# zhipeng-wei/Image-to-Video-I2V-attack

Hardware: AMD Instinct MI355X
Metric: adversarial frames/sec (10-step I2V, ResNet-50 layer3, 32x224^2 clips) (higher is better)
Workload: dtype f32

## Files before the change

### image-to-video-i2v-attack_amd/csrc/i2v_be.h

```cpp
#pragma once
#include <hip/hip_runtime.h>
#include <math.h>
#include <stdint.h>
#include <stdio.h>
#include <stdlib.h>
#include <string.h>

#include <type_traits>
#include <utility>

#include "i2v_kernels.h"

typedef float f32x16 __attribute__((ext_vector_type(16)));
typedef float f32x4 __attribute__((ext_vector_type(4)));

extern thread_local char g_be_err[256];
extern thread_local bool g_be_has_err;
int hip_fail(hipError_t e, const char* what);
#define HIPCHK(x) do { hipError_t e_ = (x); if (e_ != hipSuccess) return hip_fail(e_, #x); } while (0)
#define LAUNCH_CHECK(name) do { hipError_t e_ = hipGetLastError(); if (e_ != hipSuccess) return hip_fail(e_, name); } while (0)
extern long long g_stat_conv, g_stat_pws, g_stat_bf3, g_stat_igh, g_stat_sth, g_stat_fastblock, g_stat_vfma, g_stat_igv, g_stat_gconv;

__device__ __forceinline__ unsigned fastdiv(unsigned n, unsigned m, unsigned s) {
    return (unsigned)(((unsigned long long)n * m) >> s);
}
static inline void fastdiv_magic(unsigned d, uint32_t* m, uint32_t* s) {
    unsigned l = 0; while ((1ull << l) < d) ++l;
    *s = 31 + l;
    *m = (uint32_t)(((1ull << (31 + l)) / d) + 1);
}
typedef int i2v_v4i __attribute__((ext_vector_type(4)));
__device__ __forceinline__ I2VKEntry load_kentry(const I2VKEntry* tab, int k) {
#if defined(__HIP_DEVICE_COMPILE__)
    const i2v_v4i v = ((const __attribute__((address_space(4))) i2v_v4i*)tab)[k];
    return I2VKEntry{v.x, v.y, v.z, v.w};
#else
    return tab[k];
#endif
}

static inline void conv_magics(I2VConvParams& p) {
    fastdiv_magic((unsigned)(p.Hg * p.Wg), &p.dv_hw_m, &p.dv_hw_s);
    fastdiv_magic((unsigned)p.Wg, &p.dv_w_m, &p.dv_w_s);
    fastdiv_magic((unsigned)(p.Tg > 0 ? p.Tg : 1), &p.dv_t_m, &p.dv_t_s);
    fastdiv_magic((unsigned)(p.Wo > 0 ? p.Wo : 1), &p.dv_wo_m, &p.dv_wo_s);
}

static inline bool conv_wants_prefetch(const I2VConvParams& p) {
    return p.vec_epilogue && !p.gate_scale && !p.pre_scale && p.add0_stride == 1 && (p.add0 || p.add1 || p.mask || p.gate) && p.Kpad <= 256 && (p.pointwise || p.tap_uniform) && p.Cd > 32;
}

static inline int conv_tail_px_tiles(const I2VConvParams& p) {
    if (p.quad || p.pre_scale || p.temporal || !(p.pointwise || p.tap_uniform) || p.Cd % 16 != 0 || p.blk > 1) return 0;
    const int64_t P = (int64_t)p.N * p.Hg * p.Wg;
    const int64_t n_px = (P + 63) / 64; const int n_cd = (p.Cd + 63) / 64;
    const int64_t tiles = n_px * n_cd;
    if (tiles < 2 * 256) return 0;
    const int r = (int)(tiles % 256);
    if (r == 0 || r > 104) return 0;
    return r / n_cd;
}

static inline bool conv_halo_ok(const I2VConvParams& p) {
    return p.halo == 9 && p.tap_uniform && !p.temporal && !p.pre_scale && !p.quad && p.blk <= 1 && p.sh == 1 && p.sw == 1 && p.Hs == p.Hg &&
           p.Ws == p.Wg && (p.Ws == 14 || p.Ws == 28 || p.Ws == 56) && p.Kpad == p.K && (p.Kpad / I2V_KC) % 9 == 0;
}

static inline bool conv_dc_ok(const I2VConvParams& p) {
    return (p.pointwise || p.tap_uniform) && !p.temporal && !p.pre_scale && !p.quad && p.Cd > 32 && (p.Kpad / I2V_KC) % 2 == 0 && p.Kpad >= 4 * I2V_KC;
}

static inline bool conv_bf3_ok(const I2VConvParams& p) {
#ifdef I2V_EXPERIMENTAL
    return p.bf3 && p.wp3 && (p.pointwise || p.tap_uniform) && (!p.temporal || p.tap_uniform) && !p.pre_scale && !p.quad && p.blk <= 1 && p.blkt <= 1 && p.Cd > 32;
#else
    (void)p; return false;
#endif
}

int launch_conv_cfg0(const I2VConvParams& p, hipStream_t s);
int launch_conv_cfg1(const I2VConvParams& p, hipStream_t s);
int launch_conv_cfg2(const I2VConvParams& p, hipStream_t s);
int launch_conv_cfg3(const I2VConvParams& p, hipStream_t s);
int launch_conv_cfg4(const I2VConvParams& p, hipStream_t s);
int launch_conv_cfg5(const I2VConvParams& p, hipStream_t s);
bool conv_ighalo_ok(const I2VConvParams& p);
int launch_conv_ighalo(const I2VConvParams& p, hipStream_t s);
bool conv_igvfma_ok(const I2VConvParams& p);
int launch_conv_igvfma(const I2VConvParams& p, hipStream_t s);
bool conv_stemhalo_ok(const I2VConvParams& p);
int launch_conv_stemhalo(const I2VConvParams& p, hipStream_t s);
bool conv_vfma_ok(const I2VConvParams& p);
int launch_conv_vfma(const I2VConvParams& p, hipStream_t s);
#ifdef I2V_EXPERIMENTAL
#ifndef I2V_BF3_VARIANT
#define I2V_BF3_VARIANT 1
#endif
#endif
#ifdef I2V_EXPERIMENTAL
bool conv_stem64_ok(const I2VConvParams& p);
int launch_conv_stem64(const I2VConvParams& p, hipStream_t s);
int conv_pws_grid(const I2VConvParams& p);
int launch_conv_pws(const I2VConvParams& p, hipStream_t s);
int launch_conv_bf3(const I2VConvParams& p, hipStream_t s);
#endif
```

### image-to-video-i2v-attack_amd/csrc/i2v_conv_cfg0.hip

```cpp
#include "i2v_conv_launch.h"

int launch_conv_cfg0(const I2VConvParams& p, hipStream_t s) { return launch_conv_cfg<128, 128, 2, 2>(p, s); }
```

### image-to-video-i2v-attack_amd/csrc/i2v_conv_cfg1.hip

```cpp
#include "i2v_conv_launch.h"

int launch_conv_cfg1(const I2VConvParams& p, hipStream_t s) { return launch_conv_cfg<64, 128, 2, 2>(p, s); }
```

### image-to-video-i2v-attack_amd/csrc/i2v_conv_cfg2.hip

```cpp
#include "i2v_conv_launch.h"

int launch_conv_cfg2(const I2VConvParams& p, hipStream_t s) { return launch_conv_cfg<128, 64, 2, 2>(p, s); }
```

### image-to-video-i2v-attack_amd/csrc/i2v_conv_cfg3.hip

```cpp
#include "i2v_conv_launch.h"

int launch_conv_cfg3(const I2VConvParams& p, hipStream_t s) { return launch_conv_cfg<64, 64, 2, 2>(p, s); }
```

### image-to-video-i2v-attack_amd/csrc/i2v_conv_cfg4.hip

```cpp
#include "i2v_conv_launch.h"

int launch_conv_cfg4(const I2VConvParams& p, hipStream_t s) { return launch_conv_cfg<32, 256, 1, 4>(p, s); }
```

### image-to-video-i2v-attack_amd/csrc/i2v_conv_cfg5.hip

```cpp
#include "i2v_conv_launch.h"

int launch_conv_cfg5(const I2VConvParams& p, hipStream_t s) { return launch_conv_cfg<16, 256, 1, 4, true>(p, s); }
```

### image-to-video-i2v-attack_amd/csrc/i2v_conv_launch.h

```cpp
#pragma once
#include "i2v_conv_tile.h"

template <int BD, int BP, int WD, int WP, bool MF16 = false>
static int launch_conv_cfg(const I2VConvParams& p, hipStream_t s) {
    const int64_t P = (int64_t)p.N * p.Hg * p.Wg;
    const int n_cd = (p.Cd + BD - 1) / BD;
    const int64_t n_px = (P + BP - 1) / BP;
    const int64_t grid = n_px * n_cd;
    if (grid <= 0) return 0;
    if (grid > 0x7fffffff) { snprintf(g_be_err, sizeof g_be_err, "conv grid too large"); g_be_has_err = true; return 1; }
    if (p.quad) {
        if (p.pre_scale || (p.quad != 1 && p.quad != 2)) { snprintf(g_be_err, sizeof g_be_err, "bad quad-row launch"); g_be_has_err = true; return 1; }
        if (p.temporal) hipLaunchKernelGGL((conv_igemm<BD, BP, WD, WP, 4, false, false, true, MF16>), dim3((unsigned)grid), dim3(256), 0, s, p, n_cd);
        else hipLaunchKernelGGL((conv_igemm<BD, BP, WD, WP, 4, false, false, false, MF16>), dim3((unsigned)grid), dim3(256), 0, s, p, n_cd);
        LAUNCH_CHECK("conv_igemm");
        return 0;
    }
    if constexpr (BD == 64 && BP == 64 && !MF16) {
        if (p.cfg > 0 && ((p.cfg - 1) & 16) && conv_halo_ok(p)) {
            if (p.Ws == 14) hipLaunchKernelGGL((conv_igemm_halo<14>), dim3((unsigned)grid), dim3(256), 0, s, p, n_cd);
            else if (p.Ws == 28) hipLaunchKernelGGL((conv_igemm_halo<28>), dim3((unsigned)grid), dim3(256), 0, s, p, n_cd);
            else hipLaunchKernelGGL((conv_igemm_halo<56>), dim3((unsigned)grid), dim3(256), 0, s, p, n_cd);
            LAUNCH_CHECK("conv_igemm_halo");
            return 0;
        }
        if (p.cfg > 0 && ((p.cfg - 1) & 64) && conv_dc_ok(p)) {
            if (p.pointwise) hipLaunchKernelGGL((conv_igemm_dc<1, 2>), dim3((unsigned)grid), dim3(256), 0, s, p, n_cd);
            else hipLaunchKernelGGL((conv_igemm_dc<2, 2>), dim3((unsigned)grid), dim3(256), 0, s, p, n_cd);
            LAUNCH_CHECK("conv_igemm_dc");
            return 0;
        }
        if (p.cfg > 0 && ((p.cfg - 1) & 32)) {
            const int tail = conv_tail_px_tiles(p);
            if (tail > 0 && !conv_wants_prefetch(p)) {
                const int nA = (int)((n_px - tail) * n_cd), n_cd_b = (p.Cd + 15) / 16;
                const int64_t nB = (int64_t)tail * n_cd_b;
                const dim3 g((unsigned)(nA + nB));
                if (p.pointwise) hipLaunchKernelGGL((conv_igemm_tail<1>), g, dim3(256), 0, s, p, n_cd, nA, n_cd_b, (n_px - tail) * 64);
                else hipLaunchKernelGGL((conv_igemm_tail<2>), g, dim3(256), 0, s, p, n_cd, nA, n_cd_b, (n_px - tail) * 64);
                LAUNCH_CHECK("conv_igemm_tail");
                return 0;
            }
        }
    }
    if constexpr (MF16) {
        if (p.pre_scale) { snprintf(g_be_err, sizeof g_be_err, "pre-activation convolutions have no 16-row variant"); g_be_has_err = true; return 1; }
        if (p.pointwise) hipLaunchKernelGGL((conv_igemm<BD, BP, WD, WP, 1, false, false, false, true>), dim3((unsigned)grid), dim3(256), 0, s, p, n_cd);
        else if (p.tap_uniform && p.temporal) hipLaunchKernelGGL((conv_igemm<BD, BP, WD, WP, 2, false, false, true, true>), dim3((unsigned)grid), dim3(256), 0, s, p, n_cd);
        else if (p.tap_uniform) hipLaunchKernelGGL((conv_igemm<BD, BP, WD, WP, 2, false, false, false, true>), dim3((unsigned)grid), dim3(256), 0, s, p, n_cd);
        else if (p.temporal) hipLaunchKernelGGL((conv_igemm<BD, BP, WD, WP, 0, false, false, true, true>), dim3((unsigned)grid), dim3(256), 0, s, p, n_cd);
        else hipLaunchKernelGGL((conv_igemm<BD, BP, WD, WP, 0, false, false, false, true>), dim3((unsigned)grid), dim3(256), 0, s, p, n_cd);
    } else if (p.pre_scale) {
        if (p.temporal) { snprintf(g_be_err, sizeof g_be_err, "pre-activation convolutions have no temporal variant"); g_be_has_err = true; return 1; }
        if constexpr ((BD == 64 && BP == 64) || (BD == 128 && BP == 128)) {
            if (p.pointwise) hipLaunchKernelGGL((conv_igemm<BD, BP, WD, WP, 1, false, true>), dim3((unsigned)grid), dim3(256), 0, s, p, n_cd);
            else if (p.tap_uniform) hipLaunchKernelGGL((conv_igemm<BD, BP, WD, WP, 2, false, true>), dim3((unsigned)grid), dim3(256), 0, s, p, n_cd);
            else hipLaunchKernelGGL((conv_igemm<BD, BP, WD, WP, 0, false, true>), dim3((unsigned)grid), dim3(256), 0, s, p, n_cd);
        }
    } else if (BD == 64 && BP == 64 && conv_wants_prefetch(p) && !(p.cfg > 0 && ((p.cfg - 1) & 8))) {
        if constexpr (BD == 64 && BP == 64) {
            if (p.pointwise) hipLaunchKernelGGL((conv_igemm<BD, BP, WD, WP, 1, true>), dim3((unsigned)grid), dim3(256), 0, s, p, n_cd);
            else if (p.temporal) hipLaunchKernelGGL((conv_igemm<BD, BP, WD, WP, 2, true, false, true>), dim3((unsigned)grid), dim3(256), 0, s, p, n_cd);
            else hipLaunchKernelGGL((conv_igemm<BD, BP, WD, WP, 2, true>), dim3((unsigned)grid), dim3(256), 0, s, p, n_cd);
        }
    } else if (p.pointwise) hipLaunchKernelGGL((conv_igemm<BD, BP, WD, WP, 1, false>), dim3((unsigned)grid), dim3(256), 0, s, p, n_cd);
    else if (p.tap_uniform && p.temporal) hipLaunchKernelGGL((conv_igemm<BD, BP, WD, WP, 2, false, false, true>), dim3((unsigned)grid), dim3(256), 0, s, p, n_cd);
    else if (p.tap_uniform) hipLaunchKernelGGL((conv_igemm<BD, BP, WD, WP, 2, false>), dim3((unsigned)grid), dim3(256), 0, s, p, n_cd);
    else if (p.temporal) hipLaunchKernelGGL((conv_igemm<BD, BP, WD, WP, 0, false, false, true>), dim3((unsigned)grid), dim3(256), 0, s, p, n_cd);
    else hipLaunchKernelGGL((conv_igemm<BD, BP, WD, WP, 0, false>), dim3((unsigned)grid), dim3(256), 0, s, p, n_cd);
    LAUNCH_CHECK("conv_igemm");
    return 0;
}
```

### image-to-video-i2v-attack_amd/csrc/i2v_conv_tile.h

```cpp
#pragma once
#include "i2v_be.h"

#ifndef I2V_PROBE_T
struct I2VNoProbe {
    __device__ __forceinline__ void entry() {}
    __device__ __forceinline__ void loop_begin() {}
    __device__ __forceinline__ void loop_end(int ) {}
    __device__ __forceinline__ void exit(int ) {}
};
#define I2V_PROBE_T I2VNoProbe
#endif

#ifndef I2V_PRIO_LEVELS
#define I2V_PRIO_LEVELS 3
#endif
#ifndef I2V_DEEP
#define I2V_DEEP 1
#endif
#ifndef I2V_DEEP_STAGES
#define I2V_DEEP_STAGES 3
#endif
#ifndef I2V_BF3_STAGES
#define I2V_BF3_STAGES 2
#endif
// ... 572 lines not shown
                const float rl = lo - __builtin_bit_cast(float, a << 16), rh = hi - __builtin_bit_cast(float, a & 0xffff0000u);
                asm("v_cvt_pk_bf16_f32 %0, %1, %2" : "=v"(b) : "v"(rl), "v"(rh));
                const float sl = rl - __builtin_bit_cast(float, b << 16), sh = rh - __builtin_bit_cast(float, b & 0xffff0000u);
                asm("v_cvt_pk_bf16_f32 %0, %1, %2" : "=v"(c) : "v"(sl), "v"(sh));
                p1 = a; p2 = b; p3 = c;
            };
            bf8 wnxt[BF3 == 2 ? CPB : 1][BF3 == 2 ? TD : 1][3];
            if constexpr (BF3 == 2 && MORE) {
#pragma unroll
                for (int sb = 0; sb < CPB; ++sb)
#pragma unroll
                    for (int i = 0; i < TD; ++i)
#pragma unroll
                        for (int pl = 0; pl < 3; ++pl) wnxt[sb][i][pl] = load_w3((c + 1) * CPB + sb, i, pl);
            }
            (void)wnxt;
            [&]<int... SB>(std::integer_sequence<int, SB...>) {
                (([&] {
                    constexpr int sub = SB;
                    bf8 wa[TD][3], xb[TP][3];
                    if constexpr (BF3 == 2) {
#pragma unroll
                        for (int i = 0; i < TD; ++i)
#pragma unroll
                            for (int pl = 0; pl < 3; ++pl) wa[i][pl] = wcur[sub][i][pl];
                    } else {
                        const float* const abase = As3 + buf * AF + sub * (AF / CPB) + lane * 4;
#pragma unroll
                        for (int i = 0; i < TD; ++i)
#pragma unroll
                            for (int pl = 0; pl < 3; ++pl)
                                wa[i][pl] = __builtin_bit_cast(bf8, *reinterpret_cast<const f4*>(abase + ((wd * TD + i) * 3 + pl) * 256));
                    }
#pragma unroll
                    for (int j = 0; j < TP; ++j) {
                        float x[8];
#pragma unroll
                        for (int e = 0; e < 8; ++e) x[e] = Bs[buf][sub * KC + 8 * lk + e][wpx * (BP / WP) + j * FR + l31];
                        unsigned q1[4], q2[4], q3[4];
#pragma unroll
                        for (int e = 0; e < 4; ++e) split2(x[2 * e], x[2 * e + 1], q1[e], q2[e], q3[e]);
                        typedef unsigned u4 __attribute__((ext_vector_type(4)));
                        xb[j][0] = __builtin_bit_cast(bf8, (u4){q1[0], q1[1], q1[2], q1[3]});
                        xb[j][1] = __builtin_bit_cast(bf8, (u4){q2[0], q2[1], q2[2], q2[3]});
                        xb[j][2] = __builtin_bit_cast(bf8, (u4){q3[0], q3[1], q3[2], q3[3]});
                    }
                    constexpr int TW[6] = {2, 1, 0, 1, 0, 0}, TX[6] = {0, 1, 2, 0, 1, 0};
                    [&]<int... M>(std::integer_sequence<int, M...>) {
                        (([&] {
                            constexpr int m = M, term = m / (TD * TP), ij = m % (TD * TP), i = ij / TP, j = ij % TP;
                            acc[i][j] = __builtin_amdgcn_mfma_f32_32x32x16_bf16(wa[i][TW[term]], xb[j][TX[term]], acc[i][j], 0, 0, 0);
                            if constexpr (MORE) {
                                constexpr int jp = sub * 6 * TD * TP + m;
                                if constexpr (jp < CPB * NL) {
                                    constexpr int sb2 = jp / NL;
                                    I2V_ISSUE_PIECE_SUB(jp % NL, ((c + AHEAD) * CPB + sb2) * KC, (buf + AHEAD) % NST, vb[sb2], sb2);
                                }
                            }
                        }()), ...);
                    }(std::make_integer_sequence<int, 6 * TD * TP>{});
                }()), ...);
            }(std::make_integer_sequence<int, CPB>{});
            if constexpr (BF3 == 2 && MORE) {
#pragma unroll
                for (int sb = 0; sb < CPB; ++sb)
#pragma unroll
                    for (int i = 0; i < TD; ++i)
#pragma unroll
                        for (int pl = 0; pl < 3; ++pl) wcur[sb][i][pl] = wnxt[sb][i][pl];
            }
            return;
        }
        float fa[2][TD], fb[2][TP];
        auto read_frags = [&](const int s, const int set) {
#pragma unroll
            for (int i = 0; i < TD; ++i) fa[set][i] = As[buf][KR * s + lk][wd * (BD / WD) + i * FR + l31];
            if constexpr (QUAD) {
                const float* const bq = &Bs[buf][0][0];
#pragma unroll
                for (int j = 0; j < TP; ++j) {
                    const int px = wpx * (BP / WP) + j * FR + l31;
                    const int qd = MF16 ? s : (s >> 1), el = MF16 ? lk : 2 * (s & 1) + lk;
                    const float v = bq[(qd * BP + px) * 4 + el];
                    const bool m = ((qd & 1) && p.quad == 2) ? qok[j][1][MF16 ? 0 : (s & 1)] : qok[j][0][MF16 ? 0 : (s & 1)];
                    fb[set][j] = m ? v : 0.f;
                }
            } else {
#pragma unroll
                for (int j = 0; j < TP; ++j) fb[set][j] = Bs[buf][KR * s + lk][wpx * (BP / WP) + j * FR + l31];
            }
        };
        read_frags(0, 0);
        [&]<int... S>(std::integer_sequence<int, S...>) {
            (([&] {
                constexpr int s = S, set = S & 1;
                if constexpr (s + 1 < CPB * KS) read_frags(s + 1, set ^ 1);
                __builtin_amdgcn_sched_barrier(0);
                if constexpr (PRE) {
                    typedef const __attribute__((address_space(4))) float* cfp;
                    const int kr = c * KB + 2 * s;
                    const float sc = lk ? ((cfp)p.pre_scale)[kr + 1] : ((cfp)p.pre_scale)[kr];
                    const float sh = lk ? ((cfp)p.pre_shift)[kr + 1] : ((cfp)p.pre_shift)[kr];
#pragma unroll
                    for (int j = 0; j < TP; ++j) fb[set][j] = fmaxf(fmaf(fb[set][j], sc, sh), 0.f);
                }
#pragma unroll
                for (int i = 0; i < TD; ++i)
#pragma unroll
                    for (int j = 0; j < TP; ++j) {
                        if constexpr (MF16) acc[i][j] = __builtin_amdgcn_mfma_f32_16x16x4f32(fa[set][i], fb[set][j], acc[i][j], 0, 0, 0);
                        else acc[i][j] = __builtin_amdgcn_mfma_f32_32x32x2f32(fa[set][i], fb[set][j], acc[i][j], 0, 0, 0);
                    }
                if constexpr (MORE) {
                    [&]<int... Q>(std::integer_sequence<int, Q...>) {
                        (([&] {
                            constexpr int jp = s * PPS + Q;
                            if constexpr (jp < CPB * NL) {
                                constexpr int sub = jp / NL;
                                I2V_ISSUE_PIECE_SUB(jp % NL, ((c + AHEAD) * CPB + sub) * KC, DEEP ? (buf + AHEAD) % NST : (buf ^ 1), vb[sub], sub);
                            }
                        }()), ...);
                    }(std::make_integer_sequence<int, PPS>{});
                }
            }()), ...);
        }(std::make_integer_sequence<int, CPB * KS>{});
    };
    if constexpr (BF3 == 3) {
        asm volatile("s_waitcnt vmcnt(0)" ::: "memory");
        __builtin_amdgcn_s_barrier();
        const int l31_ = lane & 31, lk_ = lane >> 5;
#pragma unroll
        for (int j = 0; j < TP_; ++j) {
            float x[8];
#pragma unroll
            for (int e = 0; e < 8; ++e) x[e] = Bs[0][8 * lk_ + e][(wave % WP) * (BP / WP) + j * 32 + l31_];
            bf3_split_frag(x, xcur[j]);
        }
    }
    if constexpr (!HALO) {
        int c = 0, buf = 0;
        for (; c + AHEAD < nsuper; ++c) { chunk_body(c, buf, std::true_type{}); buf = buf + 1 == NST ? 0 : buf + 1; }
        for (; c < nsuper; ++c) { chunk_body(c, buf, std::false_type{}); buf = buf + 1 == NST ? 0 : buf + 1; }
    }
#undef I2V_ISSUE_PIECE
#undef I2V_ISSUE_PIECE_SUB
#undef I2V_CHUNK_VB
    if (prio_hi > 0) __builtin_amdgcn_s_setprio(0);
    probe.loop_end(probe_slot);

    const int HoWo = p.Ho * p.Wo;
    if (p.vec_epilogue) {
        conv_vec_epilogue<BD, BP, WD, WP, PREF, MF16, FUSE != 0>(p, acc, cd0, px0, smem, pre0, pregw, mid);
        return;
    }
    if (p.blk > 1 || (VID && p.blkt > 1)) {
        const int bb = p.blk * p.blk, Creal = p.Cd / ((VID ? p.blkt : 1) * bb);
#pragma unroll
        for (int j = 0; j < TP; ++j) {
            const int64_t pp = px0 + wpx * (BP / WP) + j * FR + l31;
            if (pp >= P) continue;
            const int64_t ng = fastdiv((unsigned)pp, p.dv_hw_m, p.dv_hw_s);
            const int rem = (int)(pp - ng * HWg);
            const int gi = (int)fastdiv((unsigned)rem, p.dv_w_m, p.dv_w_s), gj = rem - gi * p.Wg;
            const int64_t clip = VID ? fastdiv((unsigned)ng, p.dv_t_m, p.dv_t_s) : ng;
            const int otb = VID ? (int)(ng - clip * p.Tg) * p.ost + p.ot0 : 0;
#pragma unroll
            for (int i = 0; i < TD; ++i)
#pragma unroll
                for (int r = 0; r < NR; ++r) {
                    const int cd = cd0 + wd * (BD / WD) + i * FR + I2V_FROW(r);
                    if (cd >= p.Cd) continue;
                    const int cls3 = cd / Creal, c = cd - cls3 * Creal;
                    const int ct = VID ? cls3 / bb : 0, cls = cls3 - ct * bb;
                    const int oh = gi * p.osh + cls / p.blk + p.oh0, ow = gj * p.osw + cls % p.blk + p.ow0;
                    if (oh >= p.Ho || ow >= p.Wo || (VID && otb + ct * p.oct >= p.To)) continue;
                    const int64_t n = VID ? clip * p.To + otb + ct * p.oct : ng;
                    const int64_t o = (int64_t)c * HoWo + oh * p.Wo + ow;
                    float v = acc[i][j][r];
                    if (p.shift) v += p.shift[c];
                    if (p.add1) v += p.add1[n * p.add1_nstride + o];
                    if (p.relu) v = fmaxf(v, 0.f);
                    if (p.mask && !(p.mask[n * p.mask_nstride + o] > 0.f)) v = 0.f;
                    p.dst[n * p.dst_nstride + o] = v;
                }
        }
        return;
    }
#pragma unroll
    for (int j = 0; j < TP; ++j) {
        const int64_t pp = px0 + wpx * (BP / WP) + j * FR + l31;
        const bool pin = pp < P;
        const int64_t ng = pin ? fastdiv((unsigned)pp, p.dv_hw_m, p.dv_hw_s) : 0;
        const int rem = (int)(pin ? pp - ng * HWg : 0);
        const int gi = (int)fastdiv((unsigned)rem, p.dv_w_m, p.dv_w_s), gj = rem - gi * p.Wg;
        const int oh = gi * p.osh + p.oh0, ow = gj * p.osw + p.ow0;
        bool ok = pin && oh < p.Ho && ow < p.Wo;
        int64_t n = ng;
        if (VID) {
            const int64_t clip = fastdiv((unsigned)ng, p.dv_t_m, p.dv_t_s);
            const int ot = (int)(ng - clip * p.Tg) * p.ost + p.ot0;
            if (ot >= p.To) ok = false;
            n = clip * p.To + ot;
        }
        const int opix = oh * p.Wo + ow;
        float* dstn = p.dst + n * p.dst_nstride + opix;
        const float* a0 = nullptr; int a0_plane = HoWo;
        if (p.add0 && ok) {
            if (p.add0_stride == 1) a0 = p.add0 + n * p.add0_nstride + opix;
            else {
                const int s = p.add0_stride, qh = oh / s, qw = ow / s;
                if (qh * s == oh && qw * s == ow && qh < p.add0_H && qw < p.add0_W) {
                    a0 = p.add0 + n * p.add0_nstride + qh * p.add0_W + qw;
                    a0_plane = p.add0_H * p.add0_W;
                }
            }
        }
        const float* a1 = p.add1 ? p.add1 + n * p.add1_nstride + opix : nullptr;
        const float* mk = p.mask ? p.mask + n * p.mask_nstride + opix : nullptr;
        const int64_t gidx = (int64_t)p.gate_pix0 + n * HoWo + opix;
#pragma unroll
        for (int i = 0; i < TD; ++i) {
#pragma unroll
            for (int r = 0; r < NR; ++r) {
                const int cd = cd0 + wd * (BD / WD) + i * FR + I2V_FROW(r);
                const bool okc = ok && cd < p.Cd;
                float v = 0.f;
                if (okc) {
                    v = acc[i][j][r];
                    if (p.gate_scale && !(fmaf(mk[(int64_t)cd * HoWo], p.gate_scale[cd], p.gate_shift[cd]) > 0.f)) v = 0.f;
                    if (p.shift) v += p.shift[cd];
                    if (a0) v += a0[(int64_t)cd * a0_plane];
                    if (a1) v += a1[(int64_t)cd * HoWo];
                    if (p.relu) v = fmaxf(v, 0.f);
                    if (p.gate) { if (!((p.gate[(int64_t)cd * p.gate_stride + (gidx >> 5)] >> (gidx & 31)) & 1u)) v = 0.f; }
                    else if (mk && !p.gate_scale && !(mk[(int64_t)cd * HoWo] > 0.f)) v = 0.f;
                    dstn[(int64_t)cd * HoWo] = v;
                }
                if (p.gate_out) {
                    const unsigned long long bal = __ballot(okc && v > 0.f);
                    if (l31 == 0 && pin && cd < p.Cd) {
                        const int64_t bit0 = (int64_t)p.gate_out_pix0 + pp;
                        if constexpr (MF16)
                            reinterpret_cast<uint16_t*>(p.gate_out + (int64_t)cd * p.gate_out_stride)[bit0 >> 4] = (uint16_t)(bal >> (16 * lk));
                        else
                            p.gate_out[(int64_t)cd * p.gate_out_stride + (bit0 >> 5)] = (unsigned)(bal >> (32 * lk));
                    }
                }
            }
        }
    }
#undef I2V_FROW
#endif
}

template <int BD, int BP, int WD, int WP, int MODE, bool PREF, bool PRE = false, bool VID = false, bool MF16 = false>
__global__ void __launch_bounds__(256) I2V_CONV_WPE conv_igemm(const I2VConvParams p, const int n_cd_tiles) {
    __shared__ __attribute__((aligned(16))) float smem[conv_lds_floats<BD, BP, WD, MF16, conv_deep(MODE, PREF) ? I2V_DEEP_STAGES : 2>()];
    I2V_PROBE_T probe;
    probe.entry();
    conv_tile<BD, BP, WD, WP, MODE, PREF, PRE, VID, MF16>(p, n_cd_tiles, blockIdx.x, gridDim.x, 0, smem, probe, blockIdx.x);
    probe.exit(blockIdx.x);
}

template <int HWM>
__global__ void __launch_bounds__(256) __attribute__((amdgpu_waves_per_eu(HWM <= 14 ? I2V_SMALL_WPE : (HWM <= 28 ? 6 : 5), HWM <= 14 ? I2V_SMALL_WPE : (HWM <= 28 ? 6 : 5))))
conv_igemm_halo(const I2VConvParams p, const int n_cd_tiles) {
    __shared__ __attribute__((aligned(16))) float smem[conv_halo_lds_floats<HWM>()];
    I2V_PROBE_T probe;
    probe.entry();
    conv_tile<64, 64, 2, 2, 5, false, false, false, false, HWM>(p, n_cd_tiles, blockIdx.x, gridDim.x, 0, smem, probe, blockIdx.x);
    probe.exit(blockIdx.x);
}

#ifndef I2V_DC_WPE
#define I2V_DC_WPE 5
#endif
template <int MODE, int CPB>
__global__ void __launch_bounds__(256) __attribute__((amdgpu_waves_per_eu(I2V_DC_WPE, I2V_DC_WPE)))
conv_igemm_dc(const I2VConvParams p, const int n_cd_tiles) {
    __shared__ __attribute__((aligned(16))) float smem[conv_lds_floats<64, 64, 2, false, 2, CPB>()];
    I2V_PROBE_T probe;
    probe.entry();
    conv_tile<64, 64, 2, 2, MODE, false, false, false, false, 0, CPB>(p, n_cd_tiles, blockIdx.x, gridDim.x, 0, smem, probe, blockIdx.x);
    probe.exit(blockIdx.x);
}


template <int MODE>
__global__ void __launch_bounds__(256) __attribute__((amdgpu_waves_per_eu(I2V_SMALL_WPE, I2V_SMALL_WPE)))
conv_igemm_tail(const I2VConvParams p, const int n_cd_a, const int nA, const int n_cd_b, const int64_t px_base_b) {
    constexpr int LA = conv_lds_floats<64, 64, 2, false>(), LB = conv_lds_floats<16, 64, 1, true>();
    __shared__ __attribute__((aligned(16))) float smem[LA > LB ? LA : LB];
    I2V_PROBE_T probe;
    probe.entry();
    const int slot = (int)blockIdx.x < nA ? (int)blockIdx.x : 65536 + (int)blockIdx.x - nA;
    if ((int)blockIdx.x < nA) conv_tile<64, 64, 2, 2, MODE, false, false, false, false>(p, n_cd_a, blockIdx.x, nA, 0, smem, probe, slot, I2V_PRIO_LEVELS > 2 ? 2 : I2V_PRIO_LEVELS);
    else {
        if (I2V_PRIO_LEVELS > 0) __builtin_amdgcn_s_setprio(3);
        conv_tile<16, 64, 1, 4, MODE, false, false, false, true>(p, n_cd_b, (int)blockIdx.x - nA, (int)gridDim.x - nA, px_base_b, smem, probe, slot, 0);
        if (I2V_PRIO_LEVELS > 0) __builtin_amdgcn_s_setprio(0);
    }
    probe.exit(slot);
}
```

### image-to-video-i2v-attack_amd/csrc/i2v_engine.cpp

```cpp
#include "i2v_net.h"

#include <math.h>
#include <stdarg.h>
#include <stdio.h>
#include <stdlib.h>
#include <string.h>

using namespace eng;

#define I2V_MAX_NETS 4096
thread_local std::string eng::g_err;

int eng::fail(const char* fmt, ...) {
    char buf[512];
    va_list ap;
    va_start(ap, fmt);
    vsnprintf(buf, sizeof buf, fmt, ap);
    va_end(ap);
    g_err = buf;
    return 1;
}

int i2v_api_fail(const char* msg) { return fail("%s", msg); }

// ... 17 lines not shown
static void free_net(Net* n) {
    if (!n) return;
    for (void* p : n->dev_allocs) be_free(p);
    if (n->arena) be_free(n->arena);
    for (void* e : n->ov_ev) be_event_destroy(e);
    if (n->side) be_stream_destroy(n->side);
    delete n;
}

extern "C" int i2v_destroy(i2v_handle h) {
    if (!h) return 0;
    for (Net* n : h->nets) free_net(n);
    for (auto& t : h->timed) { be_event_destroy(t.start); be_event_destroy(t.stop); }
    delete h;
    return 0;
}

extern "C" int i2v_net_create(i2v_handle h, int* net) {
    if (!h || !net) return fail("i2v_net_create: null argument");
    std::lock_guard<std::mutex> lock(h->nets_mu);
    for (size_t i = 0; i < h->nets.size(); ++i)
        if (!h->nets[i]) { h->nets[i] = new Net(); *net = (int)i; return 0; }
    if (h->nets.size() >= I2V_MAX_NETS) return fail("more than %d backbones alive on one handle", I2V_MAX_NETS);
    h->nets.push_back(new Net());
    *net = (int)h->nets.size() - 1;
    return 0;
}

extern "C" int i2v_net_destroy(i2v_handle h, int net) {
    Net* n = get_net(h, net); if (!n) return 1;
    free_net(n);
    std::lock_guard<std::mutex> lock(h->nets_mu);
    h->nets[net] = nullptr;
    return 0;
}

extern "C" int i2v_net_add_buffer3d(i2v_handle h, int net, int C, int T, int H, int W, int* buf) {
    Net* n = get_net(h, net); if (!n) return 1;
    if (n->planned) return fail("net already planned");
    if (C <= 0 || T <= 0 || H <= 0 || W <= 0 || !buf) return fail("bad buffer shape %dx%dx%dx%d", C, T, H, W);
    Buffer b{C, H, W}; b.T = T;
    n->bufs.push_back(b);
    *buf = (int)n->bufs.size() - 1;
    return 0;
}

extern "C" int i2v_net_add_buffer(i2v_handle h, int net, int C, int H, int W, int* buf) {
    return i2v_net_add_buffer3d(h, net, C, 1, H, W, buf);
}

extern "C" int i2v_net_add_tensor(i2v_handle h, int net, int buf, int c_off, int C, int post_relu, int* tensor) {
    Net* n = get_net(h, net); if (!n) return 1;
    if (buf < 0 || buf >= (int)n->bufs.size()) return fail("bad buffer id %d", buf);
    if (c_off < 0 || C <= 0 || c_off + C > n->bufs[buf].C) return fail("tensor view outside buffer");
    n->tens.push_back(Tensor{buf, c_off, C, post_relu != 0});
    *tensor = (int)n->tens.size() - 1;
    return 0;
}

extern "C" int i2v_net_tensor_frames(i2v_handle h, int net, int tensor, int* T) {
    Net* n = get_net(h, net); if (!n) return 1;
    if (tensor < 0 || tensor >= (int)n->tens.size() || !T) return fail("bad tensor id");
    *T = n->bufs[n->tens[tensor].buf].T;
    return 0;
}

extern "C" int i2v_net_set_input(i2v_handle h, int net, int tensor) {
    Net* n = get_net(h, net); if (!n) return 1;
    if (tensor < 0 || tensor >= (int)n->tens.size()) return fail("bad tensor id");
    n->input = tensor;
    n->bufs[n->tens[tensor].buf].is_input = true;
    return 0;
}

extern "C" int i2v_net_set_relu_gain(i2v_handle h, int net, int tensor, float gain) {
    Net* n = get_net(h, net); if (!n) return 1;
    if (n->planned) return fail("net already planned");
    if (tensor < 0 || tensor >= (int)n->tens.size()) return fail("bad tensor id");
    if (!n->tens[tensor].post_relu) return fail("i2v_net_set_relu_gain: tensor %d is not the output of a ReLU", tensor);
    if (!(gain > 0.f) || !isfinite(gain)) return fail("i2v_net_set_relu_gain: the gain must be positive and finite");
    n->tens[tensor].bwd_gain = gain;
    return 0;
}

extern "C" int i2v_net_add_conv3d(i2v_handle h, int net, const i2v_conv3d_desc* d, const float* weight,
                                  const float* scale, const float* shift) {
    Net* n = get_net(h, net); if (!n) return 1;
    if (n->planned) return fail("net already planned");
    if (!d || !weight || !scale || !shift) return fail("i2v_net_add_conv: null argument");
    int nt = (int)n->tens.size();
    if (d->src < 0 || d->src >= nt || d->dst < 0 || d->dst >= nt || d->residual >= nt)
        return fail("i2v_net_add_conv: bad tensor id");
    const Tensor& S = n->tens[d->src]; const Tensor& D = n->tens[d->dst];
    const Buffer& sb = n->bufs[S.buf]; const Buffer& db = n->bufs[D.buf];
    if (S.C != d->cin || D.C != d->cout) return fail("conv channel mismatch");
    if (d->stride < 1 || d->kh < 1 || d->kw < 1 || d->pad < 0 || d->kt < 1 || d->stride_t < 1 || d->pad_t < 0 || d->dil_t < 1)
        return fail("bad conv geometry");
    int Ho = (sb.H + 2 * d->pad - d->kh) / d->stride + 1, Wo = (sb.W + 2 * d->pad - d->kw) / d->stride + 1;
    int To = (sb.T + 2 * d->pad_t - d->dil_t * (d->kt - 1) - 1) / d->stride_t + 1;
    if (Ho != db.H || Wo != db.W) return fail("conv output %dx%d does not match buffer %dx%d", Ho, Wo, db.H, db.W);
    if (To != db.T) return fail("conv output has %d frames per clip, buffer has %d", To, db.T);
    if (d->residual >= 0) {
        const Tensor& R = n->tens[d->residual]; const Buffer& rb = n->bufs[R.buf];
        if (R.C != d->cout || rb.H != db.H || rb.W != db.W || rb.T != db.T) return fail("residual shape mismatch");
    }
    Node nd; nd.type = 0; nd.cd = *d; memset(&nd.pd, 0, sizeof nd.pd);
    size_t per = (size_t)d->cin * d->kt * d->kh * d->kw;
    nd.w.resize((size_t)d->cout * per);
    for (int co = 0; co < d->cout; ++co)
        for (size_t i = 0; i < per; ++i) nd.w[co * per + i] = weight[co * per + i] * scale[co];
    nd.shift.assign(shift, shift + d->cout);
    n->nodes.push_back(std::move(nd));
    return 0;
}

extern "C" int i2v_net_add_conv(i2v_handle h, int net, const i2v_conv_desc* d, const float* weight,
                                const float* scale, const float* shift) {
    if (!d) return fail("i2v_net_add_conv: null argument");
    i2v_conv3d_desc q{d->src, d->dst, d->cin, d->cout, 1, d->kh, d->kw, 1, d->stride, 0, d->pad, 1, d->relu, d->residual};
    return i2v_net_add_conv3d(h, net, &q, weight, scale, shift);
}

extern "C" int i2v_net_add_conv_grouped(i2v_handle h, int net, const i2v_conv_desc* d, int groups, const float* weight,
                                        const float* scale, const float* shift) {
    if (!d || !weight || !scale || !shift) return fail("i2v_net_add_conv_grouped: null argument");
    if (groups == 1) return i2v_net_add_conv(h, net, d, weight, scale, shift);
    if (groups < 1 || d->cin % groups || d->cout % groups)
        return fail("i2v_net_add_conv_grouped: %d input and %d output channels are not divisible by %d groups", d->cin, d->cout, groups);
    if (d->kh != 3 || d->kw != 3 || d->pad != 1 || (d->stride != 1 && d->stride != 2))
        return fail("i2v_net_add_conv_grouped: only 3x3 / pad 1 / stride 1 or 2 is supported (got %dx%d, pad %d, stride %d)", d->kh, d->kw, d->pad, d->stride);
    const int gi = d->cin / groups, go = d->cout / groups;
    if (gi != go || (gi != 4 && gi != 8 && gi != 16 && gi != 32 && gi != 64))
        return fail("i2v_net_add_conv_grouped: group width %d -> %d is not one of 4, 8, 16, 32, 64 in and out (depthwise is not supported)", gi, go);
    if (d->residual >= 0) return fail("i2v_net_add_conv_grouped: a residual addend on a grouped convolution is not supported");
    std::vector<float> dense((size_t)d->cout * d->cin * 9, 0.f);
    for (int co = 0; co < d->cout; ++co)
        for (int ci = 0; ci < gi; ++ci)
            for (int t = 0; t < 9; ++t)
                dense[((size_t)co * d->cin + (co / go) * gi + ci) * 9 + t] = weight[((size_t)co * gi + ci) * 9 + t];
    if (i2v_net_add_conv(h, net, d, dense.data(), scale, shift)) return 1;
    Node& nd = get_net(h, net)->nodes.back();
    nd.groups = groups;
    nd.wg.resize((size_t)d->cout * gi * 9);
    for (int co = 0; co < d->cout; ++co)
        for (int i = 0; i < gi * 9; ++i) nd.wg[(size_t)co * gi * 9 + i] = weight[(size_t)co * gi * 9 + i] * scale[co];
    std::vector<float>().swap(nd.w);
    return 0;
}

static void expand_grouped(Node& nd) {
    const i2v_conv3d_desc& c = nd.cd;
    const int gi = c.cin / nd.groups, go = c.cout / nd.groups;
    nd.w.assign((size_t)c.cout * c.cin * 9, 0.f);
    for (int co = 0; co < c.cout; ++co)
        for (int ci = 0; ci < gi; ++ci)
            for (int t = 0; t < 9; ++t) nd.w[((size_t)co * c.cin + (co / go) * gi + ci) * 9 + t] = nd.wg[((size_t)co * gi + ci) * 9 + t];
}

extern "C" int i2v_net_add_conv_preact(i2v_handle h, int net, const i2v_conv_desc* d, const float* weight,
                                       const float* scale, const float* shift, const float* pre_scale,
                                       const float* pre_shift) {
    if (!d || !pre_scale || !pre_shift) return fail("i2v_net_add_conv_preact: null argument");
    if (d->kh != 1 || d->kw != 1 || d->stride != 1 || d->pad != 0 || d->residual >= 0)
        return fail("pre-activation is supported on plain 1x1/stride-1 convolutions only");
    if (i2v_net_add_conv(h, net, d, weight, scale, shift)) return 1;
    Net* n = get_net(h, net);
    if (n->tens[d->src].post_relu) return fail("pre-activation input must not be a ReLU output");
    Node& nd = n->nodes.back();
    nd.pre_scale.assign(pre_scale, pre_scale + d->cin);
    nd.pre_shift.assign(pre_shift, pre_shift + d->cin);
    return 0;
}

extern "C" int i2v_net_add_maxpool3d(i2v_handle h, int net, const i2v_pool3d_desc* d) {
    Net* n = get_net(h, net); if (!n) return 1;
    if (n->planned) return fail("net already planned");
    int nt = (int)n->tens.size();
    if (!d || d->src < 0 || d->src >= nt || d->dst < 0 || d->dst >= nt) return fail("bad pool desc");
    if (n->tens[d->src].C != n->tens[d->dst].C) return fail("pool channel mismatch");
    if (d->kt < 1 || d->k < 1 || d->stride_t < 1 || d->stride < 1 || d->pad_t < 0 || d->pad < 0) return fail("bad pool geometry");
    const Buffer& sb = n->bufs[n->tens[d->src].buf]; const Buffer& db = n->bufs[n->tens[d->dst].buf];
    if ((sb.T + 2 * d->pad_t - d->kt) / d->stride_t + 1 != db.T) return fail("pool output frames per clip do not match the buffer");
    {
        const int ho = (sb.H + 2 * d->pad - d->k) / d->stride + 1, hc = (sb.H + 2 * d->pad - d->k + d->stride - 1) / d->stride + 1;
        const int wo = (sb.W + 2 * d->pad - d->k) / d->stride + 1, wc = (sb.W + 2 * d->pad - d->k + d->stride - 1) / d->stride + 1;
        if (sb.H + 2 * d->pad < d->k || sb.W + 2 * d->pad < d->k || db.H < ho || db.H > hc || db.W < wo || db.W > wc)
            return fail("pool output plane %dx%d does not match %dx%d pooled by k=%d stride=%d pad=%d", db.H, db.W, sb.H, sb.W, d->k, d->stride, d->pad);
    }
    Node nd; nd.type = 1; nd.pd = *d; memset(&nd.cd, 0, sizeof nd.cd);
    n->nodes.push_back(std::move(nd));
    return 0;
}

extern "C" int i2v_net_add_maxpool(i2v_handle h, int net, const i2v_pool_desc* d) {
    if (!d) return fail("bad pool desc");
    i2v_pool3d_desc q{d->src, d->dst, 1, d->k, 1, d->stride, 0, d->pad};
    return i2v_net_add_maxpool3d(h, net, &q);
}

extern "C" int i2v_net_add_avgpool(i2v_handle h, int net, const i2v_pool_desc* d) {
    if (i2v_net_add_maxpool(h, net, d)) return 1;
    Net* n = get_net(h, net);
    if (d->pad != 0) return fail("average pooling with padding is not supported");
    n->nodes.back().type = 2;
    return 0;
}

extern "C" int i2v_net_add_attention(i2v_handle h, int net, const i2v_attn_desc* d) {
    Net* n = get_net(h, net); if (!n) return 1;
    if (n->planned) return fail("net already planned");
    const int nt = (int)n->tens.size();
    if (!d) return fail("bad attention desc");
    for (int t : {d->theta, d->phi, d->g, d->dst}) if (t < 0 || t >= nt) return fail("bad attention tensor");
    const Tensor& th = n->tens[d->theta]; const Tensor& ph = n->tens[d->phi]; const Tensor& gg = n->tens[d->g]; const Tensor& ds = n->tens[d->dst];
    if (th.C != ph.C || th.C != gg.C || th.C != ds.C) return fail("attention: theta / phi / g / dst channel counts differ");
    const Buffer& tb = n->bufs[th.buf]; const Buffer& pb = n->bufs[ph.buf]; const Buffer& gb = n->bufs[gg.buf]; const Buffer& db = n->bufs[ds.buf];
    if (tb.T != db.T || tb.H != db.H || tb.W != db.W) return fail("attention: dst must have theta's positions");
    if (pb.T != gb.T || pb.H != gb.H || pb.W != gb.W) return fail("attention: phi and g must have the same positions");
    if (th.post_relu || ph.post_relu || gg.post_relu) return fail("attention: theta / phi / g are linear embeddings (no ReLU)");
    if (!(d->scale > 0.f)) return fail("attention: scale must be positive");
    Node nd; nd.type = 3; nd.ad = *d; memset(&nd.cd, 0, sizeof nd.cd); memset(&nd.pd, 0, sizeof nd.pd);
    n->nodes.push_back(std::move(nd));
    return 0;
}

extern "C" int i2v_net_plan(i2v_handle h, int net, const int* hook_tensors, int n_hooks, int max_frames) {
    Net* np = get_net(h, net); if (!np) return 1;
    Net& n = *np;
    if (n.planned) return fail("net already planned");
    if (n.input < 0) return fail("input tensor not set");
    if (n_hooks <= 0 || max_frames <= 0) return fail("need >=1 hook and >=1 frame");
    if (math_bf16x3() && strncmp(be_name(), "hip", 3) == 0 && be_stat("experimental") != 1)
        return fail("I2V_MATH=bf16x3 needs a library built with -DI2V_EXPERIMENTAL (python __graft_entry__.py --experimental, then I2V_LIB=...)");
    for (int i = 0; i < n_hooks; ++i)
        if (hook_tensors[i] < 0 || hook_tensors[i] >= (int)n.tens.size()) return fail("bad hook tensor");
    n.hooks.assign(hook_tensors, hook_tensors + n_hooks);
    n.maxN = max_frames;
    const size_t N = (size_t)max_frames;
    const int Tin = n.Tin();
    if (max_frames % Tin) return fail("max_frames=%d is not a multiple of the input's %d frames per clip", max_frames, Tin);

    for (Node& nd : n.nodes) {
        if (nd.type != 0) continue;
        if (upload(n, nd.shift, &nd.shift_d)) return 1;
        nd.gconv = nd.groups > 1 && gconv_enabled();
        if (nd.gconv) {
            if (nd.cd.src == n.input) return fail("a grouped convolution directly on the input is not planned");
            if (pack_gconv(n, nd)) return 1;
            continue;
        }
        if (nd.groups > 1) expand_grouped(nd);
        if (pack_fwd(n, nd)) return 1;
        if (nd.preact()) {
            std::vector<float> ps(nd.fwd.Kpad > nd.fwd.Cdpad ? nd.fwd.Kpad : nd.fwd.Cdpad, 0.f), pt(ps.size(), 0.f);
            for (int c = 0; c < nd.cd.cin; ++c) { ps[c] = nd.pre_scale[c]; pt[c] = nd.pre_shift[c]; }
            if (upload(n, ps, &nd.pre_scale_d) || upload(n, pt, &nd.pre_shift_d)) return 1;
        }
        if (nd.cd.src == n.input) { if (pack_img(n, nd)) return 1; }
        else if (pack_bwd(n, nd)) return 1;
        if (nd.groups > 1) std::vector<float>().swap(nd.w);
    }
    size_t off = 64;
    for (const Node& nd : n.nodes) if (nd.type == 0 && nd.cd.src == n.input && nd.fwd.quad) n.stage_input = true;
    if (n.stage_input) {
        const Buffer& ib = n.bufs[n.tens[n.input].buf];
        n.in_stage_off = off; off = align_up(off + N * ib.C * ib.H * ib.W, 64) + 64;
    }
    for (Buffer& b : n.bufs) {
        if (b.is_input) continue;
        size_t sz = N / Tin * b.T * b.C * b.H * b.W;
        b.act_off = off; off = align_up(off + sz, 64);
        b.grad_off = off; off = align_up(off + sz, 64);
    }
    const char* gates_env = getenv("I2V_GATES");
    const bool use_gates = !(gates_env && gates_env[0] == '0');
    for (const Node& nd : n.nodes)
        if (use_gates && nd.type == 0 && nd.cd.relu && !nd.fwd.tpair) n.bufs[n.tens[nd.cd.dst].buf].gated = true;
    for (Buffer& b : n.bufs) {
        if (!b.gated) continue;
        const size_t pix = N / Tin * b.T * b.H * b.W;
        if (pix + 64 >= (1ull << 31)) return fail("gate rows of more than 2^31 bits are not supported");
        b.gate_words = (int)((pix + 31) / 32 + 2);
        b.gate_off = off; off = align_up(off + (size_t)b.C * b.gate_words, 64);
    }
    for (Node& nd : n.nodes)
        if (nd.type == 1) {
            const Buffer& db = n.bufs[n.tens[nd.pd.dst].buf];
            nd.idx_off = off; off = align_up(off + (N / Tin * db.T * n.tens[nd.pd.dst].C * db.H * db.W + 3) / 4, 64);
        }
    for (Node& nd : n.nodes)
        if (nd.type == 3) {
            const Buffer& tb = n.bufs[n.tens[nd.ad.theta].buf]; const Buffer& pb = n.bufs[n.tens[nd.ad.phi].buf];
            nd.p_off = off; off = align_up(off + N / Tin * ((size_t)tb.T * tb.H * tb.W) * ((size_t)pb.T * pb.H * pb.W), 64);
        }
    std::string err;
    size_t end = 0;
    if (!plan_pass(n, true, off, N, &end, &err)) return fail("plan: %s", err.c_str());
    n.arena_floats = end + 64;
    n.arena = (float*)be_malloc(n.arena_floats * sizeof(float));
    if (!n.arena) return fail("arena allocation of %zu bytes failed", n.arena_floats * sizeof(float));
    CHECK_BE(be_memset0(n.arena, n.arena_floats * sizeof(float), nullptr));
    if (!plan_pass(n, false, off, N, &end, &err)) return fail("plan: %s", err.c_str());
    mark_fusable(n);
    if (autotune(n)) return 1;
    mark_overlap(n);
    CHECK_BE(be_stream_sync(nullptr));
    n.planned = true;
    return 0;
}

extern "C" int i2v_net_fusion_info(i2v_handle h, int net, int32_t out[4]) {
    Net* n = get_net(h, net); if (!n) return 1;
    if (!n->planned || !out) return fail("i2v_net_fusion_info: net not planned");
    out[0] = out[1] = out[2] = out[3] = 0;
    int k = 0;
    for (const std::vector<Launch>* L : {&n->fwd, &n->bwd}) {
        for (const Launch& l : *L) { out[k] += l.fuse_ok ? 1 : 0; out[2 + k] += (l.fuse_ok && l.fuse_b[0]) ? 1 : 0; }
        ++k;
    }
    return 0;
}

extern "C" size_t i2v_net_workspace_bytes(i2v_handle h, int net) {
    Net* n = get_net(h, net); if (!n) return 0;
    return n->arena_floats * sizeof(float) + n->weight_bytes;
}

#ifndef I2V_SEPARATE_UNITS
#include "i2v_pack.cpp"
#include "i2v_plan.cpp"
#include "i2v_tune.cpp"
#include "i2v_run.cpp"
#include "i2v_loop_api.cpp"
#endif
```

### image-to-video-i2v-attack_amd/csrc/i2v_kernels.h

```cpp
#pragma once
#include <initializer_list>
#include "i2v_params.h"

typedef void* i2v_stream_t;

const char* be_name();
long long be_stat(const char* name);
int  be_set_device(int device);
void* be_malloc(size_t bytes);
void be_free(void* p);
int  be_h2d(void* dst, const void* src, size_t bytes);
int  be_d2d_2d(void* dst, size_t dpitch, const void* src, size_t spitch, size_t width, size_t rows,
               i2v_stream_t s);
int  be_memset0(void* p, size_t bytes, i2v_stream_t s);
const char* be_error();
int  i2v_api_fail(const char* msg);
void* be_event_create();
void be_event_destroy(void* ev);
int  be_event_record(void* ev, i2v_stream_t s);
int  be_event_elapsed_ms(void* start, void* stop, float* ms);
int  be_stream_sync(i2v_stream_t s);
i2v_stream_t be_stream_create();
void be_stream_destroy(i2v_stream_t s);
int  be_stream_wait_event(i2v_stream_t s, void* ev);
int  be_device_sync();

int k_conv(const I2VConvParams& p, i2v_stream_t s);
int k_conv_fusable(const I2VConvParams& a, const I2VConvParams& b);
inline bool i2v_conv_pair_fusable(const I2VConvParams& a, const I2VConvParams& b) {
    if (a.pointwise || !a.tap_uniform || a.temporal || a.quad || a.pre_scale || a.gate_scale || a.blk > 1 || a.blkt > 1) return false;
    for (const I2VConvParams* q : {&a, &b})
        if (!(q->Tg == q->Ts && q->Ts == q->To && q->st == 1 && q->ost == 1 && q->ot0 == 0 && q->blkt <= 1)) return false;
    if (a.sh != 1 || a.sw != 1 || a.Hs != a.Hg || a.Ws != a.Wg || a.Hg != a.Ho || a.Wg != a.Wo || a.osh != 1 || a.osw != 1 || a.oh0 || a.ow0) return false;
    if ((a.Cd != 64 && a.Cd != 128) || a.Kpad != a.K || a.add0_stride > 1) return false;
    if (!b.pointwise || b.temporal || b.quad || b.pre_scale || b.gate_scale || b.blk > 1 || b.blkt > 1 || b.add0_stride > 1) return false;
    if (b.K != a.Cd || b.Kpad != b.K || b.Cs != a.Cd || b.src != a.dst || b.src_nstride != a.dst_nstride) return false;
    if (b.Hs != a.Ho || b.Ws != a.Wo || b.Hg != a.Hg || b.Wg != a.Wg || b.Ho != a.Ho || b.Wo != a.Wo || b.sh != 1 || b.sw != 1 || b.osh != 1 || b.osw != 1 ||
        b.oh0 || b.ow0 || b.Cd < 64 || b.Tg != a.Tg) return false;
    return true;
}
int k_conv_fused(const I2VConvParams& a, const I2VConvParams& b, int halo, i2v_stream_t s);
int k_conv_candidates(const I2VConvParams& p, int* out);
inline int i2v_fastblock_rows(const I2VConvParams& a, const I2VConvParams& b, const I2VConvParams* c, const I2VConvParams* d) {
    auto plain = [](const I2VConvParams& q) {
        return !q.pre_scale && !q.gate_scale && q.blk <= 1 && q.blkt <= 1 && q.sh == 1 && q.sw == 1 && q.osh == 1 && q.osw == 1 && q.oh0 == 0 &&
               q.ow0 == 0 && q.Hs == q.Hg && q.Hg == q.Ho && q.Ws == q.Wg && q.Wg == q.Wo && q.Tg == q.Ts && q.Ts == q.To && q.st == 1 && q.ost == 1 && q.ot0 == 0 &&
               !q.add1 && !q.mask && q.Kpad % 8 == 0 && q.Kpad <= 512 && q.gate_pix0 == 0 && q.gate_out_pix0 == 0;
    };
    if (!plain(a) || !plain(b) || a.quad || a.add0 || b.add0) return 0;
    const int CM = a.Cd;
    if ((CM != 4 && CM != 8) || b.Cd != CM || b.Cs != CM || b.src != a.dst || b.src_nstride != a.dst_nstride) return 0;
    if (b.Hg != a.Hg || b.Wg != a.Wg || b.Tg != a.Tg || b.N != a.N) return 0;
    const int H = a.Hg, W = a.Wg;
    if ((H * W) % 32 != 0 || (int64_t)a.N * a.src_nstride * 4 >= (1ll << 31)) return 0;
    if (c) {
        if (!plain(*c) || c->quad || !a.relu || !b.relu || a.gate || b.gate || c->gate || !c->relu || !a.shift || !b.shift || !c->shift || !a.gate_out || !b.gate_out || !c->gate_out) return 0;
        if (c->src != b.dst || c->src_nstride != b.dst_nstride || c->Cs != CM || c->K != CM || c->Cd != 4 * CM || c->Hg != H || c->Wg != W || c->Tg != a.Tg || c->N != a.N) return 0;
        if (!c->add0 || c->add0_stride != 1) return 0;
        if (d) {
            if (!plain(*d) || d->quad || d->relu || d->add0 || d->gate || d->gate_out || !d->shift || d->src != a.src || d->src_nstride != a.src_nstride || d->Cs != a.Cs ||
                d->K != a.Cs || d->K != CM || d->Cd != c->Cd || d->Hg != H || d->Wg != W || d->Tg != a.Tg || d->N != a.N || c->add0 != d->dst || c->add0_nstride != d->dst_nstride) return 0;
        }
    } else {
        if (d || a.relu || b.relu || a.gate_out || b.gate_out || a.shift || b.shift || !a.gate || !b.gate || a.K != a.Cs || a.K > 64) return 0;
    }
    int g = W, r32 = 32; while (r32) { const int t = g % r32; g = r32; r32 = t; }
    const int Rq = 32 / g;
    if (H % Rq != 0) return 0;
    int R = Rq;
    while (R * W < 192 && R * 2 <= H && H % (R * 2) == 0) R *= 2;
    if ((size_t)CM * (R + 2) * (W + 2) * 4 > 60 * 1024) return 0;
    return R;
}
int k_fastblock(const I2VConvParams& a, const I2VConvParams& b, const I2VConvParams* c, const I2VConvParams* d, i2v_stream_t s);
int k_gconv_plan(I2VGConvParams* p);
int k_gconv(const I2VGConvParams& p, i2v_stream_t s);
int k_pool_fwd(const I2VPoolParams& p, i2v_stream_t s);
int k_pool_bwd(const I2VPoolParams& p, i2v_stream_t s);
int k_pool3d_fwd(const I2VPoolParams& p, i2v_stream_t s);
int k_pool3d_bwd(const I2VPoolParams& p, i2v_stream_t s);
int k_avgpool_fwd(const I2VPoolParams& p, i2v_stream_t s);
int k_avgpool_bwd(const I2VPoolParams& p, i2v_stream_t s);
int k_addmask(const I2VAddMaskParams& p, i2v_stream_t s);
int k_cos(const I2VCosParams& p, i2v_stream_t s);
int k_std_reduce(const I2VStdParams& p, i2v_stream_t s);
int k_std_grad(const I2VStdParams& p, i2v_stream_t s);
int k_ilaf_reduce(const I2VIlafParams& p, i2v_stream_t s);
int k_ilaf_grad(const I2VIlafParams& p, i2v_stream_t s);
int k_head_ce(const I2VHeadParams& p, i2v_stream_t s);
int k_clip_from_u8(const uint8_t* frames, float* video, int b, int t, int h, int w, i2v_stream_t s);
int k_clip_resize_crop(const uint8_t* frames, float* video, const int32_t* xtab, const int32_t* ytab, int b, int t, int H, int W,
                       int cy, int cx, int oh, int ow, i2v_stream_t s);
int k_frames_from_video(const float* video, float* x, float* u, int b, int f, int h, int w, i2v_stream_t s);
int k_compose(const float* u, const float* delta, float* x, int b, int f, int h, int w, float eps,
              int video_layout, i2v_stream_t s);
int k_adam(float* delta, float* m, float* v, const float* gx, const float* u, int64_t n, int hw,
           float eps, float step_size, float bc2_sqrt, float w1, float beta2, float w2, float adam_eps,
           i2v_stream_t s);
int k_sign_bim(float* adv, const float* u, const float* grad, int64_t n, int64_t chan_stride,
               float step, float eps, i2v_stream_t s);
int k_sign_delta(float* delta, const float* grad, int64_t n, float step, i2v_stream_t s);
int k_sign_delta_gx(float* delta, const float* gx, const float* u, int64_t n, float eps, float step,
                    i2v_stream_t s);
int k_clip_resample_crop(const uint8_t* frames, float* video, const int32_t* xb, const int32_t* xk, int kx, const int32_t* yb, const int32_t* yk,
                         int ky, int b, int t, int H, int W, int cy, int cx, int oh, int ow, i2v_stream_t s);
int k_tt_grad_mix(const float* grads, float* out, const float* kern , const int* moves , int D, int64_t NC, int T,
                  int HW, float w1, float w, i2v_stream_t s);
int k_attn_gemm(const I2VAttnGemm& p, i2v_stream_t s);
int k_softmax_rows(const I2VSoftmaxRows& p, i2v_stream_t s);
int k_resample_nearest(const float* src, float* dst, int64_t planes, int Hs, int Ws, int Hd, int Wd, const int32_t* map_y,
                       const int32_t* map_x, i2v_stream_t s);
int k_resample_nearest_bwd(const float* g, float* gsrc, int64_t planes, int Hd, int Wd, int Hs, int Ws, const int32_t* ylo,
                           const int32_t* yhi, const int32_t* xlo, const int32_t* xhi, i2v_stream_t s);
int k_grad_post_groups(int b, int c, int f, int h, int w, int mode, int64_t* group_elems);
int k_grad_post_splits(int64_t group_elems);
int k_grad_post(const float* g, float* momentum, float* out, int b, int c, int f, int h, int w, int frame_major, int mode, float decay,
                double* partial, i2v_stream_t s);
int k_tap_perts(const float* adv, const float* videos, float* out, int b, int c, int f, int h, int w, i2v_stream_t s);
int k_tap_sign_abs(const float* smooth, float* sign_out, float* reg, int64_t n, double* partial, i2v_stream_t s);
int k_tap_grad(const float* gx, const float* boxsign, float* out, int b, int c, int f, int h, int w, float weight, i2v_stream_t s);
int k_dwconv1d(const float* src, float* dst, int64_t outer, int len, int64_t inner, const float* taps , int k, i2v_stream_t s);
int k_aens_coeffs(const float* prev, float* coeffs, float momentum, int L, i2v_stream_t s);
int k_aens_reduce(const float* cos, const float* coeffs, int L, int frames, float* feat_sum,
                  float* weighted, i2v_stream_t s);
int cos_nblk(int64_t D);
```

### image-to-video-i2v-attack_amd/csrc/i2v_kernels.hip

```cpp
#include "i2v_be.h"

thread_local char g_be_err[256];
thread_local bool g_be_has_err = false;

int hip_fail(hipError_t e, const char* what) {
    snprintf(g_be_err, sizeof g_be_err, "%s: %s", what, hipGetErrorString(e));
    g_be_has_err = true;
    return 1;
}

const char* be_name() { return "hip:gfx950"; }
long long g_stat_conv = 0, g_stat_pws = 0, g_stat_bf3 = 0, g_stat_igh = 0, g_stat_sth = 0;
long long be_stat(const char* name) {
    if (!strcmp(name, "conv_launches")) return __atomic_load_n(&g_stat_conv, __ATOMIC_RELAXED);
    if (!strcmp(name, "pws_launches")) return __atomic_load_n(&g_stat_pws, __ATOMIC_RELAXED);
    if (!strcmp(name, "bf3_launches")) return __atomic_load_n(&g_stat_bf3, __ATOMIC_RELAXED);
    if (!strcmp(name, "ighalo_launches")) return __atomic_load_n(&g_stat_igh, __ATOMIC_RELAXED);
    if (!strcmp(name, "stemhalo_launches")) return __atomic_load_n(&g_stat_sth, __ATOMIC_RELAXED);
    if (!strcmp(name, "fastblock_launches")) return __atomic_load_n(&g_stat_fastblock, __ATOMIC_RELAXED);
    if (!strcmp(name, "vfma_launches")) return __atomic_load_n(&g_stat_vfma, __ATOMIC_RELAXED);
    if (!strcmp(name, "igvfma_launches")) return __atomic_load_n(&g_stat_igv, __ATOMIC_RELAXED);
    if (!strcmp(name, "gconv_launches")) return __atomic_load_n(&g_stat_gconv, __ATOMIC_RELAXED);
#ifdef I2V_EXPERIMENTAL
    if (!strcmp(name, "experimental")) return 1;
#else
    if (!strcmp(name, "experimental")) return 0;
#endif
    return -1;
}
const char* be_error() { return g_be_has_err ? g_be_err : nullptr; }
int be_set_device(int device) { HIPCHK(hipSetDevice(device)); return 0; }
void* be_malloc(size_t bytes) { void* p = nullptr; if (hipMalloc(&p, bytes) != hipSuccess) return nullptr; return p; }
void be_free(void* p) { (void)hipFree(p); }
int be_h2d(void* dst, const void* src, size_t bytes) { HIPCHK(hipMemcpy(dst, src, bytes, hipMemcpyHostToDevice)); return 0; }
int be_d2d_2d(void* dst, size_t dpitch, const void* src, size_t spitch, size_t width, size_t rows, i2v_stream_t s) {
    HIPCHK(hipMemcpy2DAsync(dst, dpitch, src, spitch, width, rows, hipMemcpyDeviceToDevice, (hipStream_t)s));
    return 0;
}
int be_memset0(void* p, size_t bytes, i2v_stream_t s) { HIPCHK(hipMemsetAsync(p, 0, bytes, (hipStream_t)s)); return 0; }

void* be_event_create() { hipEvent_t e = nullptr; if (hipEventCreate(&e) != hipSuccess) return nullptr; return (void*)e; }
void be_event_destroy(void* ev) { (void)hipEventDestroy((hipEvent_t)ev); }
int be_event_record(void* ev, i2v_stream_t s) { HIPCHK(hipEventRecord((hipEvent_t)ev, (hipStream_t)s)); return 0; }
int be_event_elapsed_ms(void* a, void* b, float* ms) { HIPCHK(hipEventElapsedTime(ms, (hipEvent_t)a, (hipEvent_t)b)); return 0; }
int be_stream_sync(i2v_stream_t s) { HIPCHK(hipStreamSynchronize((hipStream_t)s)); return 0; }
int be_device_sync() { HIPCHK(hipDeviceSynchronize()); return 0; }
i2v_stream_t be_stream_create() { hipStream_t s = nullptr; if (hipStreamCreateWithFlags(&s, hipStreamNonBlocking) != hipSuccess) return nullptr; return (i2v_stream_t)s; }
void be_stream_destroy(i2v_stream_t s) { if (s) (void)hipStreamDestroy((hipStream_t)s); }
int be_stream_wait_event(i2v_stream_t s, void* ev) { HIPCHK(hipStreamWaitEvent((hipStream_t)s, (hipEvent_t)ev, 0)); return 0; }

__constant__ float c_mean[3] = {0.485f, 0.456f, 0.406f};
__constant__ float c_std[3] = {0.229f, 0.224f, 0.225f};

static int conv_pick(const I2VConvParams& p) {
    const char* force = getenv("I2V_FORCE_CFG");
    if (force && *force) { const int f = atoi(force); return (p.pre_scale && f != 0 && f != 3) ? 3 : f; }
    if (p.Cd <= 16 && !p.pre_scale) return 5;
    if (conv_bf3_ok(p)) return p.Cd > 64 ? 2 : 3;
    if (conv_wants_prefetch(p)) return 3;
    if (p.pre_scale) {
        const double blocks128 = ceil(p.Cd / 128.0) * ceil((double)p.N * p.Hg * p.Wg / 128.0);
        return (p.Cd > 64 && blocks128 >= 256.0 * 6) ? 0 : 3;
    }
    static const struct { int BD, BP, occ; double ineff; } C[5] = {
        {128, 128, 3, 1.00}, {64, 128, 5, 1.05}, {128, 64, 5, 1.04}, {64, 64, 7, 1.10}, {32, 256, 4, 1.08}};
    const double P = (double)p.N * p.Hg * p.Wg;
    const int nchunks = p.Kpad / I2V_KC;
    int best = 0; double best_t = 1e300;
    for (int i = 0; i < 5; ++i) {
        if (C[i].BD > 32 && p.Cd <= C[i].BD / 2) continue;
        if (C[i].BD == 32 && p.Cd > 32) continue;
        const double blocks = ceil(p.Cd / (double)C[i].BD) * ceil(P / C[i].BP);
        const double rounds = ceil(blocks / 256.0);
        const double fill = blocks / (256.0 * C[i].occ);
        const double mfma = (double)nchunks * (C[i].BD / 32) * (C[i].BP / 32) / 4 * 8 * 64 * C[i].ineff *
                            (1.0 + 0.15 * (fill < 1.0 ? 1.0 - fill : 0.0));
        const double overhead = 1500.0 + (C[i].BD * C[i].BP / 256) * 10.0;
        const double t = rounds * mfma + ceil(rounds / C[i].occ) * overhead;
        if (t < best_t) { best_t = t; best = i; }
    }
    return best;
}

int k_conv_candidates(const I2VConvParams& p, int* out) {
    int n = 0;
    if (p.pre_scale) { if (p.Cd > 64) out[n++] = 0; out[n++] = 3; return n; }
#ifdef I2V_EXPERIMENTAL
    if (conv_bf3_ok(p)) {
        static const int BD3[4] = {128, 64, 128, 64};
        for (int i = 0; i < 4; ++i) {
            if (p.Cd <= BD3[i] / 2) continue;
            out[n++] = i;
            if (I2V_BF3_VARIANT == 2 && (p.Kpad / I2V_KC) % 2 == 0) out[n++] = i | 64;
            if (I2V_BF3_VARIANT == 1 && i == 0 && !p.temporal) out[n++] = 0 | 64;
        }
        return n;
    }
#endif
    static const int BD[5] = {128, 64, 128, 64, 32};
    for (int i = 0; i < 5; ++i) {
        if (BD[i] > 32 && p.Cd <= BD[i] / 2) continue;
        if (BD[i] == 32 && p.Cd > 32) continue;
        out[n++] = i;
    }
    if (conv_wants_prefetch(p)) out[n++] = 3 | 8;
    else if (conv_tail_px_tiles(p) > 0 && p.Cd > 32) out[n++] = 3 | 32;
    static const bool no_halo = [] { const char* e = getenv("I2V_HALO"); return e && e[0] == '0'; }();
    if (conv_halo_ok(p) && p.Cd > 32 && !no_halo) out[n++] = 3 | 16;
    static const bool no_dc = [] { const char* e = getenv("I2V_DC"); return e && e[0] == '0'; }();
    if (conv_dc_ok(p) && !no_dc) out[n++] = 3 | 64;
    if (p.Cd <= 16) out[n++] = 5;
    static const bool no_igh = [] { const char* e = getenv("I2V_IGHALO"); return e && e[0] == '0'; }();
    if (conv_ighalo_ok(p) && !no_igh) out[n++] = (p.Cd <= 16 ? 5 : 4) | 512;
    if (conv_stemhalo_ok(p) && !no_igh) out[n++] = 5 | 1024;
    static const bool no_vfma = [] { const char* e = getenv("I2V_VFMA"); return e && e[0] == '0'; }();
    if (conv_vfma_ok(p) && !no_vfma) out[n++] = (p.Cd <= 16 ? 5 : 4) | 2048;
    if (conv_igvfma_ok(p) && !no_vfma) out[n++] = 5 | 4096;
#ifdef I2V_EXPERIMENTAL
    static const bool want_stem64 = [] { const char* e = getenv("I2V_STEM64"); return e && e[0] == '1'; }();
    if (conv_stem64_ok(p) && want_stem64) out[n++] = 3 | 1024;
    static const bool want_pws = [] { const char* e = getenv("I2V_PWS"); return e && e[0] == '1'; }();
    if (want_pws && conv_pws_grid(p)) out[n++] = 3 | 256;
#endif
    return n;
}

#ifndef I2V_EXPERIMENTAL
int k_conv_fusable(const I2VConvParams&, const I2VConvParams&) { return 0; }
int k_conv_fused(const I2VConvParams&, const I2VConvParams&, int, i2v_stream_t) {
    snprintf(g_be_err, sizeof g_be_err, "fused conv launch: this library was built without -DI2V_EXPERIMENTAL"); g_be_has_err = true;
    return 1;
}
#endif

int k_conv(const I2VConvParams& p_in, i2v_stream_t s) {
    hipStream_t st = (hipStream_t)s;
    I2VConvParams p = p_in;
    if ((int64_t)p.N * p.Hg * p.Wg + 1024 >= (1ll << 31)) { snprintf(g_be_err, sizeof g_be_err, "conv launch of more than 2^31 grid pixels"); g_be_has_err = true; return 1; }
    conv_magics(p);
    if (p.cfg <= 0) p.cfg = conv_pick(p) + 1;
    __atomic_fetch_add(&g_stat_conv, 1, __ATOMIC_RELAXED);
#ifdef I2V_EXPERIMENTAL
    if (((p.cfg - 1) & 1024) && conv_stem64_ok(p) && !((uintptr_t)p.src & 15)) {
        __atomic_fetch_add(&g_stat_sth, 1, __ATOMIC_RELAXED);
        return launch_conv_stem64(p, st);
    }
#endif
    if (((p.cfg - 1) & 1024) && conv_stemhalo_ok(p) && !((uintptr_t)p.src & 15)) {
        __atomic_fetch_add(&g_stat_sth, 1, __ATOMIC_RELAXED);
        return launch_conv_stemhalo(p, st);
    }
    if (((p.cfg - 1) & 2048) && conv_vfma_ok(p)) {
        __atomic_fetch_add(&g_stat_vfma, 1, __ATOMIC_RELAXED);
        return launch_conv_vfma(p, st);
    }
    if (((p.cfg - 1) & 4096) && conv_igvfma_ok(p)) {
        __atomic_fetch_add(&g_stat_igv, 1, __ATOMIC_RELAXED);
        return launch_conv_igvfma(p, st);
    }
    if (((p.cfg - 1) & 512) && conv_ighalo_ok(p)) {
        __atomic_fetch_add(&g_stat_igh, 1, __ATOMIC_RELAXED);
        return launch_conv_ighalo(p, st);
    }
    if (((p.cfg - 1) & 1024) && p.quad && !p.ig_th && p.sh > 1) {
        snprintf(g_be_err, sizeof g_be_err, "conv launch pinned to a halo-tile stem kernel (configuration bit 10) is not eligible for one (source %s16-byte aligned)",
                 ((uintptr_t)p.src & 15) ? "not " : "");
        g_be_has_err = true;
        return 1;
    }
#ifdef I2V_EXPERIMENTAL
    if (((p.cfg - 1) & 256) && conv_pws_grid(p)) {
        __atomic_fetch_add(&g_stat_pws, 1, __ATOMIC_RELAXED);
        return launch_conv_pws(p, st);
    }
    if (conv_bf3_ok(p) && ((p.cfg - 1) & 7) <= 3) {
        __atomic_fetch_add(&g_stat_bf3, 1, __ATOMIC_RELAXED);
        return launch_conv_bf3(p, st);
    }
#endif
    switch ((p.cfg - 1) & 7) {
        case 0: return launch_conv_cfg0(p, st);
        case 1: return launch_conv_cfg1(p, st);
        case 2: return launch_conv_cfg2(p, st);
        case 3: return launch_conv_cfg3(p, st);
        case 5: return launch_conv_cfg5(p, st);
        default: return launch_conv_cfg4(p, st);
    }
}

#define POOL_LDS_FLOATS 8192
#define POOL_FWD_LDS_FLOATS 4096
__global__ void __launch_bounds__(256) pool_fwd_kernel(const I2VPoolParams p, const int band_rows) {
    __shared__ float xs[POOL_FWD_LDS_FLOATS];
    const int plane = blockIdx.x, n = plane / p.C, c = plane - n * p.C;
    const int ho0 = blockIdx.y * band_rows, ho1 = min(ho0 + band_rows, p.Ho);
    const int h_lo = max(ho0 * p.stride - p.pad, 0), h_hi = min((ho1 - 1) * p.stride - p.pad + p.k, p.Hs);
    const float* x = p.x + (int64_t)n * p.x_nstride + (int64_t)c * p.Hs * p.Ws;
    const int cnt = (h_hi - h_lo) * p.Ws;
    const float* xb = x + h_lo * p.Ws;
    if (((p.Ws & 3) == 0) && ((((uintptr_t)xb) & 15) == 0)) {
        for (int e = threadIdx.x * 4; e < cnt; e += 1024) *reinterpret_cast<float4*>(&xs[e]) = *reinterpret_cast<const float4*>(xb + e);
    } else {
        for (int e = threadIdx.x; e < cnt; e += 256) xs[e] = xb[e];
    }
    __syncthreads();
    float* y = p.y + (int64_t)n * p.y_nstride + (int64_t)c * p.Ho * p.Wo;
    uint8_t* ix = p.idx + (int64_t)plane * p.Ho * p.Wo;
    const int nout = (ho1 - ho0) * p.Wo;
    for (int e = threadIdx.x; e < nout; e += 256) {
        const int ho = ho0 + e / p.Wo, wo = e % p.Wo;
        int best = -1; float bv = 0.f;
        for (int kr = 0; kr < p.k; ++kr) {
            const int h = ho * p.stride - p.pad + kr; if (h < 0 || h >= p.Hs) continue;
            for (int ks = 0; ks < p.k; ++ks) {
                const int w = wo * p.stride - p.pad + ks; if (w < 0 || w >= p.Ws) continue;
                const float v = xs[(h - h_lo) * p.Ws + w];
                if (best < 0 || v > bv || v != v) { bv = v; best = kr * p.k + ks; }
            }
        }
        y[ho * p.Wo + wo] = bv;
        ix[ho * p.Wo + wo] = (uint8_t)best;
    }
}

template <int KK, int SS, int PP>
__global__ void __launch_bounds__(256) pool_bwd_kernel(const I2VPoolParams p, const int band_rows) {
    const int pk = KK ? KK : p.k, pstride = KK ? SS : p.stride, ppad = KK ? PP : p.pad;
    __shared__ float gs[POOL_LDS_FLOATS / 2];
    __shared__ uint8_t is[POOL_LDS_FLOATS / 2];
    const int plane = blockIdx.x, n = plane / p.C, c = plane - n * p.C;
    const int h0 = blockIdx.y * band_rows, h1 = min(h0 + band_rows, p.Hs);
    int ho_lo = h0 + ppad - pk + 1; ho_lo = ho_lo <= 0 ? 0 : (ho_lo + pstride - 1) / pstride;
    const int ho_hi = min((h1 - 1 + ppad) / pstride, p.Ho - 1);
    const float* gy = p.y + (int64_t)n * p.y_nstride + (int64_t)c * p.Ho * p.Wo;
    const float* yv = p.yact ? p.yact + (int64_t)n * p.yact_nstride + (int64_t)c * p.Ho * p.Wo : nullptr;
    const uint8_t* ix = p.idx + (int64_t)plane * p.Ho * p.Wo;
    const int cnt = (ho_hi - ho_lo + 1) * p.Wo;
    for (int e = threadIdx.x; e < cnt; e += 256) {
        float g = gy[ho_lo * p.Wo + e];
        if (yv && !(yv[ho_lo * p.Wo + e] > 0.f)) g = 0.f;
        gs[e] = g; is[e] = ix[ho_lo * p.Wo + e];
    }
    __syncthreads();
    const float* x = p.x + (int64_t)n * p.x_nstride + (int64_t)c * p.Hs * p.Ws;
    float* gx = p.gx + (int64_t)n * p.gx_nstride + (int64_t)c * p.Hs * p.Ws;
    const int nin = (h1 - h0) * p.Ws;
    const bool gate_x = p.mask_relu && !yv;
    const bool vec = ((p.Ws & 3) == 0) && ((((uintptr_t)(x + h0 * p.Ws) | (uintptr_t)(gx + h0 * p.Ws)) & 15) == 0);
    for (int e4 = threadIdx.x * (vec ? 4 : 1); e4 < nin; e4 += 256 * (vec ? 4 : 1)) {
        float xv[4] = {1.f, 1.f, 1.f, 1.f}, gv[4];
        if (gate_x) {
            if (vec) { const float4 t4 = *reinterpret_cast<const float4*>(x + h0 * p.Ws + e4); xv[0] = t4.x; xv[1] = t4.y; xv[2] = t4.z; xv[3] = t4.w; }
            else xv[0] = x[h0 * p.Ws + e4];
        }
        const int h = h0 + e4 / p.Ws, wb = e4 % p.Ws;
        int a_lo = h + ppad - pk + 1; a_lo = a_lo <= 0 ? 0 : (a_lo + pstride - 1) / pstride;
        const int a_hi = min((h + ppad) / pstride, p.Ho - 1);
#pragma unroll
        for (int u = 0; u < 4; ++u) {
            if (!vec && u > 0) break;
            const int w = wb + u;
            float g = 0.f;
            if (!gate_x || xv[u] > 0.f) {
                int b_lo = w + ppad - pk + 1; b_lo = b_lo <= 0 ? 0 : (b_lo + pstride - 1) / pstride;
                const int b_hi = min((w + ppad) / pstride, p.Wo - 1);
                for (int ho = a_lo; ho <= a_hi; ++ho)
                    for (int wo = b_lo; wo <= b_hi; ++wo) {
                        const int me = (h - (ho * pstride - ppad)) * pk + (w - (wo * pstride - ppad));
                        const int li = (ho - ho_lo) * p.Wo + wo;
                        if (is[li] == me) g += gs[li];
                    }
            }
            gv[u] = g;
        }
        if (vec) *reinterpret_cast<float4*>(gx + h0 * p.Ws + e4) = make_float4(gv[0], gv[1], gv[2], gv[3]);
        else gx[h0 * p.Ws + e4] = gv[0];
    }
}

__global__ void __launch_bounds__(256) pool_bwd_321_kernel(const I2VPoolParams p, const int band_pairs, const unsigned w4_m, const unsigned w4_s) {
    __shared__ float gs[POOL_LDS_FLOATS / 2];
    __shared__ uint8_t is[POOL_LDS_FLOATS / 2];
    const int plane = blockIdx.x, n = plane / p.C, c = plane - n * p.C;
    const int a0 = blockIdx.y * band_pairs, a1 = min(a0 + band_pairs, p.Hs >> 1);
    const int ho_lo = a0, ho_hi = min(a1, p.Ho - 1);
    const float* gy = p.y + (int64_t)n * p.y_nstride + (int64_t)c * p.Ho * p.Wo;
    const float* yv = p.yact ? p.yact + (int64_t)n * p.yact_nstride + (int64_t)c * p.Ho * p.Wo : nullptr;
    const uint8_t* ix = p.idx + (int64_t)plane * p.Ho * p.Wo;
    const int cnt = (ho_hi - ho_lo + 1) * p.Wo;
    for (int e = threadIdx.x; e < cnt; e += 256) {
        float g = gy[ho_lo * p.Wo + e];
        if (yv && !(yv[ho_lo * p.Wo + e] > 0.f)) g = 0.f;
        gs[e] = g; is[e] = ix[ho_lo * p.Wo + e];
    }
    __syncthreads();
    float* gx = p.gx + (int64_t)n * p.gx_nstride + (int64_t)c * p.Hs * p.Ws;
    const int W4 = p.Ws >> 2, items = (a1 - a0) * W4;
    for (int e = threadIdx.x; e < items; e += 256) {
        const int al = (int)fastdiv((unsigned)e, w4_m, w4_s), b = e - al * W4, a = a0 + al;
        float g[2][3]; int ix6[2][3];
#pragma unroll
        for (int r = 0; r < 2; ++r)
#pragma unroll
            for (int q = 0; q < 3; ++q) {
                const bool in = (a + r) <= ho_hi && (2 * b + q) < p.Wo;
                const int li = (al + r) * p.Wo + 2 * b + q;
                g[r][q] = in ? gs[li] : 0.f;
                ix6[r][q] = in ? (int)is[li] : 255;
            }
        float o[2][4];
#pragma unroll
        for (int rp = 0; rp < 2; ++rp)
#pragma unroll
            for (int u = 0; u < 4; ++u) {
                float acc = 0.f;
#pragma unroll
                for (int wr = 0; wr < (rp ? 2 : 1); ++wr) {
                    const int kr = rp ? (wr ? 0 : 2) : 1;
#pragma unroll
                    for (int wc = 0; wc < ((u & 1) ? 2 : 1); ++wc) {
                        const int q = (u >> 1) + ((u & 1) ? wc : 0) + ((u == 2) ? 0 : 0);
                        const int ks = (u & 1) ? (wc ? 0 : 2) : 1;
                        if (ix6[wr][q] == kr * 3 + ks) acc += g[wr][q];
                    }
                }
                o[rp][u] = acc;
            }
        float* row = gx + (int64_t)(2 * a) * p.Ws + 4 * b;
        *reinterpret_cast<float4*>(row) = make_float4(o[0][0], o[0][1], o[0][2], o[0][3]);
        *reinterpret_cast<float4*>(row + p.Ws) = make_float4(o[1][0], o[1][1], o[1][2], o[1][3]);
    }
}

__global__ void avgpool_fwd_kernel(const I2VPoolParams p) {
    const int64_t total = (int64_t)p.N * p.C * p.Ho * p.Wo;
    const float inv = 1.f / (float)(p.k * p.k);
    for (int64_t idx = blockIdx.x * (int64_t)blockDim.x + threadIdx.x; idx < total; idx += (int64_t)gridDim.x * blockDim.x) {
        const int wo = idx % p.Wo; int64_t r = idx / p.Wo;
        const int ho = r % p.Ho; r /= p.Ho;
        const int c = r % p.C; const int64_t n = r / p.C;
        const float* pl = p.x + n * p.x_nstride + (int64_t)c * p.Hs * p.Ws;
        float s = 0.f;
        for (int kr = 0; kr < p.k; ++kr)
            for (int ks = 0; ks < p.k; ++ks) s += pl[(ho * p.stride + kr) * p.Ws + wo * p.stride + ks];
        p.y[n * p.y_nstride + ((int64_t)c * p.Ho + ho) * p.Wo + wo] = s * inv;
    }
}

__global__ void avgpool_bwd_kernel(const I2VPoolParams p) {
    const int64_t total = (int64_t)p.N * p.C * p.Hs * p.Ws;
    const float inv = 1.f / (float)(p.k * p.k);
    for (int64_t idx = blockIdx.x * (int64_t)blockDim.x + threadIdx.x; idx < total; idx += (int64_t)gridDim.x * blockDim.x) {
        const int w = idx % p.Ws; int64_t r = idx / p.Ws;
        const int h = r % p.Hs; r /= p.Hs;
        const int c = r % p.C; const int64_t n = r / p.C;
        const int ho = h / p.stride, wo = w / p.stride;
        const bool in = (h - ho * p.stride) < p.k && (w - wo * p.stride) < p.k && ho < p.Ho && wo < p.Wo;
        p.gx[n * p.gx_nstride + ((int64_t)c * p.Hs + h) * p.Ws + w] =
            in ? p.y[n * p.y_nstride + ((int64_t)c * p.Ho + ho) * p.Wo + wo] * inv : 0.f;
    }
}

static unsigned stream_grid(int64_t total, int per_block) {
    int64_t b = (total + per_block - 1) / per_block;
    if (b < 1) b = 1;
    if (b > 256 * 16) b = 256 * 16;
    return (unsigned)b;
}

static int pool_fail(const char* m) { snprintf(g_be_err, sizeof g_be_err, "%s", m); g_be_has_err = true; return 1; }

int k_pool_fwd(const I2VPoolParams& p, i2v_stream_t s) {
    if (POOL_FWD_LDS_FLOATS / p.Ws < p.k) return pool_fail("max-pool row too wide for the LDS band");
    int band = (POOL_FWD_LDS_FLOATS / p.Ws - p.k) / p.stride + 1;
    if (band < 1) return pool_fail("max-pool row too wide for the LDS band");
    if (band > p.Ho) band = p.Ho;
    dim3 grid((unsigned)(p.N * p.C), (unsigned)((p.Ho + band - 1) / band));
    hipLaunchKernelGGL(pool_fwd_kernel, grid, dim3(256), 0, (hipStream_t)s, p, band);
    LAUNCH_CHECK("pool_fwd"); return 0;
}
int k_pool_bwd(const I2VPoolParams& p, i2v_stream_t s) {
    int out_rows = (POOL_LDS_FLOATS / 2) / p.Wo;
    if (out_rows < 1) return pool_fail("max-pool row too wide for the LDS band");
    int band = (out_rows - 1) * p.stride - p.k + 1; if (out_rows >= p.Ho) band = p.Hs;
    if (band < 1) return pool_fail("max-pool row too wide for the LDS band");
    if (band > p.Hs) band = p.Hs;
    dim3 grid((unsigned)(p.N * p.C), (unsigned)((p.Hs + band - 1) / band));
    if (p.k == 3 && p.stride == 2 && p.pad == 1 && (p.yact || !p.mask_relu) && (p.Ws & 3) == 0 && (p.Hs & 1) == 0 && p.Ho * 2 == p.Hs && p.Wo * 2 == p.Ws &&
        (((uintptr_t)p.gx | (uintptr_t)(p.gx_nstride * 4)) & 15) == 0) {
        int pairs = (POOL_LDS_FLOATS / 2) / p.Wo - 1;
        if (pairs < 1) return pool_fail("max-pool row too wide for the LDS band");
        if (pairs > p.Hs / 2) pairs = p.Hs / 2;
        uint32_t m, sh; fastdiv_magic((unsigned)(p.Ws >> 2), &m, &sh);
        dim3 g2((unsigned)(p.N * p.C), (unsigned)((p.Hs / 2 + pairs - 1) / pairs));
        hipLaunchKernelGGL(pool_bwd_321_kernel, g2, dim3(256), 0, (hipStream_t)s, p, pairs, m, sh);
    } else if (p.k == 3 && p.stride == 2 && p.pad == 1) hipLaunchKernelGGL((pool_bwd_kernel<3, 2, 1>), grid, dim3(256), 0, (hipStream_t)s, p, band);
    else if (p.k == 2 && p.stride == 2 && p.pad == 0) hipLaunchKernelGGL((pool_bwd_kernel<2, 2, 0>), grid, dim3(256), 0, (hipStream_t)s, p, band);
    else if (p.k == 3 && p.stride == 2 && p.pad == 0) hipLaunchKernelGGL((pool_bwd_kernel<3, 2, 0>), grid, dim3(256), 0, (hipStream_t)s, p, band);
    else hipLaunchKernelGGL((pool_bwd_kernel<0, 0, 0>), grid, dim3(256), 0, (hipStream_t)s, p, band);
    LAUNCH_CHECK("pool_bwd"); return 0;
}

__global__ void pool3d_fwd_kernel(const I2VPoolParams p) {
    const int64_t total = (int64_t)p.N * p.C * p.Ho * p.Wo;
    for (int64_t idx = blockIdx.x * (int64_t)blockDim.x + threadIdx.x; idx < total; idx += (int64_t)gridDim.x * blockDim.x) {
        const int wo = idx % p.Wo; int64_t r = idx / p.Wo;
        const int ho = r % p.Ho; r /= p.Ho;
        const int c = r % p.C; const int64_t n = r / p.C;
        const int64_t clip = n / p.To; const int to = (int)(n - clip * p.To);
        int best = -1; float bv = 0.f;
        for (int q = 0; q < p.kt; ++q) {
            const int ts = to * p.stride_t - p.pad_t + q; if (ts < 0 || ts >= p.Ts) continue;
            const float* pl = p.x + (clip * p.Ts + ts) * p.x_nstride + (int64_t)c * p.Hs * p.Ws;
            for (int kr = 0; kr < p.k; ++kr) {
                const int h = ho * p.stride - p.pad + kr; if (h < 0 || h >= p.Hs) continue;
                for (int ks = 0; ks < p.k; ++ks) {
                    const int w = wo * p.stride - p.pad + ks; if (w < 0 || w >= p.Ws) continue;
                    const float v = pl[h * p.Ws + w];
                    if (best < 0 || v > bv || v != v) { bv = v; best = (q * p.k + kr) * p.k + ks; }
                }
            }
        }
        p.y[n * p.y_nstride + ((int64_t)c * p.Ho + ho) * p.Wo + wo] = bv;
        p.idx[idx] = (uint8_t)best;
    }
}

__global__ void pool3d_bwd_kernel(const I2VPoolParams p) {
    const int64_t clips = p.N / p.To, total = clips * p.Ts * p.C * p.Hs * p.Ws;
    for (int64_t idx = blockIdx.x * (int64_t)blockDim.x + threadIdx.x; idx < total; idx += (int64_t)gridDim.x * blockDim.x) {
        const int w = idx % p.Ws; int64_t r = idx / p.Ws;
        const int h = r % p.Hs; r /= p.Hs;
        const int c = r % p.C; const int64_t ns = r / p.C;
        const int64_t clip = ns / p.Ts; const int ts = (int)(ns - clip * p.Ts);
        const int64_t xo = ns * p.x_nstride + ((int64_t)c * p.Hs + h) * p.Ws + w;
        float g = 0.f;
        if (!p.mask_relu || p.x[xo] > 0.f) {
            int t_lo = ts + p.pad_t - p.kt + 1; t_lo = t_lo <= 0 ? 0 : (t_lo + p.stride_t - 1) / p.stride_t;
            const int t_hi = min((ts + p.pad_t) / p.stride_t, p.To - 1);
            int a_lo = h + p.pad - p.k + 1; a_lo = a_lo <= 0 ? 0 : (a_lo + p.stride - 1) / p.stride;
            const int a_hi = min((h + p.pad) / p.stride, p.Ho - 1);
            int b_lo = w + p.pad - p.k + 1; b_lo = b_lo <= 0 ? 0 : (b_lo + p.stride - 1) / p.stride;
            const int b_hi = min((w + p.pad) / p.stride, p.Wo - 1);
            for (int to = t_lo; to <= t_hi; ++to)
                for (int ho = a_lo; ho <= a_hi; ++ho)
                    for (int wo = b_lo; wo <= b_hi; ++wo) {
                        const int me = ((ts - (to * p.stride_t - p.pad_t)) * p.k + (h - (ho * p.stride - p.pad))) * p.k +
                                       (w - (wo * p.stride - p.pad));
                        const int64_t no = clip * p.To + to;
                        if (p.idx[((no * p.C + c) * p.Ho + ho) * p.Wo + wo] == me)
                            g += p.y[no * p.y_nstride + ((int64_t)c * p.Ho + ho) * p.Wo + wo];
                    }
        }
        p.gx[ns * p.gx_nstride + ((int64_t)c * p.Hs + h) * p.Ws + w] = g;
    }
}

int k_pool3d_fwd(const I2VPoolParams& p, i2v_stream_t s) {
    if (p.kt * p.k * p.k > 256) return pool_fail("video max-pool window larger than 256 taps");
    hipLaunchKernelGGL(pool3d_fwd_kernel, dim3(stream_grid((int64_t)p.N * p.C * p.Ho * p.Wo, 256)), dim3(256), 0, (hipStream_t)s, p);
    LAUNCH_CHECK("pool3d_fwd"); return 0;
}
int k_pool3d_bwd(const I2VPoolParams& p, i2v_stream_t s) {
    hipLaunchKernelGGL(pool3d_bwd_kernel, dim3(stream_grid((int64_t)(p.N / p.To) * p.Ts * p.C * p.Hs * p.Ws, 256)), dim3(256), 0, (hipStream_t)s, p);
    LAUNCH_CHECK("pool3d_bwd"); return 0;
}

int k_avgpool_fwd(const I2VPoolParams& p, i2v_stream_t s) {
    hipLaunchKernelGGL(avgpool_fwd_kernel, dim3(stream_grid((int64_t)p.N * p.C * p.Ho * p.Wo, 256)), dim3(256), 0, (hipStream_t)s, p);
    LAUNCH_CHECK("avgpool_fwd"); return 0;
}
int k_avgpool_bwd(const I2VPoolParams& p, i2v_stream_t s) {
    hipLaunchKernelGGL(avgpool_bwd_kernel, dim3(stream_grid((int64_t)p.N * p.C * p.Hs * p.Ws, 256)), dim3(256), 0, (hipStream_t)s, p);
    LAUNCH_CHECK("avgpool_bwd"); return 0;
}

__global__ void addmask_kernel(const I2VAddMaskParams p) {
    const int64_t plane = (int64_t)p.C * p.HW, total = plane * p.N;
    for (int64_t idx = blockIdx.x * (int64_t)blockDim.x + threadIdx.x; idx < total; idx += (int64_t)gridDim.x * blockDim.x) {
        const int64_t n = idx / plane, i = idx - n * plane;
        float v = 0.f;
        if (p.a[0]) v += p.a[0][n * p.a_nstride[0] + i];
        if (p.a[1]) v += p.a[1][n * p.a_nstride[1] + i];
        if (p.a[2]) v += p.a[2][n * p.a_nstride[2] + i];
        if (p.gate) {
            const int64_t c = i / p.HW, bit = n * p.HW + (i - c * p.HW);
            if (!((p.gate[c * p.gate_stride + (bit >> 5)] >> (bit & 31)) & 1u)) v = 0.f;
        } else if (p.mask && !(p.mask[n * p.mask_nstride + i] > 0.f)) v = 0.f;
        if (p.gain != 0.f) v = __fmul_rn(p.gain, v);
// ... 922 lines not shown
```

### image-to-video-i2v-attack_amd/csrc/i2v_net.h

```cpp
#pragma once
#include "../../include/i2v_hip.h"
#include "i2v_kernels.h"

#include <stdint.h>

#include <deque>
#include <mutex>
#include <string>
#include <vector>

namespace eng {

#pragma GCC visibility push(hidden)
extern thread_local std::string g_err;
int fail(const char* fmt, ...);
#pragma GCC visibility pop

#define CHECK_BE(expr)                                                            \
    do {                                                                          \
        if ((expr) != 0) return fail("%s: %s", #expr, be_error() ? be_error() : "backend error"); \
    } while (0)

struct Buffer { int C, H, W; int T = 1; size_t act_off = 0, grad_off = 0; bool is_input = false;
                size_t gate_off = 0; int gate_words = 0; bool gated = false; };
struct Tensor { int buf, c_off, C; bool post_relu; float bwd_gain = 1.f; };

struct Packed {
    float* wp = nullptr; I2VKEntry* ktab = nullptr;
    float* wpc = nullptr;
    uint16_t* wp3 = nullptr;
    int K = 0, Kpad = 0, Cd = 0, Cdpad = 0, tap_uniform = 0;
    int halo = 0;
    int ph = 0, pw = 0, Hg = 0, Wg = 0;
    int pt = 0, Tg = 1;
    int has_dt = 0;
    int quad = 0, quad_kw = 0, quad_dw0 = 0;
    int tpair = 0;
    int ig_tt = 0, ig_th = 0, ig_tw = 0;
    int ig_p77 = 0;
};

struct Node {
    int type;
    i2v_attn_desc ad{};
    size_t p_off = 0;
    int src0() const { return type == 0 ? cd.src : type == 3 ? ad.theta : pd.src; }
    int dst0() const { return type == 0 ? cd.dst : type == 3 ? ad.dst : pd.dst; }
    i2v_conv3d_desc cd; i2v_pool3d_desc pd;
    std::vector<float> w;
    std::vector<float> shift;
    std::vector<float> pre_scale, pre_shift;
    float* shift_d = nullptr; float* pre_scale_d = nullptr; float* pre_shift_d = nullptr;
    bool preact() const { return !pre_scale.empty(); }
    Packed fwd; std::vector<Packed> bwd;
    int groups = 1; std::vector<float> wg; bool gconv = false;
    float* gw_fwd = nullptr; float* gw_bwd = nullptr; int gw_tapmask[4] = {0, 0, 0, 0};
    struct ImgGrad {
        Packed P; int blk = 0, sh = 1, blkt = 1;
        int ost = 1, ot0 = 0;
        int st = 1, oct = 1; bool skips = false;
        double flop_share = 1.0;
    };
    std::vector<ImgGrad> imgs;
    size_t idx_off = 0;
};

enum Kind { L_CONV, L_IMGGRAD, L_POOLF, L_POOLB, L_ADDMASK, L_AVGF, L_AVGB, L_MEMSET, L_POOL3F, L_POOL3B, L_AGEMM, L_SOFTMAX, L_GCONV };
struct Launch {
    Kind kind;
    I2VConvParams conv; I2VPoolParams pool; I2VAddMaskParams am; I2VGConvParams gc;
    I2VAttnGemm ag; I2VSoftmaxRows sm; int sm_rows_per_clip = 0;
    int T = 1;
    bool src_is_input = false;
    bool img_accumulate = false;
    float* ms_ptr = nullptr; size_t ms_floats_per_frame = 0;
    bool ms_gx = false;
    double alg_flops_per_frame = 0;
    int cfg_b[4] = {0, 0, 0, 0};
    int fuse_ok = 0;
    int fuse_b[4] = {0, 0, 0, 0};
    int node = -1;
    int fb_ok = 0;
    int fb_b[4] = {0, 0, 0, 0};
    int ov_after = -2, ov_join = -1;
};
inline int cfg_bucket(int clips, int max_clips) {
    int b = 0;
    while (b < 3 && (max_clips >> (b + 1)) >= clips && (max_clips >> (b + 1)) >= 1) ++b;
    return b;
}

struct Addend { const float* p; int64_t nstride; int stride, H, W; };

struct Net {
    std::vector<Buffer> bufs; std::vector<Tensor> tens; std::vector<Node> nodes;
    int input = -1; std::vector<int> hooks; int maxN = 0; bool planned = false;
    float* arena = nullptr; size_t arena_floats = 0; std::vector<void*> dev_allocs;
    std::vector<Launch> fwd, bwd;
    int frames = 0;
    int Tin() const { return bufs[tens[input].buf].T; }
    size_t weight_bytes = 0;
    std::vector<float*> hook_tmp;
    size_t in_stage_off = 0; bool stage_input = false;
    i2v_stream_t side = nullptr; std::vector<void*> ov_ev; size_t ov_used = 0;
    std::vector<std::vector<int>> ov_at[2]; int ov_max_frames = 0;
};

struct TimedLaunch { void* start; void* stop; int kind; double flops; int Cd, K, HWg, frames, pw; void* chain_from; double bytes; int count = 1; };

}

struct i2v_ctx {
    int device; std::vector<eng::Net*> nets; std::mutex nets_mu;
    int timing = 0;
    std::deque<eng::TimedLaunch> timed; size_t timed_used = 0; std::mutex timing_mu;
};

namespace eng {
#pragma GCC visibility push(hidden)

inline size_t align_up(size_t v, size_t a) { return (v + a - 1) / a * a; }

inline Net* get_net(i2v_handle h, int id) {
    if (!h || id < 0 || id >= (int)h->nets.size() || !h->nets[id]) { fail("bad net id %d", id); return nullptr; }
    return h->nets[id];
}

template <typename T>
int upload(Net& n, const std::vector<T>& host, T** dev) {
    size_t bytes = host.size() * sizeof(T);
    void* d = be_malloc(bytes ? bytes : 16);
    if (!d) return fail("device allocation of %zu bytes failed", bytes);
    n.dev_allocs.push_back(d);
    n.weight_bytes += bytes;
    if (bytes) CHECK_BE(be_h2d(d, host.data(), bytes));
    *dev = (T*)d;
    return 0;
}

bool math_bf16x3();
int pack_fwd(Net& n, Node& nd);
int pack_bwd(Net& n, Node& nd);
int pack_img(Net& n, Node& nd);
bool gconv_enabled();
int pack_gconv(Net& n, Node& nd);

struct View { float* p; int64_t nstride; int C, H, W; int T = 1; };
View view_of(Net& n, int t, bool grad);
bool plan_pass(Net& n, bool dry, size_t off, size_t N, size_t* end, std::string* err);

void mark_fusable(Net& n);
void mark_overlap(Net& n);
int autotune(Net& n);

I2VConvParams conv_prep(const Launch& l, const float* x, float* gx, int accumulate);
int conv_run(const Launch& l, int frames, const float* x, float* gx, int accumulate, i2v_stream_t s);
bool fused_fits(const Launch& a, const Launch& b, int frames);
int fused_run(const Launch& a, const Launch& b, int frames, const float* x, int halo, i2v_stream_t s);
int fast_run(const std::vector<Launch>& L, size_t li, int frames, const float* x, i2v_stream_t s);
extern long long g_overlap_launches;

#pragma GCC visibility pop
}
```

### image-to-video-i2v-attack_amd/csrc/i2v_params.h

```cpp
#pragma once
#include <stddef.h>
#include <stdint.h>

#define I2V_KC 16

struct I2VKEntry {
    int32_t chan_off;
    int32_t dh, dw;
    int32_t valid;
};

struct I2VConvParams {
    const float* src;  int64_t src_nstride;  int32_t Hs, Ws;
    int32_t Cs;
    int32_t src_span_bytes;
    const float* wp;   const I2VKEntry* ktab; int32_t K, Kpad, Cd, Cdpad;
    int32_t N, Hg, Wg, sh, sw;
    float* dst;        int64_t dst_nstride;  int32_t Ho, Wo, osh, osw, oh0, ow0;
    const float* shift;
    const float* add0; int64_t add0_nstride; int32_t add0_stride, add0_H, add0_W;
    const float* add1; int64_t add1_nstride;
    const float* mask; int64_t mask_nstride;
    uint32_t* gate_out; int32_t gate_out_stride; int32_t gate_out_pix0;
    const uint32_t* gate; int32_t gate_stride; int32_t gate_pix0;
    const float* pre_scale; const float* pre_shift;
    const float* gate_scale; const float* gate_shift;
    int32_t relu;
    int32_t pointwise;
    int32_t tap_uniform;
    int32_t blk;
    int32_t blkt;
    int32_t Tg, Ts, To, st, ost, ot0;
    int32_t oct;
    int32_t temporal;
    int32_t vec_epilogue;
    int32_t quad, quad_kw, quad_dw0;
    int32_t halo;
    int32_t ig_tt, ig_th, ig_tw;
    int32_t ig_p77;
    const float* wpc;
    uint32_t dv_hw_m, dv_hw_s, dv_w_m, dv_w_s, dv_t_m, dv_t_s, dv_wo_m, dv_wo_s;
    const void* wp3; int32_t bf3;
    int32_t cfg;
};

struct I2VFastStage {
    const float* wp; const I2VKEntry* ktab; int32_t Kpad, Cdpad;
    const float* shift; int32_t relu;
    const uint32_t* gate; int32_t gate_stride, gate_pix0;
    uint32_t* gate_out; int32_t gate_out_stride, gate_out_pix0;
};
struct I2VFastBlockParams {
    int32_t mode, CM;
    const float* src; int64_t src_nstride; int32_t Cs;
    int32_t N, T, H, W, R;
    I2VFastStage a, b, c, d;
    const float* add0; int64_t add0_nstride;
    float* dst; int64_t dst_nstride;
    uint32_t dv_w_m, dv_w_s, dv_hw_m, dv_hw_s;
    int32_t U, S, G, BU;
    uint32_t dv_bu_m, dv_bu_s, dv_s_m, dv_s_s, dv_g_m, dv_g_s;
    int32_t delay;
};

struct I2VGConvClass { int32_t Hg, Wg, oh0, ow0, tapmask; uint32_t dv_w_m, dv_w_s, dv_hw_m, dv_hw_s; };
struct I2VGConvParams {
    const float* src; int64_t src_nstride; int32_t Hs, Ws;
    const float* w;
    int32_t groups, gw, N, S, ncls;
    I2VGConvClass cls[4];
    float* dst; int64_t dst_nstride; int32_t Ho, Wo, os;
    const float* shift; int32_t relu;
    uint32_t* gate_out; int32_t gate_out_stride;
    const uint32_t* gate; int32_t gate_stride;
    const float* mask; int64_t mask_nstride;
    int32_t waves, rows, lds_bytes;
    uint32_t dv_r_m, dv_r_s;
};

struct I2VPoolParams {
    const float* x;    int64_t x_nstride;    int32_t C, Hs, Ws;
    float* y;          int64_t y_nstride;    int32_t Ho, Wo;
    float* gx;         int64_t gx_nstride;
    const float* yact; int64_t yact_nstride;
    uint8_t* idx;
    int32_t N, k, stride, pad, mask_relu;
    int32_t kt, stride_t, pad_t, Ts, To;
};

struct I2VAddMaskParams {
    float* out;        int64_t out_nstride;
    const float* a[3]; int64_t a_nstride[3];
    const float* mask; int64_t mask_nstride;
    const uint32_t* gate; int32_t gate_stride;
    int32_t N, C, HW;
    float gain;
};

struct I2VCosParams {
    const float* a;    int64_t a_nstride;
    const float* b;    int64_t b_nstride;
    int64_t D;         int32_t N;
    float* partial;    int32_t nblk;
    float* cos_out;
    float* grad;       int64_t grad_nstride;
    const float* coef_dev; int32_t coef_index; float coef_host;
    int32_t mask_relu, accumulate;
};

struct I2VIlafParams {
    const float* a;    int64_t a_nstride;
    const float* ori;  const float* adv0;
    int64_t D;         int32_t N;
    double* partial;   int32_t nblk;
    double* sums;
    double init_norm;
    float* loss_out;
    float* grad;       int64_t grad_nstride;
    int32_t mask_relu, accumulate;
    int32_t fps;
    const double* init_sq;
    int32_t mode; double coef;
};

struct I2VActMat { const float* p; int64_t nstride; int32_t T, HW; };
struct I2VAttnGemm {
    int32_t form, clips, Cc, M, N;
    I2VActMat A, B;
    float* Cact; int64_t C_nstride; int32_t C_T, C_HW;
    float* D; const float* Din;
    float scale; int32_t accumulate;
    int32_t ksplit; float* part;
};
#ifdef __HIPCC__
__host__ __device__
#endif
inline int attn_kseg(int K, int ksplit) { return ksplit <= 1 ? K : ((K + ksplit - 1) / ksplit + 31) / 32 * 32; }
struct I2VSoftmaxRows { float* X; const float* P; int64_t rows; int32_t N; int32_t mode; };

struct I2VHeadParams {
    const float* a;    int64_t a_nstride;
    int32_t C, HW, T, clips, K;
    const float* W;    const float* bias;
    const int32_t* labels;
    float scale;
    float* pooled;
    float* dpooled;
    float* logits;
    float* loss_each;
    float* grad;       int64_t grad_nstride;
    int32_t mask_relu, accumulate;
    int32_t Ctot, c_off;
    int32_t phase;
};

struct I2VStdParams {
    const float* a;    int64_t a_nstride; int64_t D; int32_t N;
    double* partial;   int32_t nblk;
    double* sums;
    double total_count;
    float* std_out;
    float* grad;       int64_t grad_nstride;
    int32_t mask_relu, accumulate;
};
```

### image-to-video-i2v-attack_amd/csrc/i2v_run.cpp

```cpp
#include "i2v_net.h"

#include <stdio.h>
#include <stdlib.h>

#include <algorithm>

using namespace eng;

namespace eng {

I2VConvParams conv_prep(const Launch& l, const float* x, float* gx, int accumulate) {
    I2VConvParams p = l.conv;
    if (l.src_is_input) p.src = x;
    if (l.kind == L_IMGGRAD) { p.dst = gx; if (accumulate || l.img_accumulate) { p.add1 = gx; p.add1_nstride = p.dst_nstride; } }
    p.vec_epilogue = (p.blk <= 1 && p.osh == 1 && p.osw == 1 && p.oh0 == 0 && p.ow0 == 0 && p.Hg == p.Ho &&
                      p.Wg == p.Wo && p.Tg == p.To && p.ost == 1 && p.ot0 == 0 &&
                      (p.Ho * p.Wo) % 4 == 0 && p.dst_nstride % 4 == 0 &&
                      (p.add0_stride == 1 || (p.add0_stride == 2 && p.Wo % 4 == 0 && p.add0_W * 2 == p.Wo &&
                                              p.add0_W % 2 == 0 && (p.add0_H * p.add0_W) % 2 == 0)) &&
                      p.add0_nstride % 4 == 0 && p.add1_nstride % 4 == 0 && p.mask_nstride % 4 == 0 &&
                      (((uintptr_t)p.dst | (uintptr_t)p.add0 | (uintptr_t)p.add1 | (uintptr_t)p.mask) & 15) == 0)
                         ? 1 : 0;
    if (!(p.Tg == p.Ts && p.Ts == p.To && p.st == 1 && p.ost == 1 && p.ot0 == 0 && p.blkt == 1)) p.temporal = 1;
    return p;
}

bool fused_fits(const Launch& a, const Launch& b, int frames) {
    for (const Launch* l : {&a, &b}) {
        const I2VConvParams& p = l->conv;
        const int64_t span = ((int64_t)frames * p.Ts / p.Tg - 1) * p.src_nstride * 4 + (int64_t)p.Cs * p.Hs * p.Ws * 4;
        if (span >= (1ll << 31)) return false;
    }
    return true;
}
int fused_run(const Launch& a, const Launch& b, int frames, const float* x, int halo, i2v_stream_t s) {
    I2VConvParams pa = conv_prep(a, x, nullptr, 0), pb = conv_prep(b, x, nullptr, 0);
    for (I2VConvParams* p : {&pa, &pb}) {
        p->N = frames;
        p->src_span_bytes = (int32_t)(((int64_t)frames * p->Ts / p->Tg - 1) * p->src_nstride * 4 + (int64_t)p->Cs * p->Hs * p->Ws * 4);
    }
    CHECK_BE(k_conv_fused(pa, pb, halo, s));
    return 0;
}

int fast_run(const std::vector<Launch>& L, size_t li, int frames, const float* x, i2v_stream_t s) {
    const int g = L[li].fb_ok;
    I2VConvParams q[4];
    for (int j = 0; j < g; ++j) { q[j] = conv_prep(L[li + j], x, nullptr, 0); q[j].N = frames; }
    const I2VConvParams* c = g == 3 ? &q[2] : g == 4 ? &q[3] : nullptr;
    const I2VConvParams* d = g == 4 ? &q[2] : nullptr;
    if (i2v_fastblock_rows(q[0], q[1], c, d) <= 0) return 2;
    if (k_fastblock(q[0], q[1], c, d, s)) { fail("k_fastblock: %s", be_error() ? be_error() : "backend error"); return 1; }
    return 0;
}

int conv_run(const Launch& l, int frames, const float* x, float* gx, int accumulate, i2v_stream_t s) {
    I2VConvParams p = conv_prep(l, x, gx, accumulate);
    const int clips = frames / p.Tg;
    const int64_t plane_bytes = (int64_t)p.Cs * p.Hs * p.Ws * 4, stride_bytes = p.src_nstride * 4;
    const int64_t clip_bytes = (int64_t)(p.Ts - 1) * stride_bytes + plane_bytes;
    int64_t per = clip_bytes >= (1ll << 31) ? 0 : 1 + ((1ll << 31) - 1 - clip_bytes) / (stride_bytes * p.Ts);
    if (per < 1) return fail("one clip of a convolution input exceeds 2 GiB");
    if (per < clips && (p.gate || p.gate_out)) {
        per -= per % 32;
        if (per < 1) return fail("a sliced convolution launch cannot keep its gate rows word-aligned");
    }
    for (int c0 = 0; c0 < clips; c0 += (int)per) {
        I2VConvParams q = p;
        const int nc = clips - c0 < per ? clips - c0 : (int)per;
        q.N = nc * p.Tg;
        q.src += (int64_t)c0 * p.Ts * p.src_nstride; q.dst += (int64_t)c0 * p.To * p.dst_nstride;
        if (q.add0) q.add0 += (int64_t)c0 * p.To * p.add0_nstride;
        if (q.add1) q.add1 += (int64_t)c0 * p.To * p.add1_nstride;
        if (q.mask) q.mask += (int64_t)c0 * p.To * p.mask_nstride;
        q.gate_pix0 = p.gate_pix0 + (int32_t)((int64_t)c0 * p.To * p.Ho * p.Wo);
        q.gate_out_pix0 = p.gate_out_pix0 + (int32_t)((int64_t)c0 * p.To * p.Ho * p.Wo);
        q.src_span_bytes = (int32_t)((int64_t)(nc * p.Ts - 1) * stride_bytes + plane_bytes);
        CHECK_BE(k_conv(q, s));
    }
    return 0;
}

}

long long eng::g_overlap_launches = 0;

static TimedLaunch* timing_begin(i2v_ctx* h, int kind, double flops, i2v_stream_t s, TimedLaunch* prev) {
    if (!h->timing) return nullptr;
    TimedLaunch* t;
    {
        std::lock_guard<std::mutex> lock(h->timing_mu);
        if (h->timed_used == h->timed.size()) {
            TimedLaunch fresh{be_event_create(), be_event_create(), 0, 0.0, 0, 0, 0, 0, 0, nullptr, 0.0, 1};
            if (!fresh.start || !fresh.stop) return nullptr;
            h->timed.push_back(fresh);
        }
        t = &h->timed[h->timed_used++];
    }
    t->kind = kind; t->flops = flops; t->Cd = t->K = t->HWg = t->frames = t->pw = 0; t->bytes = 0.0; t->count = 1;
    t->chain_from = prev ? prev->stop : nullptr;
    if (!t->chain_from) be_event_record(t->start, s);
    return t;
}

static double launch_flops(const std::vector<Launch>& L, size_t li, int fb, int fuse, int frames, int clips) {
    const Launch& l = L[li];
    double flops = 0.0;
    if (fb) { for (int j = 0; j < fb; ++j) { const Launch& m = L[li + j]; flops += m.alg_flops_per_frame > 0 ? m.alg_flops_per_frame * frames : 2.0 * frames * m.conv.Hg * m.conv.Wg * (double)m.conv.Cd * m.conv.K; } }
    else if ((l.kind == L_CONV || l.kind == L_GCONV) && l.alg_flops_per_frame > 0) flops = l.alg_flops_per_frame * frames;
    else if (l.kind == L_CONV) flops = 2.0 * frames * l.conv.Hg * l.conv.Wg * ((double)l.conv.Cd * l.conv.K + (fuse ? (double)L[li + 1].conv.Cd * L[li + 1].conv.K : 0.0));
    else if (l.kind == L_IMGGRAD) flops = l.alg_flops_per_frame * frames;
    else if (l.kind == L_AGEMM) flops = 2.0 * clips * (double)l.ag.Cc * l.ag.M * l.ag.N;
    return flops;
}

static int launch_timing_kind(const Launch& l, bool backward_pass) {
    switch (l.kind) {
        case L_CONV: case L_AGEMM: case L_GCONV: return backward_pass ? 5 : 0;
        case L_IMGGRAD: return 1;
        case L_POOLF: case L_AVGF: case L_POOL3F: return 2;
        case L_POOLB: case L_AVGB: case L_POOL3B: return 3;
        case L_ADDMASK: case L_MEMSET: case L_SOFTMAX: return 4;
    }
    return 4;
}

static double launch_bytes(const std::vector<Launch>& L, size_t li, int fb, int fuse, int frames, int clips, int accumulate) {
    const Launch& l = L[li];
    const I2VConvParams& q = l.conv;
    const double out = (double)frames * q.Hg * q.Wg * q.Cd;
    const double src = (double)clips * q.Ts * q.Cs * q.Hs * q.Ws;
    double b = 4.0 * (src + (double)q.K * q.Cd + out);
    if (q.add0) b += 4.0 * out / (q.add0_stride * q.add0_stride);
    if (q.add1 || l.kind == L_IMGGRAD) b += (q.add1 || accumulate || l.img_accumulate) ? 4.0 * out : 0.0;
    if (q.mask) b += 4.0 * out;
    if (q.gate) b += out / 8.0;
    if (q.gate_out) b += out / 8.0;
    if (fb) {
        const I2VConvParams& last = L[li + fb - 1].conv;
        const double outl = (double)frames * last.Hg * last.Wg * last.Cd;
        b = 4.0 * (src + outl);
        for (int j = 0; j < fb; ++j) {
            const I2VConvParams& r = L[li + j].conv;
            const double o = (double)frames * r.Hg * r.Wg * r.Cd;
            b += 4.0 * (double)r.K * r.Cd + (r.gate ? o / 8.0 : 0.0) + (r.gate_out ? o / 8.0 : 0.0);
        }
        if (fb == 3) b += 4.0 * outl;
    }
    if (fuse) {
        const I2VConvParams& r = L[li + 1].conv;
        const double out2 = (double)frames * r.Hg * r.Wg * r.Cd;
        b += 4.0 * ((double)r.K * r.Cd + out2) - 4.0 * out;
        if (r.add0) b += 4.0 * out2;
        if (r.add1) b += 4.0 * out2;
        if (r.mask) b += 4.0 * out2;
        if (r.gate) b += out2 / 8.0;
        if (r.gate_out) b += out2 / 8.0;
    }
    return b;
}

namespace {

struct ListTiming {
    i2v_ctx* h; i2v_stream_t s; bool backward_pass;
    TimedLaunch* prev = nullptr;
    TimedLaunch* seg = nullptr;

    TimedLaunch* open(const std::vector<Launch>& L, size_t li, int fb, int fuse, int frames, int clips, int accumulate) {
        const Launch& l = L[li];
        const int kind = launch_timing_kind(l, backward_pass);
        const double flops = launch_flops(L, li, fb, fuse, frames, clips);
        const bool conv = l.kind == L_CONV || l.kind == L_IMGGRAD || l.kind == L_GCONV;
        if (h->timing == 2) {
            if (!seg || seg->kind != kind) {
                close();
                seg = timing_begin(h, kind, 0.0, s, seg);
                if (seg) seg->count = 0;
            }
            if (seg) { seg->flops += flops; seg->count += 1; if (conv) seg->bytes += launch_bytes(L, li, fb, fuse, frames, clips, accumulate); }
            return prev = nullptr;
        }
        TimedLaunch* const tl = prev = timing_begin(h, kind, flops, s, prev);
        if (tl && conv) {
            tl->Cd = l.conv.Cd; tl->K = l.conv.K; tl->HWg = l.conv.Hg * l.conv.Wg; tl->frames = frames; tl->pw = l.conv.pointwise;
            tl->bytes = launch_bytes(L, li, fb, fuse, frames, clips, accumulate);
        }
        if (tl && l.kind == L_AGEMM) {
            const I2VAttnGemm& q = l.ag;
            tl->Cd = q.Cc; tl->K = q.form == 1 ? q.Cc : (q.form == 2 ? q.N : q.M); tl->HWg = q.form == 2 ? q.M : q.N; tl->frames = frames; tl->pw = 10 + q.form;
            tl->bytes = 4.0 * clips * ((double)q.M * q.N + (double)q.Cc * q.M + (double)q.Cc * q.N);
        }
        return tl;
    }
    void close() { if (seg) be_event_record(seg->stop, s); }
};

struct SideStream {
    Net& n; std::vector<Launch>& L; const std::vector<std::vector<int>>& at; i2v_stream_t main;
    int clips; const float* x; float* gx; int accumulate;
    struct Pending { int join; void* done; };
    std::vector<Pending> pending;

    void* event() {
        if (n.ov_used == n.ov_ev.size()) { void* e = be_event_create(); if (!e) return nullptr; n.ov_ev.push_back(e); }
        return n.ov_ev[n.ov_used++];
    }
    int issue(int p) {
        for (int i : at[p + 1]) {
            void* ready = event(); void* done = event();
            if (!ready || !done) return fail("launch overlap: event creation failed");
            CHECK_BE(be_event_record(ready, main)); CHECK_BE(be_stream_wait_event(n.side, ready));
            Launch& m = L[i];
            const int fr = clips * m.T;
            if (fr * m.conv.Hg * m.conv.Wg != 0) {
                const int cb = m.cfg_b[cfg_bucket(clips, n.maxN / n.Tin())];
                if (cb) m.conv.cfg = cb;
                if (conv_run(m, fr, x, gx, accumulate, n.side)) return 1;
                __atomic_fetch_add(&g_overlap_launches, 1, __ATOMIC_RELAXED);
            }
            CHECK_BE(be_event_record(done, n.side));
            pending.push_back(Pending{m.ov_join, done});
        }
        return 0;
    }
    int join(int upto) {
        for (size_t i = 0; i < pending.size();) {
            if (pending[i].join <= upto) { CHECK_BE(be_stream_wait_event(main, pending[i].done)); pending[i] = pending.back(); pending.pop_back(); }
            else ++i;
        }
        return 0;
    }
};

}

static int run_list(i2v_ctx* h, Net& n, std::vector<Launch>& L, int in_frames, const float* x, float* gx, int accumulate,
                    i2v_stream_t s, bool backward_pass) {
    const int clips = in_frames / n.Tin();
    const int bucket = cfg_bucket(clips, n.maxN / n.Tin());
    ListTiming timing{h, s, backward_pass};
    SideStream side{n, L, n.ov_at[backward_pass ? 1 : 0], s, clips, x, gx, accumulate};
    const bool overlap = !h->timing && n.side && !side.at.empty() && in_frames <= n.ov_max_frames;
    if (overlap) n.ov_used = 0;
    if (overlap && side.issue(-1)) return 1;
    for (size_t li = 0; li < L.size(); ++li) {
        Launch& l = L[li];
        const int frames = clips * l.T;
        const size_t li0 = li;
        if (overlap && l.ov_after != -2) continue;
        const int fuse = (l.kind == L_CONV && l.fuse_ok && li + 1 < L.size() && frames * l.conv.Hg * l.conv.Wg > 0 && fused_fits(l, L[li + 1], frames))
                             ? l.fuse_b[bucket] : 0;
        const int fb = (l.kind == L_CONV && l.fb_ok && li + l.fb_ok <= L.size() && frames * l.conv.Hg * l.conv.Wg > 0) ? l.fb_b[bucket] * l.fb_ok : 0;
        if (overlap && side.join((int)li + (fb ? fb - 1 : fuse ? 1 : 0))) return 1;
        TimedLaunch* const tl = h->timing ? timing.open(L, li, fb, fuse, frames, clips, accumulate) : nullptr;
        struct Stop { TimedLaunch* t; i2v_stream_t s; ~Stop() { if (t) be_event_record(t->stop, s); } } stop{tl, s};
        switch (l.kind) {
            case L_CONV:
            case L_IMGGRAD: {
                if (frames * l.conv.Hg * l.conv.Wg == 0) break;
                if (fuse) { if (fused_run(l, L[li + 1], frames, x, fuse == 2, s)) return 1; ++li; break; }
                if (fb) {
                    const int rc = fast_run(L, li, frames, x, s);
                    if (rc == 1) return 1;
                    if (rc == 0) { li += fb - 1; break; }
                }
                const int cb = l.cfg_b[bucket];
                if (cb) l.conv.cfg = cb;
                if (conv_run(l, frames, x, gx, accumulate, s)) return 1;
            } break;
            case L_GCONV: {
#ifdef I2V_HAVE_GCONV
                I2VGConvParams p = l.gc; p.N = frames; CHECK_BE(k_gconv(p, s));
#else
                return fail("this build has no grouped-convolution kernel");
#endif
            } break;
            case L_POOLF: { I2VPoolParams p = l.pool; p.N = frames; CHECK_BE(k_pool_fwd(p, s)); } break;
            case L_POOL3F: {
                I2VPoolParams p = l.pool; p.N = frames;
                if (p.kt == 1 && p.pad_t == 0 && p.Ts == p.stride_t * p.To) { p.x_nstride *= p.stride_t; CHECK_BE(k_pool_fwd(p, s)); }
                else CHECK_BE(k_pool3d_fwd(p, s));
            } break;
            case L_POOL3B: {
                I2VPoolParams p = l.pool; p.N = frames;
                if (p.kt == 1 && p.pad_t == 0 && p.Ts == p.stride_t * p.To && p.gx_nstride == (int64_t)p.C * p.Hs * p.Ws) {
                    CHECK_BE(be_memset0(p.gx, (size_t)frames * p.stride_t * p.gx_nstride * sizeof(float), s));
                    p.x_nstride *= p.stride_t; p.gx_nstride *= p.stride_t;
                    CHECK_BE(k_pool_bwd(p, s));
                } else CHECK_BE(k_pool3d_bwd(p, s));
            } break;
            case L_AVGF: { I2VPoolParams p = l.pool; p.N = frames; CHECK_BE(k_avgpool_fwd(p, s)); } break;
            case L_AVGB: { I2VPoolParams p = l.pool; p.N = frames; CHECK_BE(k_avgpool_bwd(p, s)); } break;
            case L_MEMSET:
                if (!l.ms_gx) CHECK_BE(be_memset0(l.ms_ptr, l.ms_floats_per_frame * frames * sizeof(float), s));
                else if (!accumulate) CHECK_BE(be_memset0(gx, l.ms_floats_per_frame * frames * sizeof(float), s));
                break;
            case L_POOLB: { I2VPoolParams p = l.pool; p.N = frames; CHECK_BE(k_pool_bwd(p, s)); } break;
            case L_ADDMASK: { I2VAddMaskParams p = l.am; p.N = frames; CHECK_BE(k_addmask(p, s)); } break;
            case L_AGEMM: { I2VAttnGemm p = l.ag; p.clips = clips; CHECK_BE(k_attn_gemm(p, s)); } break;
            case L_SOFTMAX: { I2VSoftmaxRows p = l.sm; p.rows = (int64_t)clips * l.sm_rows_per_clip; CHECK_BE(k_softmax_rows(p, s)); } break;
        }
        if (overlap) for (size_t p = li0; p <= li; ++p) if (side.issue((int)p)) return 1;
    }
    if (overlap && side.join((int)L.size())) return 1;
    timing.close();
    return 0;
}

extern "C" int i2v_net_forward(i2v_handle h, int net, const float* x, int frames, void* stream) {
    Net* n = get_net(h, net); if (!n) return 1;
    if (!n->planned) return fail("net not planned");
    if (frames <= 0 || frames > n->maxN) return fail("frames=%d outside 1..%d", frames, n->maxN);
    if (frames % n->Tin()) return fail("frames=%d is not a multiple of the input's %d frames per clip", frames, n->Tin());
    if (!x) return fail("null input");
    n->frames = frames;
    if (n->stage_input) {
        static const bool always = [] { const char* e = getenv("I2V_STAGE_COPY"); return e && e[0] == '1'; }();
        bool need = always || ((uintptr_t)x & 15) != 0;
        const int bucket = cfg_bucket(frames / n->Tin(), n->maxN / n->Tin());
        for (const Launch& l : n->fwd)
            if (l.kind == L_CONV && l.src_is_input && l.conv.quad && !(l.cfg_b[bucket] > 0 && ((l.cfg_b[bucket] - 1) & 1024))) need = true;
        if (need) {
            const Buffer& ib = n->bufs[n->tens[n->input].buf];
            const size_t bytes = (size_t)frames * ib.C * ib.H * ib.W * sizeof(float);
            float* staged = n->arena + n->in_stage_off;
            CHECK_BE(be_d2d_2d(staged, bytes, x, bytes, bytes, 1, stream));
            x = staged;
        }
    }
    return run_list(h, *n, n->fwd, frames, x, nullptr, 0, stream, false);
}

extern "C" int i2v_net_backward(i2v_handle h, int net, float* gx, int accumulate, void* stream) {
    Net* n = get_net(h, net); if (!n) return 1;
    if (!n->planned || n->frames <= 0) return fail("backward before forward");
    if (!gx) return fail("null gradient output");
    return run_list(h, *n, n->bwd, n->frames, nullptr, gx, accumulate, stream, true);
}

extern "C" int i2v_timing_enable(i2v_handle h, int enable) {
    if (!h) return fail("null handle");
    h->timing = enable == 2 ? 2 : (enable != 0 ? 1 : 0); h->timed_used = 0;
    return 0;
}

#define I2V_TIMING_FIELDS 8
extern "C" int i2v_timing_collect_ex(i2v_handle h, double* out, int n_kinds, int n_fields) {
    if (!h || !out || n_kinds < 6 || n_fields < I2V_TIMING_FIELDS) return fail("i2v_timing_collect_ex: bad argument");
    for (int i = 0; i < n_kinds * n_fields; ++i) out[i] = 0.0;
    if (h->timed_used) CHECK_BE(be_device_sync());
    const char* dump_path = getenv("I2V_TIMING_DUMP");
    FILE* dump = dump_path ? fopen(dump_path, "a") : nullptr;
    for (size_t i = 0; i < h->timed_used; ++i) {
        const TimedLaunch& t = h->timed[i];
        float ms = 0.f;
        CHECK_BE(be_event_elapsed_ms(t.chain_from ? t.chain_from : t.start, t.stop, &ms));
        if (dump && h->timing != 2) fprintf(dump, "%d %d %d %d %d %d %.4f %.3f %.3f\n", t.kind, t.Cd, t.K, t.HWg, t.frames, t.pw, ms, t.flops * 1e-9, t.bytes * 1e-6);
        if (t.kind < 0 || t.kind >= n_kinds) continue;
        double* o = out + (size_t)t.kind * n_fields;
        o[0] += ms; o[1] += t.flops; o[2] += t.count; o[3] += t.bytes;
        if (h->timing != 2 && t.bytes > 0 && t.flops < 19.7 * t.bytes) { o[4] += ms; o[5] += t.bytes; o[6] += 1; o[7] += t.flops; }
    }
    if (dump) fclose(dump);
    h->timed_used = 0;
    return 0;
}

extern "C" int i2v_timing_collect(i2v_handle h, double* ms_by_kind, double* flops_by_kind, int64_t* launches_by_kind,
                                  int n_kinds) {
    if (!h || !ms_by_kind || !flops_by_kind || !launches_by_kind || n_kinds < 6 || n_kinds > 16) return fail("i2v_timing_collect: bad argument");
    double tmp[16 * I2V_TIMING_FIELDS];
    if (i2v_timing_collect_ex(h, tmp, n_kinds, I2V_TIMING_FIELDS)) return 1;
    for (int i = 0; i < n_kinds; ++i) {
        ms_by_kind[i] = tmp[i * I2V_TIMING_FIELDS]; flops_by_kind[i] = tmp[i * I2V_TIMING_FIELDS + 1];
        launches_by_kind[i] = (int64_t)tmp[i * I2V_TIMING_FIELDS + 2];
    }
    return 0;
}

extern "C" int i2v_net_hook_info(i2v_handle h, int net, int hook, float** act, int64_t* act_stride,
                                 float** grad, int64_t* grad_stride, int64_t* D, int32_t* post_relu) {
    Net* n = get_net(h, net); if (!n) return 1;
    if (!n->planned) return fail("net not planned");
    if (hook < 0 || hook >= (int)n->hooks.size()) return fail("bad hook index");
    int t = n->hooks[hook];
    View a = view_of(*n, t, false), g = view_of(*n, t, true);
    int64_t d = (int64_t)a.C * a.H * a.W;
    if (act) *act = a.p;
    if (act_stride) *act_stride = a.nstride;
    if (grad_stride) *grad_stride = n->hook_tmp[hook] ? d : g.nstride;
    if (grad) *grad = n->hook_tmp[hook] ? n->hook_tmp[hook] : g.p;
    if (D) *D = d;
    if (post_relu) *post_relu = n->tens[t].post_relu ? 1 : 0;
    return 0;
}

extern "C" int i2v_net_read_tensor(i2v_handle h, int net, int tensor, int which, float* out, int frames,
                                   void* stream) {
    Net* n = get_net(h, net); if (!n) return 1;
    if (!n->planned) return fail("net not planned");
    if (tensor < 0 || tensor >= (int)n->tens.size() || tensor == n->input) return fail("bad tensor id");
    View v = view_of(*n, tensor, which != 0);
    if (frames <= 0 || frames > n->maxN / n->Tin() * v.T) return fail("bad frame count");
    for (const std::vector<Launch>* L : {&n->fwd, &n->bwd})
        for (const Launch& l : *L) {
            if (l.kind != L_CONV || !l.fuse_ok || !(l.fuse_b[0] | l.fuse_b[1] | l.fuse_b[2] | l.fuse_b[3])) continue;
            const float* lo = l.conv.dst; const float* hi = lo + (int64_t)(n->maxN / n->Tin() * std::max(1, l.conv.To) - 1) * l.conv.dst_nstride + (int64_t)l.conv.Cd * l.conv.Ho * l.conv.Wo;
            const float* vlo = v.p; const float* vhi = v.p + (int64_t)(frames - 1) * v.nstride + (int64_t)v.C * v.H * v.W;
            if (vlo < hi && lo < vhi)
                return fail("i2v_net_read_tensor: this tensor is the intermediate of a fused 3x3 -> pointwise pair and is never stored "
                            "(plan without I2V_FUSE / I2V_FORCE_FUSE to read it)");
        }
    for (const std::vector<Launch>* L : {&n->fwd, &n->bwd})
        for (size_t i = 0; i < L->size(); ++i) {
            const Launch& l = (*L)[i];
            if (l.kind != L_CONV || !l.fb_ok || !(l.fb_b[0] | l.fb_b[1] | l.fb_b[2] | l.fb_b[3])) continue;
            for (int j = 0; j + 1 < l.fb_ok && i + j < L->size(); ++j) {
                const I2VConvParams& q = (*L)[i + j].conv;
                const float* lo = q.dst; const float* hi = lo + (int64_t)(n->maxN / n->Tin() * std::max(1, q.To) - 1) * q.dst_nstride + (int64_t)q.Cd * q.Ho * q.Wo;
                const float* vlo = v.p; const float* vhi = v.p + (int64_t)(frames - 1) * v.nstride + (int64_t)v.C * v.H * v.W;
                if (vlo < hi && lo < vhi)
                    return fail("i2v_net_read_tensor: this tensor is an intermediate of a fused fast-pathway block and is never stored "
                                "(plan with I2V_FASTBLOCK=0 to read it)");
            }
        }
    size_t row = (size_t)v.C * v.H * v.W * sizeof(float);
    CHECK_BE(be_d2d_2d(out, row, v.p, (size_t)v.nstride * sizeof(float), row, frames, stream));
    return 0;
}
```

### image-to-video-i2v-attack_amd/csrc/i2v_tune.cpp

```cpp
#include "i2v_net.h"

#include <stdio.h>
#include <stdlib.h>
#include <string.h>

#include <algorithm>

namespace eng {

void mark_fusable(Net& n) {
    const int64_t frames = n.maxN, clips = n.maxN / n.Tin();
    typedef std::pair<const float*, const float*> Range;
    auto rng = [](const void* q, int64_t fr, int64_t ns, int64_t plane) {
        const float* f = (const float*)q;
        return f ? Range(f, f + (fr > 0 ? (fr - 1) * ns : 0) + std::max<int64_t>(plane, 1)) : Range(nullptr, nullptr);
    };
    auto meet = [](const Range& a, const Range& b) { return a.first && b.first && a.first < b.second && b.first < a.second; };
    auto touches = [&](const Launch& c, const Range& w, bool skip_src, bool skip_dst) {
        if (c.kind == L_CONV || c.kind == L_IMGGRAD || c.kind == L_GCONV) {
            const I2VConvParams& q = c.conv;
            const int64_t fs = clips * std::max(1, q.Ts), fo = clips * std::max(1, q.To), dplane = (int64_t)(q.blk > 1 ? q.Cd / (q.blk * q.blk) : q.Cd) * q.Ho * q.Wo;
            return (!skip_src && meet(w, rng(q.src, fs, q.src_nstride, (int64_t)q.Cs * q.Hs * q.Ws))) ||
                   meet(w, rng(q.add0, fo, q.add0_nstride, dplane)) || meet(w, rng(q.add1, fo, q.add1_nstride, dplane)) ||
                   meet(w, rng(q.mask, fo, q.mask_nstride, dplane)) || (!skip_dst && meet(w, rng(q.dst, fo, q.dst_nstride, dplane)));
        }
        if (c.kind == L_ADDMASK) {
            const int64_t fr = clips * std::max(1, c.T), pl = (int64_t)c.am.C * c.am.HW;
            return meet(w, rng(c.am.out, fr, c.am.out_nstride, pl)) || meet(w, rng(c.am.a[0], fr, c.am.a_nstride[0], pl)) ||
                   meet(w, rng(c.am.a[1], fr, c.am.a_nstride[1], pl)) || meet(w, rng(c.am.a[2], fr, c.am.a_nstride[2], pl)) ||
                   meet(w, rng(c.am.mask, fr, c.am.mask_nstride, pl));
        }
        if (c.kind == L_MEMSET) return meet(w, rng(c.ms_ptr, 1, 0, (int64_t)c.ms_floats_per_frame * clips * std::max(1, c.T)));
        if (c.kind == L_AGEMM || c.kind == L_SOFTMAX) return true;
        const I2VPoolParams& q = c.pool;
        const int64_t fr = clips * std::max(std::max(1, c.T), std::max(q.Ts, q.To)), pin = (int64_t)q.C * q.Hs * q.Ws, pout = (int64_t)q.C * q.Ho * q.Wo;
        return meet(w, rng(q.x, fr, q.x_nstride, pin)) || meet(w, rng(q.gx, fr, q.gx_nstride, pin)) || meet(w, rng(q.y, fr, q.y_nstride, pout)) ||
               meet(w, rng(q.yact, fr, q.yact_nstride, pout));
    };
    std::vector<Range> hooked;
    for (size_t h = 0; h < n.hooks.size(); ++h) {
        View a = view_of(n, n.hooks[h], false), g = view_of(n, n.hooks[h], true);
        hooked.push_back(rng(a.p, frames, a.nstride, (int64_t)a.C * a.H * a.W));
        hooked.push_back(rng(g.p, frames, g.nstride, (int64_t)g.C * g.H * g.W));
    }
    auto dst_of = [&](const Launch& l) {
        return rng(l.conv.dst, clips * std::max(1, l.conv.To), l.conv.dst_nstride, (int64_t)l.conv.Cd * l.conv.Ho * l.conv.Wo);
    };
    for (std::vector<Launch>* L : {&n.fwd, &n.bwd})
        for (size_t i = 0; i + 2 < L->size(); ++i) {
            Launch& a = (*L)[i]; Launch& c = (*L)[i + 1]; Launch& b = (*L)[i + 2];
            if (a.kind != L_CONV || c.kind != L_CONV || b.kind != L_CONV || a.src_is_input || c.src_is_input || !k_conv_fusable(a.conv, b.conv)) continue;
            if (k_conv_fusable(a.conv, c.conv)) continue;
            const I2VConvParams& pa = a.conv; const I2VConvParams& pc = c.conv;
            const bool dep = touches(c, dst_of(a), false, false) || touches(a, dst_of(c), false, false) ||
                             (pa.gate_out && (pa.gate_out == pc.gate || pa.gate_out == pc.gate_out)) || (pc.gate_out && pc.gate_out == pa.gate);
            if (!dep) std::swap(a, c);
        }
    for (std::vector<Launch>* L : {&n.fwd, &n.bwd})
        for (size_t i = 0; i + 1 < L->size(); ++i) {
            Launch& a = (*L)[i]; Launch& b = (*L)[i + 1];
            a.fuse_ok = 0;
            if (a.kind != L_CONV || b.kind != L_CONV || a.src_is_input || b.src_is_input || a.T != b.T) continue;
            const int ok = k_conv_fusable(a.conv, b.conv);
            if (!ok) continue;
            const Range w = dst_of(a);
            bool other = false;
            for (auto& hk : hooked) other |= meet(hk, w);
            for (std::vector<Launch>* M : {&n.fwd, &n.bwd})
                for (size_t j = 0; j < M->size() && !other; ++j)
                    other |= touches((*M)[j], w, M == L && j == i + 1, M == L && j == i);
            if (!other) a.fuse_ok = ok;
            if (getenv("I2V_FUSE_DEBUG"))
                fprintf(stderr, "[i2v fuse] %s pair %zu: 3x3 Cd=%d K=%d %dx%d -> 1x1 Cd=%d K=%d: eligible=%d other_reader=%d\n", L == &n.fwd ? "fwd" : "bwd", i,
                        a.conv.Cd, a.conv.K, a.conv.Hg, a.conv.Wg, b.conv.Cd, b.conv.K, ok, (int)other);
        }
    {
        const bool fb_off = [] { const char* e = getenv("I2V_FASTBLOCK"); return e && e[0] == '0'; }();
        auto cd_of = [&](const Launch& l) -> const i2v_conv3d_desc* { return (l.kind == L_CONV && l.node >= 0 && n.nodes[l.node].type == 0 && !n.nodes[l.node].preact()) ? &n.nodes[l.node].cd : nullptr; };
        auto unit = [](const i2v_conv3d_desc& c) { return c.stride == 1 && c.stride_t == 1 && c.dil_t == 1; };
        auto is_pw = [&](const i2v_conv3d_desc& c) { return unit(c) && c.kt == 1 && c.kh == 1 && c.kw == 1 && c.pad == 0 && c.pad_t == 0; };
        auto is_t = [&](const i2v_conv3d_desc& c) { return unit(c) && c.kh == 1 && c.kw == 1 && c.pad == 0 && (c.kt & 1) && 2 * c.pad_t == c.kt - 1; };
        auto is_33 = [&](const i2v_conv3d_desc& c) { return unit(c) && c.kt == 1 && c.kh == 3 && c.kw == 3 && c.pad == 1 && c.pad_t == 0; };
        auto private_to = [&](std::vector<Launch>* L, size_t first, size_t last, const Launch& w) {
            const Range r = dst_of(w);
            for (auto& hk : hooked) if (meet(hk, r)) return false;
            for (std::vector<Launch>* M : {&n.fwd, &n.bwd})
                for (size_t j = 0; j < M->size(); ++j) {
                    if (M == L && j >= first && j <= last) continue;
                    if (touches((*M)[j], r, false, false)) return false;
                }
            return true;
        };
        for (Launch& l : n.fwd) l.fb_ok = 0;
        for (Launch& l : n.bwd) l.fb_ok = 0;
        for (size_t i = 0; !fb_off && i + 2 < n.bwd.size(); ++i) {
            Launch& a = n.bwd[i]; Launch& x = n.bwd[i + 1]; Launch& b = n.bwd[i + 2];
            const i2v_conv3d_desc* ca = cd_of(a); const i2v_conv3d_desc* cb = cd_of(b);
            if (!ca || !cb || !is_pw(*ca) || !is_33(*cb) || b.conv.src != a.conv.dst || x.kind != L_CONV) continue;
            const I2VConvParams& px = x.conv;
            const bool dep = touches(x, dst_of(a), false, false) || touches(a, dst_of(x), false, false) || touches(x, dst_of(b), false, false) || touches(b, dst_of(x), false, false) ||
                             (px.gate_out && (px.gate_out == a.conv.gate || px.gate_out == b.conv.gate));
            if (!dep) { Launch t = x; n.bwd[i + 1] = n.bwd[i]; n.bwd[i] = t; }
        }
        for (size_t i = 0; !fb_off && i + 1 < n.bwd.size(); ++i) {
            Launch& a = n.bwd[i]; Launch& b = n.bwd[i + 1];
            const i2v_conv3d_desc* ca = cd_of(a); const i2v_conv3d_desc* cb = cd_of(b);
            if (!ca || !cb || !is_pw(*ca) || !is_33(*cb) || a.T != b.T || b.conv.src != a.conv.dst) continue;
            if (i2v_fastblock_rows(a.conv, b.conv, nullptr, nullptr) <= 0) continue;
            if (!private_to(&n.bwd, i, i + 1, a)) continue;
            a.fb_ok = 2;
        }
        for (size_t i = 0; !fb_off && i + 2 < n.fwd.size(); ++i) {
            Launch& a = n.fwd[i]; Launch& b = n.fwd[i + 1];
            const i2v_conv3d_desc* ca = cd_of(a); const i2v_conv3d_desc* cb = cd_of(b);
            if (!ca || !cb || a.src_is_input || !(is_t(*ca) || is_pw(*ca)) || !is_33(*cb) || !ca->relu || !cb->relu || ca->residual >= 0 || cb->residual >= 0 || cb->src != ca->dst) continue;
            Launch& c3 = n.fwd[i + 2];
            const i2v_conv3d_desc* cc = cd_of(c3);
            if (!cc || !is_pw(*cc)) continue;
            if (cc->src == cb->dst && cc->residual >= 0 && cc->relu && a.T == b.T && a.T == c3.T) {
                if (i2v_fastblock_rows(a.conv, b.conv, &c3.conv, nullptr) <= 0) continue;
                if (!private_to(&n.fwd, i, i + 2, a) || !private_to(&n.fwd, i, i + 2, b)) continue;
                a.fb_ok = 3;
            } else if (i + 3 < n.fwd.size() && cc->src == ca->src && !cc->relu && cc->residual < 0) {
                Launch& c4 = n.fwd[i + 3];
                const i2v_conv3d_desc* c4d = cd_of(c4);
                if (!c4d || !is_pw(*c4d) || c4d->src != cb->dst || c4d->residual != cc->dst || !c4d->relu || a.T != b.T || a.T != c3.T || a.T != c4.T) continue;
                if (i2v_fastblock_rows(a.conv, b.conv, &c4.conv, &c3.conv) <= 0) continue;
                if (!private_to(&n.fwd, i, i + 3, a) || !private_to(&n.fwd, i, i + 3, b) || !private_to(&n.fwd, i, i + 3, c3)) continue;
                a.fb_ok = 4;
            }
        }
        const bool fb_force = [] { const char* e = getenv("I2V_FORCE_FASTBLOCK"); return e && e[0] == '1'; }();
        for (std::vector<Launch>* L : {&n.fwd, &n.bwd})
            for (Launch& a : *L)
                for (int bk = 0; bk < 4; ++bk) a.fb_b[bk] = (a.fb_ok && fb_force) ? 1 : 0;
        if (getenv("I2V_FUSE_DEBUG"))
            for (std::vector<Launch>* L : {&n.fwd, &n.bwd})
                for (size_t i = 0; i < L->size(); ++i)
                    if ((*L)[i].fb_ok) fprintf(stderr, "[i2v fastblock] %s launch %zu: group of %d (Cs %d -> %d mid channels, %dx%d)\n", L == &n.fwd ? "fwd" : "bwd", i, (*L)[i].fb_ok,
                                               (*L)[i].conv.Cs, (*L)[i].conv.Cd, (*L)[i].conv.Hg, (*L)[i].conv.Wg);
    }
    const char* force = getenv("I2V_FORCE_FUSE");
    const int f = force ? atoi(force) : 0;
    for (std::vector<Launch>* L : {&n.fwd, &n.bwd})
        for (Launch& a : *L)
            for (int b = 0; b < 4; ++b) a.fuse_b[b] = (a.fuse_ok && f) ? ((f == 2 && (a.fuse_ok & 2)) ? 2 : 1) : 0;
}

void mark_overlap(Net& n) {
    for (int k = 0; k < 2; ++k) n.ov_at[k].clear();
    for (std::vector<Launch>* L : {&n.fwd, &n.bwd}) for (Launch& l : *L) { l.ov_after = -2; l.ov_join = -1; }
    const char* e = getenv("I2V_OVERLAP_MAX_FRAMES");
    n.ov_max_frames = e ? atoi(e) : 0;
    if (n.ov_max_frames <= 0) return;
    const int64_t clips = n.maxN / n.Tin();
    typedef std::pair<const char*, const char*> Range;
    struct RW { std::vector<Range> r, w; bool barrier = false; };
    static const char gx_tag[16] = {0};
    const Range GX(gx_tag, gx_tag + 16);
    auto rng = [](const void* q, int64_t fr, int64_t stride_bytes, int64_t plane_bytes) {
        const char* f = (const char*)q;
        return f ? Range(f, f + (fr > 0 ? (fr - 1) * stride_bytes : 0) + std::max<int64_t>(plane_bytes, 1)) : Range(nullptr, nullptr);
    };
    auto rw_of = [&](const Launch& c) {
        RW o;
        auto rd = [&](const Range& x) { if (x.first) o.r.push_back(x); };
        auto wr = [&](const Range& x) { if (x.first) o.w.push_back(x); };
        if (c.kind == L_CONV || c.kind == L_IMGGRAD || c.kind == L_GCONV) {
            const I2VConvParams& q = c.conv;
            const int64_t fs = clips * std::max(1, q.Ts), fo = clips * std::max(1, q.To);
            const int64_t dplane = 4ll * (q.blk > 1 ? q.Cd / (q.blk * q.blk) : q.Cd) * q.Ho * q.Wo;
            if (!c.src_is_input) rd(rng(q.src, fs, 4 * q.src_nstride, 4ll * q.Cs * q.Hs * q.Ws));
            rd(rng(q.add0, fo, 4 * q.add0_nstride, dplane)); rd(rng(q.add1, fo, 4 * q.add1_nstride, dplane)); rd(rng(q.mask, fo, 4 * q.mask_nstride, dplane));
            rd(rng(q.gate, 1, 0, 4ll * q.Cd * q.gate_stride)); wr(rng(q.gate_out, 1, 0, 4ll * q.Cd * q.gate_out_stride));
            if (c.kind == L_IMGGRAD) { wr(GX); rd(GX); } else wr(rng(q.dst, fo, 4 * q.dst_nstride, dplane));
        } else if (c.kind == L_ADDMASK) {
            const int64_t fr = clips * std::max(1, c.T), pl = 4ll * c.am.C * c.am.HW;
            wr(rng(c.am.out, fr, 4 * c.am.out_nstride, pl));
            for (int i = 0; i < 3; ++i) rd(rng(c.am.a[i], fr, 4 * c.am.a_nstride[i], pl));
            rd(rng(c.am.mask, fr, 4 * c.am.mask_nstride, pl)); rd(rng(c.am.gate, 1, 0, 4ll * c.am.C * c.am.gate_stride));
        } else if (c.kind == L_MEMSET) {
            if (c.ms_gx) wr(GX); else wr(rng(c.ms_ptr, 1, 0, 4ll * (int64_t)c.ms_floats_per_frame * clips * std::max(1, c.T)));
        } else if (c.kind == L_AGEMM || c.kind == L_SOFTMAX) {
            o.barrier = true;
        } else {
            const I2VPoolParams& q = c.pool;
            const int64_t fr = clips * std::max(std::max(1, c.T), std::max(q.Ts, q.To)), pin = 4ll * q.C * q.Hs * q.Ws, pout = 4ll * q.C * q.Ho * q.Wo;
            const Range idx = rng(q.idx, 1, 0, fr * (int64_t)q.C * q.Ho * q.Wo);
            const bool fwd = c.kind == L_POOLF || c.kind == L_POOL3F || c.kind == L_AVGF;
            if (fwd) { rd(rng(q.x, fr, 4 * q.x_nstride, pin)); wr(rng(q.y, fr, 4 * q.y_nstride, pout)); wr(idx); }
            else { rd(rng(q.x, fr, 4 * q.x_nstride, pin)); rd(rng(q.y, fr, 4 * q.y_nstride, pout)); rd(rng(q.yact, fr, 4 * q.yact_nstride, pout)); rd(idx);
                   wr(rng(q.gx, fr * std::max(1, q.stride_t), 4 * q.gx_nstride, pin)); }
        }
        return o;
    };
    auto meet = [](const std::vector<Range>& A, const std::vector<Range>& B) {
        for (const Range& a : A) for (const Range& b : B) if (a.first < b.second && b.first < a.second) return true;
        return false;
    };
    auto conflict = [&](const RW& a, const RW& b) { return a.barrier || b.barrier || meet(a.r, b.w) || meet(a.w, b.w) || meet(a.w, b.r); };
    int k = 0;
    for (std::vector<Launch>* L : {&n.fwd, &n.bwd}) {
        const int M = (int)L->size();
        std::vector<RW> rw; rw.reserve(M);
        for (const Launch& l : *L) rw.push_back(rw_of(l));
        std::vector<char> member(M, 0);
        for (int i = 0; i < M; ++i) {
            const Launch& l = (*L)[i];
            for (int j = 0; j < l.fb_ok && i + j < M; ++j) member[i + j] = 1;
            if (l.fuse_ok) { member[i] = 1; if (i + 1 < M) member[i + 1] = 1; }
        }
        n.ov_at[k].assign(M + 1, {});
        int hoisted = 0;
        for (int i = 1; i < M; ++i) {
            Launch& l = (*L)[i];
            if (l.kind != L_CONV || member[i] || l.src_is_input) continue;
            int dep = -1;
            for (int j = i - 1; j >= 0; --j) if (conflict(rw[i], rw[j])) { dep = j; break; }
            if (dep >= i - 1) continue;
            if (dep >= 0 && (*L)[dep].ov_after != -2) continue;
            int join = M;
            for (int j = i + 1; j < M; ++j) if (conflict(rw[j], rw[i])) { join = j; break; }
            l.ov_after = dep; l.ov_join = join;
            n.ov_at[k][dep + 1].push_back(i);
            ++hoisted;
            if (getenv("I2V_FUSE_DEBUG"))
                fprintf(stderr, "[i2v overlap] %s launch %d (Cd %d, K %d, %dx%d): side stream after launch %d, joined before launch %d of %d\n", k ? "bwd" : "fwd", i,
                        l.conv.Cd, l.conv.K, l.conv.Hg, l.conv.Wg, dep, join, M);
        }
        if (!hoisted) n.ov_at[k].clear();
        ++k;
    }
    if (n.ov_at[0].empty() && n.ov_at[1].empty()) return;
    n.side = be_stream_create();
    if (!n.side) { n.ov_at[0].clear(); n.ov_at[1].clear(); }
}

namespace {

struct Probe {
    float* scratch = nullptr; void* e0 = nullptr; void* e1 = nullptr;
    const float* x = nullptr; float* gx = nullptr;

    int init(Net& n) {
        const Buffer& ib = n.bufs[n.tens[n.input].buf];
        const size_t img = (size_t)n.maxN * ib.C * ib.H * ib.W;
        scratch = (float*)be_malloc(2 * img * sizeof(float));
        if (!scratch) return fail("autotune scratch allocation failed");
        CHECK_BE(be_memset0(scratch, 2 * img * sizeof(float), nullptr));
        e0 = be_event_create(); e1 = be_event_create();
        x = n.stage_input ? n.arena + n.in_stage_off : scratch;
        gx = scratch + img;
        return 0;
    }
    ~Probe() { if (e0) be_event_destroy(e0); if (e1) be_event_destroy(e1); if (scratch) be_free(scratch); }

    template <class F>
    int time(F&& fn, int reps, float* ms_per_run, bool warm_up = true) {
        if (warm_up && fn()) return 1;
        be_event_record(e0, nullptr);
        for (int r = 0; r < reps; ++r) if (fn()) return 1;
        be_event_record(e1, nullptr);
        if (be_stream_sync(nullptr)) return 1;
        float ms = 0.f; be_event_elapsed_ms(e0, e1, &ms);
        *ms_per_run = ms / reps;
        return 0;
    }
};

template <class F>
int for_each_bucket(int max_clips, int Tg, F&& fn) {
    for (int b = 3; b >= 0; --b) {
        const int clips_b = max_clips >> b;
        if (clips_b < 1 || (b > 0 && clips_b == (max_clips >> (b - 1)))) continue;
        if (const int rc = fn(b, clips_b * Tg)) return rc;
    }
    return 0;
}

const char* list_name(const Net& n, const std::vector<Launch>* L) { return L == &n.fwd ? "fwd" : "bwd"; }

int tune_tiles(Net& n, Probe& pr, int max_clips) {
    for (std::vector<Launch>* L : {&n.fwd, &n.bwd})
        for (Launch& l : *L) {
            if (l.kind != L_CONV && l.kind != L_IMGGRAD) continue;
            const int planned_cfg = l.conv.cfg;
            const int reps = l.kind == L_IMGGRAD ? 4 : 2;
            const int rc = for_each_bucket(max_clips, l.conv.Tg, [&](int b, int lf) -> int {
                if (lf * l.conv.Hg * l.conv.Wg == 0) return 0;
                int cand[16]; I2VConvParams probe = l.conv; probe.N = lf;
                probe.temporal = conv_prep(l, pr.x, pr.gx, 0).temporal;
                const int nc = k_conv_candidates(probe, cand);
                if (nc <= 1) { if (nc == 1) l.cfg_b[b] = cand[0] + 1; return 0; }
                auto time_cfg = [&](int cfg_plus_1, float* per_launch) {
                    l.conv.cfg = cfg_plus_1;
                    return pr.time([&] { return conv_run(l, lf, pr.x, pr.gx, 0, nullptr); }, reps, per_launch);
                };
                float best = 1e30f; int best_c = -1;
                for (int ci = 0; ci < nc; ++ci) {
                    float ms = 0.f;
                    if (time_cfg(cand[ci] + 1, &ms)) return 1;
                    if ((cand[ci] & 2048) && getenv("I2V_FUSE_DEBUG"))
                        fprintf(stderr, "[i2v vfma] %s launch Cd %d K %d (%dx%d) at %d frames: conv_vfma %.1f us, best tile so far %.1f us\n", list_name(n, L),
                                l.conv.Cd, l.conv.K, l.conv.Hg, l.conv.Wg, lf, 1e3f * ms, 1e3f * best);
                    if (ms < best) { best = ms; best_c = cand[ci]; }
                }
                static const bool no_nt = [] { const char* e = getenv("I2V_NT"); return e && e[0] == '0'; }();
                if (best_c >= 0 && l.kind == L_CONV && !no_nt) {
                    float ms = 0.f;
                    if (time_cfg((best_c | 128) + 1, &ms)) return 1;
                    if (ms < 0.98f * best) { best = ms; best_c |= 128; }
                }
                l.cfg_b[b] = best_c >= 0 ? best_c + 1 : 0;
                return 0;
            });
            l.conv.cfg = l.cfg_b[0] ? l.cfg_b[0] : planned_cfg;
            if (rc) return 1;
        }
    return 0;
}

int tune_fastblocks(Net& n, Probe& pr, int max_clips) {
    const bool fb_force = [] { const char* e = getenv("I2V_FORCE_FASTBLOCK"); return e && e[0] == '1'; }();
    for (std::vector<Launch>* L : {&n.fwd, &n.bwd})
        for (size_t i = 0; i < L->size(); ++i) {
            Launch& a = (*L)[i];
            if (!a.fb_ok || i + a.fb_ok > L->size()) continue;
            for (int bk = 0; bk < 4; ++bk) a.fb_b[bk] = 0;
            const int rc = for_each_bucket(max_clips, a.conv.Tg, [&](int bk, int lf) -> int {
                auto run_sep = [&]() { for (int j = 0; j < a.fb_ok; ++j) { Launch& m = (*L)[i + j]; if (m.cfg_b[bk]) m.conv.cfg = m.cfg_b[bk]; if (conv_run(m, lf, pr.x, pr.gx, 0, nullptr)) return 1; } return 0; };
                auto run_fb = [&]() { return fast_run(*L, i, lf, pr.x, nullptr); };
                float t_sep = 0.f, t_fb = 0.f;
                if (run_fb() != 0) return 0;
                if (pr.time(run_sep, 3, &t_sep) || pr.time(run_fb, 3, &t_fb)) return 1;
                a.fb_b[bk] = (fb_force || t_fb < 0.97f * t_sep) ? 1 : 0;
                if (getenv("I2V_FUSE_DEBUG"))
                    fprintf(stderr, "[i2v fastblock] %s group %zu (%d launches, %d -> %d mid channels) at %d frames: separate %.1f us, fused %.1f us -> %s\n",
                            list_name(n, L), i, a.fb_ok, a.conv.Cs, a.conv.Cd, lf, 1e3f * t_sep, 1e3f * t_fb, a.fb_b[bk] ? "fused" : "separate");
                return 0;
            });
            for (int j = 0; j < a.fb_ok; ++j) { Launch& m = (*L)[i + j]; m.conv.cfg = m.cfg_b[0] ? m.cfg_b[0] : m.conv.cfg; }
            if (rc) return 1;
        }
    return 0;
}

int tune_pairs(Net& n, Probe& pr, int max_clips) {
    for (std::vector<Launch>* L : {&n.fwd, &n.bwd})
        for (size_t i = 0; i + 1 < L->size(); ++i) {
            Launch& a = (*L)[i]; Launch& b = (*L)[i + 1];
            if (!a.fuse_ok) continue;
            for (int bk = 0; bk < 4; ++bk) a.fuse_b[bk] = 0;
            const int rc = for_each_bucket(max_clips, a.conv.Tg, [&](int bk, int lf) -> int {
                if (!fused_fits(a, b, lf)) return 0;
                const int ca = a.conv.cfg, cb = b.conv.cfg;
                if (a.cfg_b[bk]) a.conv.cfg = a.cfg_b[bk];
                if (b.cfg_b[bk]) b.conv.cfg = b.cfg_b[bk];
                float best = 1e30f; int best_v = 0, rc = 0;
                for (int v = 0; v <= ((a.fuse_ok & 2) ? 2 : 1); ++v) {
                    auto once = [&]() { return v == 0 ? (conv_run(a, lf, pr.x, pr.gx, 0, nullptr) || conv_run(b, lf, pr.x, pr.gx, 0, nullptr))
                                                      : fused_run(a, b, lf, pr.x, v == 2, nullptr); };
                    if (v > 0 && once()) {
                        if (getenv("I2V_FUSE_DEBUG")) fprintf(stderr, "[i2v fuse] pair %zu variant %d does not launch: %s\n", i, v, g_err.c_str());
                        g_err.clear(); continue;
                    }
                    float ms = 0.f;
                    if (pr.time(once, 2, &ms, v == 0)) { rc = 1; break; }
                    if ((v == 0 ? ms : ms * 1.03f) < best) { best = v == 0 ? ms : ms * 1.03f; best_v = v; }
                    if (getenv("I2V_FUSE_DEBUG"))
                        fprintf(stderr, "[i2v fuse] %s pair %zu (Cd %d -> %d, %dx%d) at %d frames: variant %d = %.1f us\n", list_name(n, L), i,
                                a.conv.Cd, b.conv.Cd, a.conv.Hg, a.conv.Wg, lf, v, 1e3f * ms);
                }
                a.fuse_b[bk] = best_v;
                a.conv.cfg = ca; b.conv.cfg = cb;
                return rc;
            });
            if (rc) return 1;
        }
    return 0;
}

}

int autotune(Net& n) {
    const char* off = getenv("I2V_AUTOTUNE");
    if (off && off[0] == '0') return 0;
    int rc;
    {
        Probe pr;
        if (pr.init(n)) return 1;
        const int max_clips = n.maxN / n.Tin();
        const bool on_device = strncmp(be_name(), "hip", 3) == 0;
        rc = tune_tiles(n, pr, max_clips);
        if (!rc && on_device) rc = tune_fastblocks(n, pr, max_clips);
        static const bool fuse_on = [] { const char* e = getenv("I2V_FUSE"); return e && e[0] == '1'; }();
        if (!rc && fuse_on && on_device) rc = tune_pairs(n, pr, max_clips);
    }
    if (rc) return g_err.empty() ? fail("autotune failed") : 1;
    CHECK_BE(be_memset0(n.arena, n.arena_floats * sizeof(float), nullptr));
    return 0;
}

}
```

Baseline: 754.3.

## Launch strided-conv backward phase classes as one grouped grid

Adds a grouped implicit-GEMM kernel that runs all sub-pixel output classes of a strided conv's input-gradient (the backward launches sharing one node) in a single grid, with per-class weights, tap tables, sizes and block ranges. The class with the largest K is ordered first so heavy blocks are scheduled early. The autotuner times the separate launches against the grouped version for each tile config and frame bucket, and picks grouped only when it is clearly faster. This targets launch overhead and tail underutilisation from small per-class grids, at the cost of extra per-block class selection and more autotune time.

```diff
diff --git a/image-to-video-i2v-attack_amd/csrc/i2v_be.h b/image-to-video-i2v-attack_amd/csrc/i2v_be.h
--- a/image-to-video-i2v-attack_amd/csrc/i2v_be.h
+++ b/image-to-video-i2v-attack_amd/csrc/i2v_be.h
@@ -19,7 +19,7 @@
 int hip_fail(hipError_t e, const char* what);
 #define HIPCHK(x) do { hipError_t e_ = (x); if (e_ != hipSuccess) return hip_fail(e_, #x); } while (0)
 #define LAUNCH_CHECK(name) do { hipError_t e_ = hipGetLastError(); if (e_ != hipSuccess) return hip_fail(e_, name); } while (0)
-extern long long g_stat_conv, g_stat_pws, g_stat_bf3, g_stat_igh, g_stat_sth, g_stat_fastblock, g_stat_vfma, g_stat_igv, g_stat_gconv;
+extern long long g_stat_conv, g_stat_pws, g_stat_bf3, g_stat_igh, g_stat_sth, g_stat_fastblock, g_stat_vfma, g_stat_igv, g_stat_gconv, g_stat_classgroup;
 
 __device__ __forceinline__ unsigned fastdiv(unsigned n, unsigned m, unsigned s) {
     return (unsigned)(((unsigned long long)n * m) >> s);
@@ -84,6 +84,12 @@
 int launch_conv_cfg3(const I2VConvParams& p, hipStream_t s);
 int launch_conv_cfg4(const I2VConvParams& p, hipStream_t s);
 int launch_conv_cfg5(const I2VConvParams& p, hipStream_t s);
+int launch_conv_group_cfg0(const I2VConvGroupParams& g, hipStream_t s);
+int launch_conv_group_cfg1(const I2VConvGroupParams& g, hipStream_t s);
+int launch_conv_group_cfg2(const I2VConvGroupParams& g, hipStream_t s);
+int launch_conv_group_cfg3(const I2VConvGroupParams& g, hipStream_t s);
+int launch_conv_group_cfg4(const I2VConvGroupParams& g, hipStream_t s);
+int launch_conv_group_cfg5(const I2VConvGroupParams& g, hipStream_t s);
 bool conv_ighalo_ok(const I2VConvParams& p);
 int launch_conv_ighalo(const I2VConvParams& p, hipStream_t s);
 bool conv_igvfma_ok(const I2VConvParams& p);
diff --git a/image-to-video-i2v-attack_amd/csrc/i2v_conv_cfg0.hip b/image-to-video-i2v-attack_amd/csrc/i2v_conv_cfg0.hip
--- a/image-to-video-i2v-attack_amd/csrc/i2v_conv_cfg0.hip
+++ b/image-to-video-i2v-attack_amd/csrc/i2v_conv_cfg0.hip
@@ -1,3 +1,4 @@
 #include "i2v_conv_launch.h"
 
 int launch_conv_cfg0(const I2VConvParams& p, hipStream_t s) { return launch_conv_cfg<128, 128, 2, 2>(p, s); }
+int launch_conv_group_cfg0(const I2VConvGroupParams& g, hipStream_t s) { return launch_conv_group_cfg<128, 128, 2, 2>(g, s); }
diff --git a/image-to-video-i2v-attack_amd/csrc/i2v_conv_cfg1.hip b/image-to-video-i2v-attack_amd/csrc/i2v_conv_cfg1.hip
--- a/image-to-video-i2v-attack_amd/csrc/i2v_conv_cfg1.hip
+++ b/image-to-video-i2v-attack_amd/csrc/i2v_conv_cfg1.hip
@@ -1,3 +1,4 @@
 #include "i2v_conv_launch.h"
 
 int launch_conv_cfg1(const I2VConvParams& p, hipStream_t s) { return launch_conv_cfg<64, 128, 2, 2>(p, s); }
+int launch_conv_group_cfg1(const I2VConvGroupParams& g, hipStream_t s) { return launch_conv_group_cfg<64, 128, 2, 2>(g, s); }
diff --git a/image-to-video-i2v-attack_amd/csrc/i2v_conv_cfg2.hip b/image-to-video-i2v-attack_amd/csrc/i2v_conv_cfg2.hip
--- a/image-to-video-i2v-attack_amd/csrc/i2v_conv_cfg2.hip
+++ b/image-to-video-i2v-attack_amd/csrc/i2v_conv_cfg2.hip
@@ -1,3 +1,4 @@
 #include "i2v_conv_launch.h"
 
 int launch_conv_cfg2(const I2VConvParams& p, hipStream_t s) { return launch_conv_cfg<128, 64, 2, 2>(p, s); }
+int launch_conv_group_cfg2(const I2VConvGroupParams& g, hipStream_t s) { return launch_conv_group_cfg<128, 64, 2, 2>(g, s); }
diff --git a/image-to-video-i2v-attack_amd/csrc/i2v_conv_cfg3.hip b/image-to-video-i2v-attack_amd/csrc/i2v_conv_cfg3.hip
--- a/image-to-video-i2v-attack_amd/csrc/i2v_conv_cfg3.hip
+++ b/image-to-video-i2v-attack_amd/csrc/i2v_conv_cfg3.hip
@@ -1,3 +1,4 @@
 #include "i2v_conv_launch.h"
 
 int launch_conv_cfg3(const I2VConvParams& p, hipStream_t s) { return launch_conv_cfg<64, 64, 2, 2>(p, s); }
+int launch_conv_group_cfg3(const I2VConvGroupParams& g, hipStream_t s) { return launch_conv_group_cfg<64, 64, 2, 2>(g, s); }
diff --git a/image-to-video-i2v-attack_amd/csrc/i2v_conv_cfg4.hip b/image-to-video-i2v-attack_amd/csrc/i2v_conv_cfg4.hip
--- a/image-to-video-i2v-attack_amd/csrc/i2v_conv_cfg4.hip
+++ b/image-to-video-i2v-attack_amd/csrc/i2v_conv_cfg4.hip
@@ -1,3 +1,4 @@
 #include "i2v_conv_launch.h"
 
 int launch_conv_cfg4(const I2VConvParams& p, hipStream_t s) { return launch_conv_cfg<32, 256, 1, 4>(p, s); }
+int launch_conv_group_cfg4(const I2VConvGroupParams& g, hipStream_t s) { return launch_conv_group_cfg<32, 256, 1, 4>(g, s); }
diff --git a/image-to-video-i2v-attack_amd/csrc/i2v_conv_cfg5.hip b/image-to-video-i2v-attack_amd/csrc/i2v_conv_cfg5.hip
--- a/image-to-video-i2v-attack_amd/csrc/i2v_conv_cfg5.hip
+++ b/image-to-video-i2v-attack_amd/csrc/i2v_conv_cfg5.hip
@@ -1,3 +1,4 @@
 #include "i2v_conv_launch.h"
 
 int launch_conv_cfg5(const I2VConvParams& p, hipStream_t s) { return launch_conv_cfg<16, 256, 1, 4, true>(p, s); }
+int launch_conv_group_cfg5(const I2VConvGroupParams& g, hipStream_t s) { return launch_conv_group_cfg<16, 256, 1, 4, true>(g, s); }
diff --git a/image-to-video-i2v-attack_amd/csrc/i2v_conv_launch.h b/image-to-video-i2v-attack_amd/csrc/i2v_conv_launch.h
--- a/image-to-video-i2v-attack_amd/csrc/i2v_conv_launch.h
+++ b/image-to-video-i2v-attack_amd/csrc/i2v_conv_launch.h
@@ -71,3 +71,22 @@
     LAUNCH_CHECK("conv_igemm");
     return 0;
 }
+
+template <int BD, int BP, int WD, int WP, bool MF16 = false>
+static int launch_conv_group_cfg(const I2VConvGroupParams& g_in, hipStream_t s) {
+    I2VConvGroupParams g = g_in;
+    g.n_cd = (g.base.Cd + BD - 1) / BD;
+    int64_t grid = 0;
+    for (int c = 0; c < g.ncls; ++c) {
+        const int64_t P = (int64_t)g.base.N * g.cls[c].Hg * g.cls[c].Wg;
+        const int64_t nwg = (P + BP - 1) / BP * g.n_cd;
+        if (nwg <= 0 || grid + nwg > 0x7ffffff0) { snprintf(g_be_err, sizeof g_be_err, "class group: bad grid"); g_be_has_err = true; return 1; }
+        g.cls[c].first = (int32_t)grid; g.cls[c].nwg = (int32_t)nwg;
+        grid = (grid + nwg + 7) / 8 * 8;
+    }
+    for (int c = g.ncls; c < I2V_GROUP_MAX; ++c) g.cls[c] = g.cls[g.ncls - 1];
+    if (g.base.tap_uniform) hipLaunchKernelGGL((conv_igemm_group<BD, BP, WD, WP, 2, MF16>), dim3((unsigned)grid), dim3(256), 0, s, g);
+    else hipLaunchKernelGGL((conv_igemm_group<BD, BP, WD, WP, 0, MF16>), dim3((unsigned)grid), dim3(256), 0, s, g);
+    LAUNCH_CHECK("conv_igemm_group");
+    return 0;
+}
diff --git a/image-to-video-i2v-attack_amd/csrc/i2v_conv_tile.h b/image-to-video-i2v-attack_amd/csrc/i2v_conv_tile.h
--- a/image-to-video-i2v-attack_amd/csrc/i2v_conv_tile.h
+++ b/image-to-video-i2v-attack_amd/csrc/i2v_conv_tile.h
@@ -898,3 +898,25 @@
     }
     probe.exit(slot);
 }
+
+template <int BD, int BP, int WD, int WP, int MODE, bool MF16 = false>
+__global__ void __launch_bounds__(256) __attribute__((amdgpu_waves_per_eu(conv_waves_per_simd(BD, BP, false, false, MODE), conv_waves_per_simd(BD, BP, false, true, MODE))))
+conv_igemm_group(const I2VConvGroupParams g) {
+    __shared__ __attribute__((aligned(16))) float smem[conv_lds_floats<BD, BP, WD, MF16>()];
+    I2V_PROBE_T probe;
+    probe.entry();
+    const int b = (int)blockIdx.x;
+    int cls = 0;
+#pragma unroll
+    for (int c = 1; c < I2V_GROUP_MAX; ++c) if (c < g.ncls && b >= g.cls[c].first) cls = c;
+#define I2V_CLS(f) (cls == 0 ? g.cls[0].f : cls == 1 ? g.cls[1].f : cls == 2 ? g.cls[2].f : g.cls[3].f)
+    const int bid = b - I2V_CLS(first), nwg = I2V_CLS(nwg);
+    if (bid >= nwg) return;
+    I2VConvParams p = g.base;
+    p.wp = I2V_CLS(wp); p.ktab = I2V_CLS(ktab); p.K = I2V_CLS(K); p.Kpad = I2V_CLS(Kpad); p.Hg = I2V_CLS(Hg); p.Wg = I2V_CLS(Wg);
+    p.oh0 = I2V_CLS(oh0); p.ow0 = I2V_CLS(ow0);
+    p.dv_hw_m = I2V_CLS(dv_hw_m); p.dv_hw_s = I2V_CLS(dv_hw_s); p.dv_w_m = I2V_CLS(dv_w_m); p.dv_w_s = I2V_CLS(dv_w_s);
+#undef I2V_CLS
+    conv_tile<BD, BP, WD, WP, MODE, false, false, false, MF16>(p, g.n_cd, bid, nwg, 0, smem, probe, b);
+    probe.exit(b);
+}
diff --git a/image-to-video-i2v-attack_amd/csrc/i2v_engine.cpp b/image-to-video-i2v-attack_amd/csrc/i2v_engine.cpp
--- a/image-to-video-i2v-attack_amd/csrc/i2v_engine.cpp
+++ b/image-to-video-i2v-attack_amd/csrc/i2v_engine.cpp
@@ -343,6 +343,7 @@
     CHECK_BE(be_memset0(n.arena, n.arena_floats * sizeof(float), nullptr));
     if (!plan_pass(n, false, off, N, &end, &err)) return fail("plan: %s", err.c_str());
     mark_fusable(n);
+    mark_classgroups(n);
     if (autotune(n)) return 1;
     mark_overlap(n);
     CHECK_BE(be_stream_sync(nullptr));
diff --git a/image-to-video-i2v-attack_amd/csrc/i2v_kernels.h b/image-to-video-i2v-attack_amd/csrc/i2v_kernels.h
--- a/image-to-video-i2v-attack_amd/csrc/i2v_kernels.h
+++ b/image-to-video-i2v-attack_amd/csrc/i2v_kernels.h
@@ -1,4 +1,6 @@
 #pragma once
+#include <string.h>
+
 #include <initializer_list>
 #include "i2v_params.h"
 
@@ -40,6 +42,22 @@
     return true;
 }
 int k_conv_fused(const I2VConvParams& a, const I2VConvParams& b, int halo, i2v_stream_t s);
+inline bool i2v_conv_group_ok(const I2VConvParams* m, int n) {
+    if (n < 2 || n > I2V_GROUP_MAX) return false;
+    for (int i = 0; i < n; ++i) {
+        const I2VConvParams& q = m[i];
+        if (q.pointwise || q.quad || q.pre_scale || q.gate_scale || q.blk > 1 || q.blkt > 1 || q.temporal || q.bf3 || q.wp3 || q.vec_epilogue || q.gate_out) return false;
+        if (q.osh < 2 || q.osw != q.osh || q.oh0 < 0 || q.oh0 >= q.osh || q.ow0 < 0 || q.ow0 >= q.osw || q.Hg <= 0 || q.Wg <= 0 || q.N <= 0) return false;
+        for (int j = 0; j < i; ++j) if (m[j].oh0 == q.oh0 && m[j].ow0 == q.ow0) return false;
+        I2VConvParams r = q;
+        r.wp = m[0].wp; r.ktab = m[0].ktab; r.K = m[0].K; r.Kpad = m[0].Kpad; r.Hg = m[0].Hg; r.Wg = m[0].Wg; r.oh0 = m[0].oh0; r.ow0 = m[0].ow0;
+        r.dv_hw_m = m[0].dv_hw_m; r.dv_hw_s = m[0].dv_hw_s; r.dv_w_m = m[0].dv_w_m; r.dv_w_s = m[0].dv_w_s; r.cfg = m[0].cfg;
+        if (memcmp(&r, &m[0], sizeof r) != 0) return false;
+    }
+    return true;
+}
+int k_conv_group(const I2VConvParams* members, int n, int tile, i2v_stream_t s) __attribute__((weak));
+int k_conv_group_tiles(const I2VConvParams* members, int n, int* out) __attribute__((weak));
 int k_conv_candidates(const I2VConvParams& p, int* out);
 inline int i2v_fastblock_rows(const I2VConvParams& a, const I2VConvParams& b, const I2VConvParams* c, const I2VConvParams* d) {
     auto plain = [](const I2VConvParams& q) {
diff --git a/image-to-video-i2v-attack_amd/csrc/i2v_kernels.hip b/image-to-video-i2v-attack_amd/csrc/i2v_kernels.hip
--- a/image-to-video-i2v-attack_amd/csrc/i2v_kernels.hip
+++ b/image-to-video-i2v-attack_amd/csrc/i2v_kernels.hip
@@ -10,7 +10,7 @@
 }
 
 const char* be_name() { return "hip:gfx950"; }
-long long g_stat_conv = 0, g_stat_pws = 0, g_stat_bf3 = 0, g_stat_igh = 0, g_stat_sth = 0;
+long long g_stat_conv = 0, g_stat_pws = 0, g_stat_bf3 = 0, g_stat_igh = 0, g_stat_sth = 0, g_stat_classgroup = 0;
 long long be_stat(const char* name) {
     if (!strcmp(name, "conv_launches")) return __atomic_load_n(&g_stat_conv, __ATOMIC_RELAXED);
     if (!strcmp(name, "pws_launches")) return __atomic_load_n(&g_stat_pws, __ATOMIC_RELAXED);
@@ -21,6 +21,7 @@
     if (!strcmp(name, "vfma_launches")) return __atomic_load_n(&g_stat_vfma, __ATOMIC_RELAXED);
     if (!strcmp(name, "igvfma_launches")) return __atomic_load_n(&g_stat_igv, __ATOMIC_RELAXED);
     if (!strcmp(name, "gconv_launches")) return __atomic_load_n(&g_stat_gconv, __ATOMIC_RELAXED);
+    if (!strcmp(name, "classgroup_launches")) return __atomic_load_n(&g_stat_classgroup, __ATOMIC_RELAXED);
 #ifdef I2V_EXPERIMENTAL
     if (!strcmp(name, "experimental")) return 1;
 #else
@@ -185,6 +186,52 @@
         case 3: return launch_conv_cfg3(p, st);
         case 5: return launch_conv_cfg5(p, st);
         default: return launch_conv_cfg4(p, st);
+    }
+}
+
+int k_conv_group_tiles(const I2VConvParams* m, int n, int* out) {
+    if (!i2v_conv_group_ok(m, n)) return 0;
+    int cnt = 0;
+    static const int BD[6] = {128, 64, 128, 64, 32, 16};
+    for (int i = 0; i < 6; ++i) {
+        if (i < 4 && m[0].Cd <= BD[i] / 2) continue;
+        if (i == 4 && m[0].Cd > 32) continue;
+        if (i == 5 && m[0].Cd > 16) continue;
+        out[cnt++] = i;
+    }
+    return cnt;
+}
+
+int k_conv_group(const I2VConvParams* m_in, int n, int tile, i2v_stream_t s) {
+    if (!i2v_conv_group_ok(m_in, n)) { snprintf(g_be_err, sizeof g_be_err, "class group: the launches are not the classes of one input gradient"); g_be_has_err = true; return 1; }
+    int order[I2V_GROUP_MAX];
+    for (int i = 0; i < n; ++i) order[i] = i;
+    for (int i = 1; i < n; ++i)
+        for (int j = i; j > 0 && m_in[order[j]].Kpad > m_in[order[j - 1]].Kpad; --j) { const int t = order[j]; order[j] = order[j - 1]; order[j - 1] = t; }
+    if (tile < 0) { I2VConvParams q = m_in[order[0]]; q.cfg = 0; tile = conv_pick(q) & 7; }
+    if (tile > 5) { snprintf(g_be_err, sizeof g_be_err, "class group: no tile configuration %d", tile); g_be_has_err = true; return 1; }
+    I2VConvGroupParams g;
+    memset(&g, 0, sizeof g);
+    g.ncls = n;
+    for (int c = 0; c < n; ++c) {
+        I2VConvParams q = m_in[order[c]];
+        if ((int64_t)q.N * q.Hg * q.Wg + 1024 >= (1ll << 31)) { snprintf(g_be_err, sizeof g_be_err, "conv launch of more than 2^31 grid pixels"); g_be_has_err = true; return 1; }
+        conv_magics(q);
+        q.cfg = tile + 1;
+        if (c == 0) g.base = q;
+        I2VConvClass& k = g.cls[c];
+        k.wp = q.wp; k.ktab = q.ktab; k.K = q.K; k.Kpad = q.Kpad; k.Hg = q.Hg; k.Wg = q.Wg; k.oh0 = q.oh0; k.ow0 = q.ow0;
+        k.dv_hw_m = q.dv_hw_m; k.dv_hw_s = q.dv_hw_s; k.dv_w_m = q.dv_w_m; k.dv_w_s = q.dv_w_s;
+    }
+    __atomic_fetch_add(&g_stat_classgroup, 1, __ATOMIC_RELAXED);
+    hipStream_t st = (hipStream_t)s;
+    switch (tile) {
+        case 0: return launch_conv_group_cfg0(g, st);
+        case 1: return launch_conv_group_cfg1(g, st);
+        case 2: return launch_conv_group_cfg2(g, st);
+        case 3: return launch_conv_group_cfg3(g, st);
+        case 5: return launch_conv_group_cfg5(g, st);
+        default: return launch_conv_group_cfg4(g, st);
     }
 }
 
diff --git a/image-to-video-i2v-attack_amd/csrc/i2v_net.h b/image-to-video-i2v-attack_amd/csrc/i2v_net.h
--- a/image-to-video-i2v-attack_amd/csrc/i2v_net.h
+++ b/image-to-video-i2v-attack_amd/csrc/i2v_net.h
@@ -82,6 +82,8 @@
     int node = -1;
     int fb_ok = 0;
     int fb_b[4] = {0, 0, 0, 0};
+    int grp_ok = 0;
+    int grp_b[4] = {0, 0, 0, 0};
     int ov_after = -2, ov_join = -1;
 };
 inline int cfg_bucket(int clips, int max_clips) {
@@ -150,6 +152,7 @@
 bool plan_pass(Net& n, bool dry, size_t off, size_t N, size_t* end, std::string* err);
 
 void mark_fusable(Net& n);
+void mark_classgroups(Net& n);
 void mark_overlap(Net& n);
 int autotune(Net& n);
 
@@ -158,6 +161,8 @@
 bool fused_fits(const Launch& a, const Launch& b, int frames);
 int fused_run(const Launch& a, const Launch& b, int frames, const float* x, int halo, i2v_stream_t s);
 int fast_run(const std::vector<Launch>& L, size_t li, int frames, const float* x, i2v_stream_t s);
+bool group_prep(const std::vector<Launch>& L, size_t li, int frames, I2VConvParams* out);
+int group_run(const std::vector<Launch>& L, size_t li, int frames, int grp, i2v_stream_t s);
 extern long long g_overlap_launches;
 
 #pragma GCC visibility pop
diff --git a/image-to-video-i2v-attack_amd/csrc/i2v_params.h b/image-to-video-i2v-attack_amd/csrc/i2v_params.h
--- a/image-to-video-i2v-attack_amd/csrc/i2v_params.h
+++ b/image-to-video-i2v-attack_amd/csrc/i2v_params.h
@@ -42,6 +42,18 @@
     uint32_t dv_hw_m, dv_hw_s, dv_w_m, dv_w_s, dv_t_m, dv_t_s, dv_wo_m, dv_wo_s;
     const void* wp3; int32_t bf3;
     int32_t cfg;
+};
+
+#define I2V_GROUP_MAX 4
+struct I2VConvClass {
+    const float* wp; const I2VKEntry* ktab; int32_t K, Kpad, Hg, Wg, oh0, ow0;
+    uint32_t dv_hw_m, dv_hw_s, dv_w_m, dv_w_s;
+    int32_t first, nwg;
+};
+struct I2VConvGroupParams {
+    I2VConvParams base;
+    int32_t ncls, n_cd;
+    I2VConvClass cls[I2V_GROUP_MAX];
 };
 
 struct I2VFastStage {
diff --git a/image-to-video-i2v-attack_amd/csrc/i2v_run.cpp b/image-to-video-i2v-attack_amd/csrc/i2v_run.cpp
--- a/image-to-video-i2v-attack_amd/csrc/i2v_run.cpp
+++ b/image-to-video-i2v-attack_amd/csrc/i2v_run.cpp
@@ -54,6 +54,27 @@
     return 0;
 }
 
+bool group_prep(const std::vector<Launch>& L, size_t li, int frames, I2VConvParams* out) {
+    const int g = L[li].grp_ok;
+    if (!k_conv_group || g < 2 || g > I2V_GROUP_MAX || li + g > L.size()) return false;
+    for (int j = 0; j < g; ++j) {
+        const Launch& m = L[li + j];
+        if (m.kind != L_CONV || m.src_is_input || m.T != L[li].T || m.node != L[li].node) return false;
+        I2VConvParams& q = out[j];
+        q = conv_prep(m, nullptr, nullptr, 0);
+        const int64_t span = ((int64_t)frames * q.Ts / q.Tg - 1) * q.src_nstride * 4 + (int64_t)q.Cs * q.Hs * q.Ws * 4;
+        if (span >= (1ll << 31)) return false;
+        q.N = frames; q.src_span_bytes = (int32_t)span; q.cfg = 0;
+    }
+    return i2v_conv_group_ok(out, g);
+}
+int group_run(const std::vector<Launch>& L, size_t li, int frames, int grp, i2v_stream_t s) {
+    I2VConvParams q[I2V_GROUP_MAX];
+    if (!group_prep(L, li, frames, q)) return fail("class group: not eligible at %d frames", frames);
+    CHECK_BE(k_conv_group(q, L[li].grp_ok, grp - 2, s));
+    return 0;
+}
+
 int conv_run(const Launch& l, int frames, const float* x, float* gx, int accumulate, i2v_stream_t s) {
     I2VConvParams p = conv_prep(l, x, gx, accumulate);
     const int clips = frames / p.Tg;
@@ -103,10 +124,11 @@
     return t;
 }
 
-static double launch_flops(const std::vector<Launch>& L, size_t li, int fb, int fuse, int frames, int clips) {
+static double launch_flops(const std::vector<Launch>& L, size_t li, int fb, int fuse, int frames, int clips, int grp = 0) {
     const Launch& l = L[li];
     double flops = 0.0;
-    if (fb) { for (int j = 0; j < fb; ++j) { const Launch& m = L[li + j]; flops += m.alg_flops_per_frame > 0 ? m.alg_flops_per_frame * frames : 2.0 * frames * m.conv.Hg * m.conv.Wg * (double)m.conv.Cd * m.conv.K; } }
+    if (grp) { for (int j = 0; j < grp; ++j) flops += launch_flops(L, li + j, 0, 0, frames, clips); }
+    else if (fb) { for (int j = 0; j < fb; ++j) { const Launch& m = L[li + j]; flops += m.alg_flops_per_frame > 0 ? m.alg_flops_per_frame * frames : 2.0 * frames * m.conv.Hg * m.conv.Wg * (double)m.conv.Cd * m.conv.K; } }
     else if ((l.kind == L_CONV || l.kind == L_GCONV) && l.alg_flops_per_frame > 0) flops = l.alg_flops_per_frame * frames;
     else if (l.kind == L_CONV) flops = 2.0 * frames * l.conv.Hg * l.conv.Wg * ((double)l.conv.Cd * l.conv.K + (fuse ? (double)L[li + 1].conv.Cd * L[li + 1].conv.K : 0.0));
     else if (l.kind == L_IMGGRAD) flops = l.alg_flops_per_frame * frames;
@@ -125,11 +147,16 @@
     return 4;
 }
 
-static double launch_bytes(const std::vector<Launch>& L, size_t li, int fb, int fuse, int frames, int clips, int accumulate) {
+static double launch_bytes(const std::vector<Launch>& L, size_t li, int fb, int fuse, int frames, int clips, int accumulate, int grp = 0) {
     const Launch& l = L[li];
     const I2VConvParams& q = l.conv;
     const double out = (double)frames * q.Hg * q.Wg * q.Cd;
     const double src = (double)clips * q.Ts * q.Cs * q.Hs * q.Ws;
+    if (grp) {
+        double b = -4.0 * src * (grp - 1);
+        for (int j = 0; j < grp; ++j) b += launch_bytes(L, li + j, 0, 0, frames, clips, accumulate);
+        return b;
+    }
     double b = 4.0 * (src + (double)q.K * q.Cd + out);
     if (q.add0) b += 4.0 * out / (q.add0_stride * q.add0_stride);
     if (q.add1 || l.kind == L_IMGGRAD) b += (q.add1 || accumulate || l.img_accumulate) ? 4.0 * out : 0.0;
@@ -167,10 +194,10 @@
     TimedLaunch* prev = nullptr;
     TimedLaunch* seg = nullptr;
 
-    TimedLaunch* open(const std::vector<Launch>& L, size_t li, int fb, int fuse, int frames, int clips, int accumulate) {
+    TimedLaunch* open(const std::vector<Launch>& L, size_t li, int fb, int fuse, int frames, int clips, int accumulate, int grp = 0) {
         const Launch& l = L[li];
         const int kind = launch_timing_kind(l, backward_pass);
-        const double flops = launch_flops(L, li, fb, fuse, frames, clips);
+        const double flops = launch_flops(L, li, fb, fuse, frames, clips, grp);
         const bool conv = l.kind == L_CONV || l.kind == L_IMGGRAD || l.kind == L_GCONV;
         if (h->timing == 2) {
             if (!seg || seg->kind != kind) {
@@ -178,13 +205,14 @@
                 seg = timing_begin(h, kind, 0.0, s, seg);
                 if (seg) seg->count = 0;
             }
-            if (seg) { seg->flops += flops; seg->count += 1; if (conv) seg->bytes += launch_bytes(L, li, fb, fuse, frames, clips, accumulate); }
+            if (seg) { seg->flops += flops; seg->count += 1; if (conv) seg->bytes += launch_bytes(L, li, fb, fuse, frames, clips, accumulate, grp); }
             return prev = nullptr;
         }
         TimedLaunch* const tl = prev = timing_begin(h, kind, flops, s, prev);
         if (tl && conv) {
             tl->Cd = l.conv.Cd; tl->K = l.conv.K; tl->HWg = l.conv.Hg * l.conv.Wg; tl->frames = frames; tl->pw = l.conv.pointwise;
-            tl->bytes = launch_bytes(L, li, fb, fuse, frames, clips, accumulate);
+            tl->bytes = launch_bytes(L, li, fb, fuse, frames, clips, accumulate, grp);
+            for (int j = 1; j < grp; ++j) tl->K += L[li + j].conv.K;
         }
         if (tl && l.kind == L_AGEMM) {
             const I2VAttnGemm& q = l.ag;
@@ -252,8 +280,12 @@
         const int fuse = (l.kind == L_CONV && l.fuse_ok && li + 1 < L.size() && frames * l.conv.Hg * l.conv.Wg > 0 && fused_fits(l, L[li + 1], frames))
                              ? l.fuse_b[bucket] : 0;
         const int fb = (l.kind == L_CONV && l.fb_ok && li + l.fb_ok <= L.size() && frames * l.conv.Hg * l.conv.Wg > 0) ? l.fb_b[bucket] * l.fb_ok : 0;
-        if (overlap && side.join((int)li + (fb ? fb - 1 : fuse ? 1 : 0))) return 1;
-        TimedLaunch* const tl = h->timing ? timing.open(L, li, fb, fuse, frames, clips, accumulate) : nullptr;
+        int grp = (l.kind == L_CONV && l.grp_ok && !fb && !fuse && frames * l.conv.Hg * l.conv.Wg > 0) ? l.grp_b[bucket] : 0;
+        I2VConvParams gq[I2V_GROUP_MAX];
+        if (grp && !group_prep(L, li, frames, gq)) grp = 0;
+        const int grpn = grp ? l.grp_ok : 0;
+        if (overlap && side.join((int)li + (fb ? fb - 1 : fuse ? 1 : grpn ? grpn - 1 : 0))) return 1;
+        TimedLaunch* const tl = h->timing ? timing.open(L, li, fb, fuse, frames, clips, accumulate, grpn) : nullptr;
         struct Stop { TimedLaunch* t; i2v_stream_t s; ~Stop() { if (t) be_event_record(t->stop, s); } } stop{tl, s};
         switch (l.kind) {
             case L_CONV:
@@ -265,6 +297,7 @@
                     if (rc == 1) return 1;
                     if (rc == 0) { li += fb - 1; break; }
                 }
+                if (grp) { CHECK_BE(k_conv_group(gq, grpn, grp - 2, s)); li += grpn - 1; break; }
                 const int cb = l.cfg_b[bucket];
                 if (cb) l.conv.cfg = cb;
                 if (conv_run(l, frames, x, gx, accumulate, s)) return 1;
diff --git a/image-to-video-i2v-attack_amd/csrc/i2v_tune.cpp b/image-to-video-i2v-attack_amd/csrc/i2v_tune.cpp
--- a/image-to-video-i2v-attack_amd/csrc/i2v_tune.cpp
+++ b/image-to-video-i2v-attack_amd/csrc/i2v_tune.cpp
@@ -145,6 +145,31 @@
     for (std::vector<Launch>* L : {&n.fwd, &n.bwd})
         for (Launch& a : *L)
             for (int b = 0; b < 4; ++b) a.fuse_b[b] = (a.fuse_ok && f) ? ((f == 2 && (a.fuse_ok & 2)) ? 2 : 1) : 0;
+}
+
+void mark_classgroups(Net& n) {
+    for (std::vector<Launch>* L : {&n.fwd, &n.bwd})
+        for (Launch& l : *L) { l.grp_ok = 0; for (int b = 0; b < 4; ++b) l.grp_b[b] = 0; }
+    const char* e = getenv("I2V_CLASSGROUP");
+    if (!k_conv_group || (e && e[0] == '0')) return;
+    const bool force = e && e[0] == '1';
+    std::vector<Launch>& L = n.bwd;
+    for (size_t i = 0; i < L.size();) {
+        size_t j = i + 1;
+        if (L[i].kind == L_CONV && L[i].node >= 0)
+            while (j < L.size() && L[j].kind == L_CONV && L[j].node == L[i].node) ++j;
+        const size_t run = j - i;
+        if (run >= 2 && run <= I2V_GROUP_MAX) {
+            L[i].grp_ok = (int)run;
+            I2VConvParams q[I2V_GROUP_MAX];
+            if (!group_prep(L, i, L[i].T, q)) L[i].grp_ok = 0;
+            for (int b = 0; b < 4; ++b) L[i].grp_b[b] = (L[i].grp_ok && force) ? 1 : 0;
+            if (getenv("I2V_FUSE_DEBUG"))
+                fprintf(stderr, "[i2v classgroup] bwd launches %zu..%zu (node %d, Cd %d, %dx%d -> %dx%d): %s\n", i, j - 1, L[i].node, L[i].conv.Cd, L[i].conv.Hs, L[i].conv.Ws,
+                        L[i].conv.Ho, L[i].conv.Wo, L[i].grp_ok ? "one grid" : "not admitted");
+        }
+        i = j;
+    }
 }
 
 void mark_overlap(Net& n) {
@@ -209,6 +234,7 @@
             const Launch& l = (*L)[i];
             for (int j = 0; j < l.fb_ok && i + j < M; ++j) member[i + j] = 1;
             if (l.fuse_ok) { member[i] = 1; if (i + 1 < M) member[i + 1] = 1; }
+            for (int j = 0; j < l.grp_ok && i + j < M; ++j) member[i + j] = 1;
         }
         n.ov_at[k].assign(M + 1, {});
         int hoisted = 0;
@@ -345,6 +371,38 @@
     return 0;
 }
 
+int tune_classgroups(Net& n, Probe& pr, int max_clips) {
+    if (!k_conv_group || !k_conv_group_tiles) return 0;
+    const bool force = [] { const char* e = getenv("I2V_CLASSGROUP"); return e && e[0] == '1'; }();
+    for (std::vector<Launch>* L : {&n.fwd, &n.bwd})
+        for (size_t i = 0; i < L->size(); ++i) {
+            Launch& a = (*L)[i];
+            if (!a.grp_ok) continue;
+            for (int bk = 0; bk < 4; ++bk) a.grp_b[bk] = 0;
+            const int rc = for_each_bucket(max_clips, a.conv.Tg, [&](int bk, int lf) -> int {
+                I2VConvParams q[I2V_GROUP_MAX];
+                if (lf * a.conv.Hg * a.conv.Wg == 0 || !group_prep(*L, i, lf, q)) return 0;
+                int tiles[8]; const int nt = k_conv_group_tiles(q, a.grp_ok, tiles);
+                auto run_sep = [&]() { for (int j = 0; j < a.grp_ok; ++j) { Launch& m = (*L)[i + j]; if (m.cfg_b[bk]) m.conv.cfg = m.cfg_b[bk]; if (conv_run(m, lf, pr.x, pr.gx, 0, nullptr)) return 1; } return 0; };
+                float t_sep = 0.f, best = 1e30f; int best_t = -1;
+                if (pr.time(run_sep, 3, &t_sep)) return 1;
+                for (int ti = 0; ti < nt; ++ti) {
+                    float ms = 0.f;
+                    if (pr.time([&] { return group_run(*L, i, lf, tiles[ti] + 2, nullptr); }, 3, &ms)) return 1;
+                    if (ms < best) { best = ms; best_t = tiles[ti]; }
+                }
+                a.grp_b[bk] = (best_t >= 0 && (force || best < 0.97f * t_sep)) ? best_t + 2 : 0;
+                if (getenv("I2V_FUSE_DEBUG"))
+                    fprintf(stderr, "[i2v classgroup] %s group %zu (%d classes, Cd %d, %dx%d) at %d frames: separate %.1f us, one grid %.1f us on tile %d -> %s\n",
+                            list_name(n, L), i, a.grp_ok, a.conv.Cd, a.conv.Ho, a.conv.Wo, lf, 1e3f * t_sep, 1e3f * best, best_t, a.grp_b[bk] ? "one grid" : "separate");
+                return 0;
+            });
+            for (int j = 0; j < a.grp_ok; ++j) { Launch& m = (*L)[i + j]; m.conv.cfg = m.cfg_b[0] ? m.cfg_b[0] : m.conv.cfg; }
+            if (rc) return 1;
+        }
+    return 0;
+}
+
 int tune_pairs(Net& n, Probe& pr, int max_clips) {
     for (std::vector<Launch>* L : {&n.fwd, &n.bwd})
         for (size_t i = 0; i + 1 < L->size(); ++i) {
@@ -393,6 +451,7 @@
         const bool on_device = strncmp(be_name(), "hip", 3) == 0;
         rc = tune_tiles(n, pr, max_clips);
         if (!rc && on_device) rc = tune_fastblocks(n, pr, max_clips);
+        if (!rc && on_device) rc = tune_classgroups(n, pr, max_clips);
         static const bool fuse_on = [] { const char* e = getenv("I2V_FUSE"); return e && e[0] == '1'; }();
         if (!rc && fuse_on && on_device) rc = tune_pairs(n, pr, max_clips);
     }
```

New measurement: 757.2, median of 6. No clear change (+0.4%).
